# cchao0116/EasyDGL

Hardware: AMD Instinct MI355X
Metric: sequences/sec (fwd+bwd+Adam) B=512 L=100 d=128 |I|=20K (higher is better)
Workload: dtype bf16

## Files before the change

### easydgl_amd/_lib.py

```python
from __future__ import annotations

import ctypes
import os
from ctypes import c_char_p, c_float, c_int, c_int64, c_long, c_uint32, c_void_p

import torch

_HERE = os.path.dirname(os.path.abspath(__file__))
LIB_PATH = os.environ.get("EDGL_LIB_PATH") or os.path.join(_HERE, "libeasydgl_hip.so")

F32, BF16 = 0, 1
EPI_BIAS, EPI_GELU, EPI_SAVE_PRE, EPI_MUL_DGELU, EPI_ACCUM, EPI_OUT_F32, EPI_RELU = 1, 2, 4, 8, 16, 32, 64
MAU_CAUSAL, MAU_NO_DIAG, MAU_DIAG_ZERO = 1, 2, 4
MAU_NO_SKIP = 8
TATTN_CAUSAL = 1

P, I, F, L, U32, I64 = c_void_p, c_int, c_float, c_long, c_uint32, c_int64

SIGNATURES = {
    "edgl_last_error": (c_char_p, []),
    "edgl_version": (I, []),
    "edgl_profile_next": (I, [I, P, P]),
    "edgl_rng_advance": (I, [P, P]),
    "edgl_mask_random": (I, [P, I, I, I, I64, P, U32, P, P, P, P]),
    "edgl_mask_last": (I, [P, I, I, I64, P, P]),
    "edgl_encode_fwd": (I, [P, P, P, P, P, P, P, I, I, I, I, I, I64, F, F, P, U32, P, P, P, I, P]),
    "edgl_encode_bwd_workspace": (L, [I, I, I]),
    "edgl_encode_bwd": (I, [P, P, P, I, I, I, I, I, F, P, U32, P, P, P, P, I, P]),
    "edgl_encode_bwd_add": (I, [P, P, P, P, P, I, I, I, I, I, F, P, U32, P, P, P, P, I, P]),
    "edgl_encode_fwd_ct": (I, [P, P, P, P, P, P, P, I, I, I, I, I, I64, F, F, P, U32, P, P, P, I, I, I, P]),
    "edgl_encode_fwd_prep": (I, [P, P, P, P, P, P, P, I, I, I, I, I, I64, F, F, P, U32, P, P, P, I, I, P, I, P, P, P, P, P, P, I, P]),
    "edgl_encode_bwd_add_ct": (I, [P, P, P, P, P, I, I, I, I, I, F, P, U32, P, P, P, P, I, I, P]),
    "edgl_encode_bwd_label_fused": (I, [I, I]),
    "edgl_encode_bwd_add_label": (I, [P, P, P, P, P, I, I, I, I, I, F, P, U32, P, P, P, P, I, P, P, P, P, I, P, I, P]),
    "edgl_embed_pos_fwd": (I, [P, P, P, P, P, I, I, I, I, F, F, P, U32, P, P, P, I, P]),
    "edgl_embed_pos_bwd": (I, [P, P, I, I, I, I, F, P, U32, P, P, I, P]),
    "edgl_embed_pos_fwd_ct": (I, [P, P, P, P, P, I, I, I, I, F, F, P, U32, P, P, P, I, I, P]),
    "edgl_embed_pos_bwd_ct": (I, [P, P, I, I, I, I, F, P, U32, P, P, I, I, P]),
    "edgl_gemm": (I, [P, P, P, I, I, I, I, I, I, I, I, P, P, I, I, P, I, P]),
    "edgl_colsum": (I, [P, I, I, I, P, I, P, I, I, P]),
    "edgl_gemm_dw_workspace": (L, [I, I, I, I]),
    "edgl_gemm_dw": (I, [P, P, P, P, I, I, I, I, I, I, P, I, P]),
    "edgl_gemm_dw_defer": (I, [I, P]),
    "edgl_bimau_pack_bytes": (L, [I, I, I, I]),
    "edgl_bimau_pack": (I, [P, P, P, P, I, I, I, P, I, P]),
    "edgl_bimau_saved_bytes": (L, [I, I, I, I, I]),
    "edgl_bimau_mark_group": (I, [I, I, I]),
    "edgl_bimau_fwd": (I, [P, P, I, P, P, P, P, I, I, I, I, I, F, P, U32, P, P, P, I, I, P]),
    "edgl_bimau_fwd_zr": (I, [P, P, I, P, P, P, P, I, I, I, I, I, F, P, U32, P, P, P, P, I, I, P]),
    "edgl_bimau_dropbits_bytes": (L, [I, I, I]),
    "edgl_bimau_dropbits": (I, [I, I, I, F, P, U32, P, P]),
    "edgl_bimau_fwd_db": (I, [P, P, I, P, P, P, P, I, I, I, I, I, F, P, U32, P, F, P, P, P, P, I, I, P]),
    "edgl_bimau_bwd_db": (I, [P, P, P, P, P, P, P, P, P, I, I, I, I, I, F, P, U32, P, F, P, P, P, P, P, P, I, I, P]),
    "edgl_bimau_job_order": (I, [P, I, I, P, P]),
    "edgl_bimau_fwd_ord": (I, [P, P, I, P, P, P, P, I, I, I, I, I, F, P, U32, P, F, P, P, P, P, P, I, I, P]),
    "edgl_bimau_bwd_ord": (I, [P, P, P, P, P, P, P, P, I, P, F, P, P, P, I, I, I, I, I, F, P, U32, P, F, P, P, P, P, P, P, P, I, I, P]),
    "edgl_bimau_bwd_workspace": (L, [I, I, I, I, I, I]),
    "edgl_bimau_bwd": (I, [P, P, P, P, P, P, P, P, P, I, I, I, I, I, F, P, U32, P, P, P, P, P, P, I, I, P]),
    "edgl_add_layernorm_fwd": (I, [P, P, I, P, P, I, I, I, F, P, U32, P, I, P, P, I, P]),
    "edgl_add_layernorm_bwd": (I, [P, P, I, P, P, P, I, I, I, F, P, U32, P, I, P, P, P, P, P, P, I, P]),
    "edgl_add_layernorm_bwd_act": (I, [P, P, I, P, P, P, I, I, I, F, P, U32, P, I, P, P, P, P, P, P, P, I, P]),
    "edgl_add_layernorm_fwd_ct": (I, [P, P, I, P, P, I, I, I, F, P, U32, P, I, P, P, I, I, I, P]),
    "edgl_add_layernorm_bwd_act_ct": (I, [P, P, I, P, P, P, I, I, I, F, P, U32, P, I, P, P, P, P, P, P, P, I, I, I, P]),
    "edgl_score_chunks": (I, [I, I]),
    "edgl_compact_rows": (I, [P, P, I, I, P, P, P, P, P, I, P]),
    "edgl_compact_scan": (I, [P, I, P, P, P, P]),
    "edgl_compact_scan_labels": (I, [P, I, P, P, P, P, P]),
    "edgl_compact_gather": (I, [P, P, P, I, I, P, P, I, P]),
    "edgl_scatter_rows": (I, [P, P, I, I, P, I, P]),
    "edgl_score_lse_fwd": (I, [P, P, P, P, I, I, I, I, I, P, P, P, P, P, I, P]),
    "edgl_ce_loss_fwd": (I, [P, P, P, I, P, P, P]),
    "edgl_ce_loss_fwd_add": (I, [P, P, P, I, P, P, P, P, P]),
    "edgl_ce_loss_fwd_add_w": (I, [P, P, P, I, P, P, P, P, P, P]),
    "edgl_score_bwd_workspace": (L, [I, I, I, I, I]),
    "edgl_score_ce_bwd": (I, [P, P, P, P, P, P, P, I, I, I, I, I, P, P, P, P, P, I, P]),
    "edgl_score_flash_workspace": (L, [I, I, I, I, I]),
    "edgl_score_flash_fwd": (I, [P, P, P, P, I, I, I, I, I, P, P, P, P, I, P]),
    "edgl_score_prepare_table": (I, [P, I, I, I, I, I, P, I, P]),
    "edgl_score_flash_fwd_pre": (I, [P, P, P, P, I, I, I, I, I, P, P, P, P, I, I, P]),
    "edgl_score_flash_fwd_coef": (I, [P, P, P, P, I, I, I, P, P, P, P, P, I, P]),
    "edgl_score_flash_fwd_coef_w": (I, [P, P, P, P, I, I, I, P, P, P, P, P, P, I, P]),
    "edgl_score_flash_fwd_rows_w": (I, [P, P, P, P, I, I, I, P, P, P, P, P, P, P, P, I, P]),
    "edgl_score_ce_nparts": (I, [I, I]),
    "edgl_score_flash_fwd_rows_wp": (I, [P, P, P, P, I, I, I, P, P, P, P, P, P, P, P, P, I, P]),
    "edgl_ce_loss_parts": (I, [P, I, P, P, P, P, P]),
    "edgl_score_flash_bwd": (I, [P, P, P, P, P, P, P, I, I, I, I, I, P, P, P, P, P, I, P]),
    "edgl_score_flash_bwd_ex": (I, [P, P, P, P, P, P, P, I, I, I, I, I, P, P, P, P, P, I, I, P]),
    "edgl_score_flash_label_term": (I, [P, P, P, P, I, I, I, I, I, P, P, P, I, P]),
    "edgl_reduce_defer": (I, [I, P]),
    "edgl_reduce_flush": (I, [P]),
    "edgl_mask_topk": (I, [P, I, I, I, P, I, I, P, P, P]),
    "edgl_score_topk_fused_supported": (I, [I, I, I, I, I, I]),
    "edgl_score_topk_fused_workspace": (L, [I, I, I, I, I]),
    "edgl_score_topk_fused": (I, [P, P, P, P, I, I, I, I, I, I, I, P, P, P, I, P]),
    "edgl_topk_merge": (I, [P, P, I, I, I, P, P, P]),
    "edgl_rank_metrics": (I, [P, I, I, P, P, P]),
    "edgl_tpp_workspace": (I, []),
    "edgl_tpp_fwd": (I, [P, P, P, P, P, I, I, I, I, I, F, P, P, I, P]),
    "edgl_tpp_bwd": (I, [P, P, P, P, P, I, I, I, I, I, F, P, P, P, P]),
    "edgl_tpp_fwd_bwd": (I, [P, P, P, P, P, I, I, I, I, I, F, P, P, I, P, P]),
    "edgl_tpp_norm": (I, [P, P, I, I, I, P, P]),
    "edgl_tpp_fwd_bwd_ex": (I, [P, P, P, P, P, I, I, I, I, I, F, P, P, I, P, I, P]),
    "edgl_tpp_rows_workspace": (L, [I, I, I]),
    "edgl_tpp_fwd_bwd_rows": (I, [P, P, P, P, P, I, I, I, I, I, F, P, P, I, P, P]),
    "edgl_tpp_prep_bytes": (L, [I, I, I]),
    "edgl_tpp_prep": (I, [P, P, P, P, I, I, I, I, P, P]),
    "edgl_bimau_bwd_tpp": (I, [P, P, P, P, P, P, P, I, P, F, P, P, P, I, I, I, I, I, F, P, U32, P, F, P, P, P, P, P, P, I, I, P]),
# ... 130 lines not shown
```

### easydgl_amd/csrc/bimau_bwd_impl.h

```cpp
#pragma once
#include <algorithm>

#include "bimau_common.h"

#ifdef EDGL_PHASE_TIMING
extern __device__ unsigned long long g_phase_cycles[16];
#endif

namespace bimau {


constexpr int KY_ECH = 8;
constexpr int KY_NY = EP / KY_ECH;
constexpr int KY_BLOCKS = 384;

constexpr int WG_NJ64 = 4;
constexpr int big_nj(int dh) { return dh == 64 ? WG_NJ64 : 32 / (dh / 16); }
inline int big_row_splits(int dh, int E) {
    const int nc = big_nj(dh) * 16;
    const int groups = std::max(1, (dh * E + nc - 1) / nc);
    return std::max(16, 512 / groups);
}

struct WsLayout { size_t dz, dh, rowdot, dsc, wpart, total; };
inline WsLayout ws_layout(int B, int T_, int C, int H, int E) {
    const int dh = C / H;
    const bool big = dh >= 64;
    const size_t R = (size_t)B * H * T_;
    WsLayout w;
    size_t o = 0;
    auto take = [&](size_t bytes) { const size_t at = o; o += (bytes + 255) & ~(size_t)255; return at; };
    w.dz = take(R * EP * sizeof(float));
    w.dh = take((size_t)(big ? 1 : KY_NY) * R * dh * sizeof(float));
    w.rowdot = take(R * sizeof(float));
    w.dsc = take((size_t)B * H * EP * sizeof(float));
    w.wpart = take((size_t)(big ? big_row_splits(dh, E) : KY_BLOCKS) * ((size_t)(dh + 3) * dh * E + EP) * sizeof(float));
    w.total = o;
    return w;
}

struct BwdP {
    const void* qkvt; const int64_t* ids; const float* spans; const uint8_t* marks; const char* pack;
    const void* d_out; const float* d_lam_ext; const float* lam; const float* z; const void* hin;
    int B, T, C, H, E;
    float rate; const uint64_t* rng; uint32_t stream_id;
    void* d_qkvt;
    float* dz_ws; float* dh_ws; float* rowdot_ws; float* dsc_part; float* wpart;
    int waves;
    int flags;
    int noskip;
    const uint32_t* dbits;
    float qk_scale;
    const void* tpp_desc; int tpp_M; const float* tpp_sums; float tpp_coef;
    const int32_t* order;
    float* tpp_part;
};

template <typename T>
__device__ __forceinline__ void st_frag(T* dst, const f32x4& a) {
    Frag4<T> f = frag_from_acc<T>(a);
    if constexpr (sizeof(T) == 4) *reinterpret_cast<uint4*>(dst) = *reinterpret_cast<uint4*>(&f);
    else *reinterpret_cast<uint2*>(dst) = *reinterpret_cast<uint2*>(&f);
}

template <typename T, int DT, int NT, int EC, bool PREF = true, int FL = -1, bool DB = false, bool TP = false, bool SK = false>
__global__ __launch_bounds__(256) void bimau_bwd_sweep1_kernel(BwdP p) {
    constexpr int dh = 16 * DT, Tp = 16 * NT, LDT = Tp + 4;
    extern __shared__ __attribute__((aligned(16))) char smem[];
    const int E = EC ? EC : p.E;
    const int lane = threadIdx.x & 63, wave = __builtin_amdgcn_readfirstlane(threadIdx.x >> 6);
    const long slot = (long)blockIdx.x * p.waves + wave;
    if (slot >= (long)p.B * p.H) return;
    const int sb = (int)(slot / p.H), head = (int)(slot % p.H);
    const int b = p.order ? __builtin_amdgcn_readfirstlane(p.order[sb]) : sb;
    const long job = (long)b * p.H + head;
    const long bp = (long)head * p.B + b;
    const int g4 = (lane >> 4) * 4, l15 = lane & 15;
    constexpr bool SWZ = img_swz<T>();
    const int g4s = SWZ ? swz_col<16>(l15, g4) : g4;
    int cw[DT];
#pragma unroll
    for (int ub = 0; ub < DT; ++ub) cw[ub] = SWZ ? swz_col<16 * DT>(l15, ub * 16 + g4) : ub * 16 + g4;

    constexpr bool TR = sizeof(T) == 2;
    constexpr size_t EXTRA = TR ? 0 : (size_t)EP * LDT;
    constexpr size_t MASK_ELEMS = (size_t)Tp * sizeof(float) / sizeof(T);
    constexpr size_t WAVE_ELEMS = 2 * (size_t)Tp * dh + (size_t)Tp * EP + EXTRA + MASK_ELEMS;
    T* Ks = reinterpret_cast<T*>(smem) + (size_t)wave * WAVE_ELEMS;
    T* Vs = Ks + Tp * dh;
    T* Ms = Vs + Tp * dh;
    T* MTs = Ms + Tp * EP;
    const T* qkvt = reinterpret_cast<const T*>(p.qkvt) + (long)b * p.T * 4 * p.C;
    const T* dout = reinterpret_cast<const T*>(p.d_out) + (long)b * p.T * p.C;
    T* dqkvt = reinterpret_cast<T*>(p.d_qkvt) + (long)b * p.T * 4 * p.C;
    const int ldq = 4 * p.C;
    const KeyMask<NT> km = stage_wave<T, DT, NT, EC>(
        qkvt + p.C + head * dh, Ks, nullptr, static_cast<const T*>(nullptr), static_cast<T*>(nullptr), static_cast<T*>(nullptr),
        qkvt + 2 * p.C + head * dh, Vs, nullptr, ldq, p.marks + (long)b * p.T * E, E, Ms, TR ? nullptr : MTs,
        p.ids + (long)b * p.T, reinterpret_cast<float*>(Ks + WAVE_ELEMS - MASK_ELEMS), p.T, LDT, lane);
    __builtin_amdgcn_fence(__ATOMIC_RELEASE, "wavefront");
    __builtin_amdgcn_wave_barrier();

    const PackDims pd = pack_dims<T>(dh, E);
    const float* iscs_g = reinterpret_cast<const float*>(p.pack + pd.off_f32) + 3 * pd.JE + EP;
    float isc[4];
#pragma unroll
    for (int i = 0; i < 4; ++i) isc[i] = iscs_g[g4 + i];

    const float cscale = p.qk_scale > 0.f ? p.qk_scale : rsqrtf((float)dh);
    const DropKey dk = make_dropkey(p.rng, p.stream_id, p.rate);
    const Frag4<T> ident = identity_frag<T>(lane);
    const f32x4 zero4 = {0.f, 0.f, 0.f, 0.f};

    struct QOps { Frag4<T> qf[DT], dof[DT]; float4 z; float lam[4], dlx[4]; uint32_t kb; uint32_t nmw; float spr; };
    const float* dlx_src = p.d_lam_ext ? p.d_lam_ext : p.lam;
    const float dlx_on = p.d_lam_ext ? 1.0f : 0.0f;
    TppDesc td{};
    int tp_novf = 0;
    float tp_k = 0.f;
    if constexpr (TP) {
        td = tpp_desc(p.tpp_desc, p.B, p.T, p.tpp_M);
        tp_novf = __builtin_amdgcn_readfirstlane(td.novf[b]);
        int cnt;
        if (p.tpp_sums) {
            cnt = reinterpret_cast<const int*>(p.tpp_sums)[4];
        } else {
            cnt = 0;
            for (int i = lane; i < p.B; i += 64) cnt += td.cntp[i];
            for (int o = 32; o > 0; o >>= 1) cnt += __shfl_xor(cnt, o, 64);
        }
        tp_k = -p.tpp_coef / ((float)cnt * (float)p.H);
        if (job == 0 && lane == 0) reinterpret_cast<int*>(p.tpp_part)[2 * p.B * p.H] = cnt;
    }
    auto load_q = [&](int qt) {
        QOps o;
        const int q = min(qt * 16 + l15, p.T - 1);
        const long row = bp * p.T + q;
#pragma unroll
        for (int ub = 0; ub < DT; ++ub) {
            o.qf[ub] = frag_ld<T>(qkvt + (long)q * ldq + head * dh + ub * 16 + g4);
            o.dof[ub] = frag_ld<T>(dout + (long)q * p.C + head * dh + ub * 16 + g4);
        }
        o.z = *reinterpret_cast<const float4*>(p.z + row * EP + g4);
        if constexpr (DB) o.kb = p.dbits[(bp * NT + qt) * 64 + lane];
        if constexpr (TP) {
            const float4 l4 = *reinterpret_cast<const float4*>(p.lam + row * EC + g4);
            o.lam[0] = l4.x; o.lam[1] = l4.y; o.lam[2] = l4.z; o.lam[3] = l4.w;
            o.dlx[0] = 0.f; o.dlx[1] = 0.f; o.dlx[2] = 0.f; o.dlx[3] = 0.f;
            o.nmw = td.nmw[((long)b * p.T + q) * 4 + (lane >> 4)];
            o.spr = td.spr[(long)b * p.T + q];
        } else if constexpr (EC == 16) {
            const float4 l4 = *reinterpret_cast<const float4*>(p.lam + row * EC + g4), d4 = *reinterpret_cast<const float4*>(dlx_src + row * EC + g4);
            o.lam[0] = l4.x; o.lam[1] = l4.y; o.lam[2] = l4.z; o.lam[3] = l4.w;
            o.dlx[0] = d4.x; o.dlx[1] = d4.y; o.dlx[2] = d4.z; o.dlx[3] = d4.w;
        } else {
#pragma unroll
            for (int i = 0; i < 4; ++i) {
                const int e = min(g4 + i, E - 1);
                o.lam[i] = p.lam[row * E + e];
                o.dlx[i] = dlx_src[row * E + e];
            }
        }
        return o;
    };
    auto mask_q = [&](QOps& o, bool ok) {
#pragma unroll
        for (int ub = 0; ub < DT; ++ub)
            if (!ok) o.dof[ub] = frag_zero<T>();
#pragma unroll
        for (int i = 0; i < 4; ++i) {
            const bool oke = ok && (EC == 16 || (g4 + i) < E);
            o.lam[i] = oke ? o.lam[i] : 0.f;
            o.dlx[i] = oke ? o.dlx[i] * dlx_on : 0.f;
        }
    };
    PH_DECL
    auto run = [&](auto nk_c) {
    constexpr int NK = decltype(nk_c)::value, K0 = NT - NK;
    const KeyMask<NK> kmk = keymask_tail<NK, NT>(km);
    float dsc_acc[4] = {0.f, 0.f, 0.f, 0.f}, tp_a = 0.f, tp_b = 0.f;
    f32x4 dVa[DT][NK];
#pragma unroll
    for (int u = 0; u < DT; ++u)
#pragma unroll
        for (int kt = 0; kt < NK; ++kt) dVa[u][kt] = zero4;
    QOps qcur = load_q(0);
    touch_regs(qcur);
    float pend_dz[4] = {0.f, 0.f, 0.f, 0.f}, pend_rowdot = 0.f;
    int pend_q = p.T;
    auto flush_pending = [&]() {
        if (pend_q < p.T) {
            *reinterpret_cast<float4*>(p.dz_ws + (bp * p.T + pend_q) * EP + g4) = make_float4(pend_dz[0], pend_dz[1], pend_dz[2], pend_dz[3]);
            if (lane < 16) p.rowdot_ws[bp * p.T + pend_q] = pend_rowdot;
        }
    };
    for (int qt = 0; qt < NT; ++qt) {
        asm volatile("" ::: "memory");
        const int q = qt * 16 + l15;
        const bool qok = q < p.T;
        QOps qnext;
        if constexpr (PREF) qnext = load_q(qt + 1 < NT ? qt + 1 : qt);
        asm volatile("" ::: "memory");
        mask_q(qcur, qok);
        if constexpr (TP) {
            float gr[4] = {0.f, 0.f, 0.f, 0.f};
            tpp_slot(qcur.lam, qcur.nmw, qcur.spr, qok && qcur.spr >= 0.f, tp_k, gr, tp_a, tp_b);
            for (int j = 0; j < tp_novf; ++j) {
                const int tj = td.ovf_pos[(long)b * td.M + j];
                if ((tj >> 4) != qt) continue;
                tpp_slot(qcur.lam, td.ovf_nm[((long)b * td.M + j) * 4 + (lane >> 4)], qcur.spr, qok && q == tj, tp_k, gr, tp_a, tp_b);
            }
#pragma unroll
            for (int i = 0; i < 4; ++i) qcur.dlx[i] = gr[i];
        }
        const float zq4[4] = {qcur.z.x, qcur.z.y, qcur.z.z, qcur.z.w};
        f32x4 s[NK];
#pragma unroll
        for (int kt = 0; kt < NK; ++kt) {
            f32x4 a = zero4;
#pragma unroll
            for (int ub = 0; ub < DT; ++ub)
                a = mma16(frag_ld<T>(Ks + ((K0 + kt) * 16 + l15) * dh + cw[ub]), qcur.qf[ub], a);
            s[kt] = a;
        }
        if constexpr (FL == 0) masked_softmax_impl<NK, false, false>(s, kmk, cscale, lane, q, dk.scale);
        else {
            masked_softmax<NK, 0>(s, kmk, cscale, lane, q, (p.flags & MAU_CAUSAL) != 0);
#pragma unroll
            for (int kt = 0; kt < NK; ++kt)
#pragma unroll
                for (int r = 0; r < 4; ++r) s[kt][r] *= dk.scale;
        }
        asm volatile("" ::: "memory");
        flush_pending();
        asm volatile("" ::: "memory");
        PH_MARK(0);
        Frag4<T> lf;
#pragma unroll
        for (int i = 0; i < 4; ++i) lf.v[i] = from_f32<T>(qcur.lam[i]);
        Frag4<T> dOT[DT];
#pragma unroll
        for (int vt = 0; vt < DT; ++vt) dOT[vt] = frag_from_acc<T>(mma16(qcur.dof[vt], ident, zero4));
        float rowdot = 0.f;
        f32x4 dlamT = zero4;
        const uint32_t dbase = (uint32_t)((bp * p.T + q) * p.T);
#pragma unroll
        for (int kt = 0; kt < NK; ++kt) {
            const f32x4 gacc = mma16(frag_ld<T>(Ms + ((K0 + kt) * 16 + l15) * EP + g4s), lf, zero4);
            f32x4 da = zero4;
#pragma unroll
            for (int vb = 0; vb < DT; ++vb)
                da = mma16(frag_ld<T>(Vs + ((K0 + kt) * 16 + l15) * dh + cw[vb]), qcur.dof[vb], da);
            f32x4 ap, dg, gv = gacc;
            const bool dtile = K0 + kt == qt && (FL == 0 || !(p.flags & MAU_NO_DIAG));
            if constexpr (FL == 0) {
#pragma unroll
                for (int r = 0; r < 4; ++r) gv[r] = (dtile && g4 + r == l15) ? 1.0f : gacc[r];
            } else if (dtile) {
#pragma unroll
                for (int r = 0; r < 4; ++r) gv[r] = (g4 + r == l15) ? ((p.flags & MAU_DIAG_ZERO) ? 0.0f : 1.0f) : gacc[r];
            }
            uint64_t hw = 0ull;
            if constexpr (!DB) hw = drop_hash_quad(dk, dbase + (K0 + kt) * 16 + g4);
            const bool keep[4] = {drop_quad_keep<0>(dk, hw), drop_quad_keep<1>(dk, hw), drop_quad_keep<2>(dk, hw), drop_quad_keep<3>(dk, hw)};
#pragma unroll
            for (int r = 0; r < 4; ++r) {
                float fp;
                if constexpr (DB) fp = keep_bit(qcur.kb, (K0 + kt) * 4 + r, s[kt][r]);
                else fp = keep[r] ? s[kt][r] : 0.f;
                ap[r] = gv[r] * fp;
                dg[r] = da[r] * fp;
                rowdot = fmaf(dg[r], gv[r], rowdot);
            }
            if constexpr (FL == 0) {
#pragma unroll
                for (int r = 0; r < 4; ++r) dg[r] = (dtile && g4 + r == l15) ? 0.f : dg[r];
            } else if (dtile) {
#pragma unroll
                for (int r = 0; r < 4; ++r) dg[r] = (g4 + r == l15) ? 0.f : dg[r];
            }
            dlamT = mma16(kfrag<T, SWZ ? 16 : 0>(Ms, EP, MTs, LDT, (K0 + kt) * 16, 0, lane), frag_from_acc<T>(dg), dlamT);
            const Frag4<T> apT = frag_from_acc<T>(transpose_tile<T>(ap, ident));
#pragma unroll
            for (int vt = 0; vt < DT; ++vt) dVa[vt][kt] = mma16(dOT[vt], apT, dVa[vt][kt]);
            if (kt & 1) __builtin_amdgcn_sched_barrier(0);
        }
        PH_MARK(1);
        float dz4[4];
#pragma unroll
        for (int i = 0; i < 4; ++i) {
            const float dl = dlamT[i] + qcur.dlx[i];
            const float sg = sigmoid_f(zq4[i] * isc[i]);
            dz4[i] = dl * sg;
            if (qok && (EC == 16 || (g4 + i) < E)) dsc_acc[i] += dl * (qcur.lam[i] - zq4[i] * sg);
        }
        pend_rowdot = group_sum4(rowdot);
#pragma unroll
        for (int i = 0; i < 4; ++i) pend_dz[i] = dz4[i];
        pend_q = q;
        if constexpr (PREF) qcur = qnext;
        else if (qt + 1 < NT) qcur = load_q(qt + 1);
        PH_MARK(2);
    }
#pragma unroll
    for (int i = 0; i < 4; ++i) {
        float v = dsc_acc[i];
        v += __shfl_xor(v, 1, 64); v += __shfl_xor(v, 2, 64); v += __shfl_xor(v, 4, 64); v += __shfl_xor(v, 8, 64);
        dsc_acc[i] = v;
    }
    if constexpr (TP) {
#pragma unroll
        for (int o = 1; o < 16; o <<= 1) { tp_a += __shfl_xor(tp_a, o, 64); tp_b += __shfl_xor(tp_b, o, 64); }
    }
    flush_pending();
    if constexpr (TP) {
        if (lane == 0) *reinterpret_cast<float2*>(p.tpp_part + job * 2) = make_float2(tp_a, tp_b);
    }
    if (l15 == 0) *reinterpret_cast<float4*>(p.dsc_part + job * EP + g4) = make_float4(dsc_acc[0], dsc_acc[1], dsc_acc[2], dsc_acc[3]);
#pragma unroll
    for (int kt = 0; kt < NT; ++kt) {
        const int k = kt * 16 + l15;
        if (k < p.T) {
#pragma unroll
            for (int ut = 0; ut < DT; ++ut) {
                T* dst = dqkvt + (long)k * ldq + 2 * p.C + head * dh + ut * 16 + g4;
                if constexpr (K0 > 0) {
                    if (kt < K0) st_frag<T>(dst, zero4);
                    else st_frag<T>(dst, dVa[ut][kt < K0 ? 0 : kt - K0]);
                } else {
                    st_frag<T>(dst, dVa[ut][kt]);
                }
            }
        }
    }
    };
    if constexpr (SK) {
        static_assert(FL == 0 && sizeof(T) == 2, "the key-tile skip exists for the bidirectional bf16 form");
        dispatch_nk<NT>(NT - km.kt0, run);
    } else {
        run(std::integral_constant<int, NT>{});
    }
    PH_MARK(3);
    PH_FLUSH(0);
}

template <typename T, int DT, int NT, int EC, int NYP = KY_NY, bool PREF = true, int FL = -1, bool DB = false, int US = 1, int SL = 0, bool SK = false>
__global__ __launch_bounds__(256) void bimau_bwd_sweep2_kernel(BwdP p) {
    constexpr int dh = 16 * DT, Tp = 16 * NT, LDT = Tp + 4;
    static_assert(DT % US == 0 && SL < US, "channel slices");
    constexpr int DTS = DT / US, U0 = SL * DTS;
    extern __shared__ __attribute__((aligned(16))) char smem[];
    const int E = EC ? EC : p.E;
    const int lane = threadIdx.x & 63, wave = __builtin_amdgcn_readfirstlane(threadIdx.x >> 6);
    const long slot = (long)blockIdx.x * p.waves + wave;
    if (slot >= (long)p.B * p.H) return;
    const int sb = (int)(slot / p.H), head = (int)(slot % p.H);
    const int b = p.order ? __builtin_amdgcn_readfirstlane(p.order[sb]) : sb;
    const long job = (long)b * p.H + head;
    const long bp = (long)head * p.B + b;
    const int g4 = (lane >> 4) * 4, l15 = lane & 15;
    constexpr bool SWZ = img_swz<T>();
    const int g4s = SWZ ? swz_col<16>(l15, g4) : g4;
    int cw[DT];
#pragma unroll
    for (int ub = 0; ub < DT; ++ub) cw[ub] = SWZ ? swz_col<16 * DT>(l15, ub * 16 + g4) : ub * 16 + g4;

    constexpr bool TR = sizeof(T) == 2;
    constexpr size_t EXTRA = TR ? 0 : (size_t)dh * LDT;
    constexpr size_t MASK_ELEMS = (size_t)Tp * sizeof(float) / sizeof(T);
    constexpr size_t WAVE_ELEMS = 3 * (size_t)Tp * dh + (size_t)Tp * EP + EXTRA + MASK_ELEMS;
    T* Ks = reinterpret_cast<T*>(smem) + (size_t)wave * WAVE_ELEMS;
    T* Ts = Ks + Tp * dh;
    T* Vs = Ts + Tp * dh;
    T* Ms = Vs + Tp * dh;
    T* KTs = Ms + Tp * EP;
    const T* qkvt = reinterpret_cast<const T*>(p.qkvt) + (long)b * p.T * 4 * p.C;
    const T* dout = reinterpret_cast<const T*>(p.d_out) + (long)b * p.T * p.C;
    const T* hin = reinterpret_cast<const T*>(p.hin);
    T* dqkvt = reinterpret_cast<T*>(p.d_qkvt) + (long)b * p.T * 4 * p.C;
    const int ldq = 4 * p.C;
    const KeyMask<NT> km = stage_wave<T, DT, NT, EC>(
        qkvt + p.C + head * dh, Ks, TR ? nullptr : KTs, qkvt + 3 * p.C + head * dh, Ts, static_cast<T*>(nullptr),
        qkvt + 2 * p.C + head * dh, Vs, static_cast<T*>(nullptr), ldq, p.marks + (long)b * p.T * E, E, Ms, static_cast<T*>(nullptr),
        p.ids + (long)b * p.T, reinterpret_cast<float*>(Ks + WAVE_ELEMS - MASK_ELEMS), p.T, LDT, lane);
    __builtin_amdgcn_fence(__ATOMIC_RELEASE, "wavefront");
    __builtin_amdgcn_wave_barrier();

    const float cscale = p.qk_scale > 0.f ? p.qk_scale : rsqrtf((float)dh);
    const DropKey dk = make_dropkey(p.rng, p.stream_id, p.rate);
    float cz = cscale;
    if constexpr (FL == 0) {
        bool real = false;
        for (int k = lane; k < Tp; k += 64) real |= km.madd[k] == 0.f;
        cz = __any(real) ? cscale : 0.f;
    }
    (void)cz;
    const Frag4<T> ident = identity_frag<T>(lane);
    const f32x4 zero4 = {0.f, 0.f, 0.f, 0.f};
    const long R = (long)p.B * p.H * p.T;

    struct QOps { Frag4<T> qf[DT], dof[DT], hf[DT]; float4 dHp[DT][NYP]; float lam[4], rowdot; uint32_t kb; };
    auto load_q = [&](int qt) {
        QOps o;
        const int q = min(qt * 16 + l15, p.T - 1);
        const long row = bp * p.T + q;
#pragma unroll
        for (int ub = 0; ub < DT; ++ub) {
            o.qf[ub] = frag_ld<T>(qkvt + (long)q * ldq + head * dh + ub * 16 + g4);
            o.dof[ub] = frag_ld<T>(dout + (long)q * p.C + head * dh + ub * 16 + g4);
            o.hf[ub] = frag_ld<T>(hin + row * dh + ub * 16 + g4);
#pragma unroll
            for (int y = 0; y < NYP; ++y)
                o.dHp[ub][y] = *reinterpret_cast<const float4*>(p.dh_ws + ((long)y * R + row) * dh + ub * 16 + g4);
        }
        if constexpr (EC == 16) {
            const float4 l4 = *reinterpret_cast<const float4*>(p.lam + row * EC + g4);
            o.lam[0] = l4.x; o.lam[1] = l4.y; o.lam[2] = l4.z; o.lam[3] = l4.w;
        } else {
#pragma unroll
            for (int i = 0; i < 4; ++i) o.lam[i] = p.lam[row * E + min(g4 + i, E - 1)];
        }
        o.rowdot = p.rowdot_ws[row];
        if constexpr (DB) o.kb = p.dbits[(bp * NT + qt) * 64 + lane];
        return o;
    };
    PH_DECL
#ifdef EDGL_PHASE_TIMING
    const unsigned long long clk_m0 = __builtin_readcyclecounter(), clk_r0 = wall_clock64();
#endif
    auto run = [&](auto nk_c) {
    constexpr int NK = decltype(nk_c)::value, K0 = NT - NK;
    const KeyMask<NK> kmk = keymask_tail<NK, NT>(km);
    f32x4 dKa[DTS][NK], dTa[DTS][NK];
#pragma unroll
    for (int u = 0; u < DTS; ++u)
#pragma unroll
        for (int kt = 0; kt < NK; ++kt) { dKa[u][kt] = zero4; dTa[u][kt] = zero4; }
    QOps qcur = load_q(0);
    touch_regs(qcur);
    Frag4<T> pend_dq[DTS];
    int pend_q = p.T;
    auto flush_pending = [&]() {
        if (pend_q < p.T) {
#pragma unroll
            for (int ut = 0; ut < DTS; ++ut) {
                T* dst = dqkvt + (long)pend_q * ldq + head * dh + (U0 + ut) * 16 + g4;
                if constexpr (sizeof(T) == 4) *reinterpret_cast<uint4*>(dst) = *reinterpret_cast<uint4*>(&pend_dq[ut]);
                else *reinterpret_cast<uint2*>(dst) = *reinterpret_cast<uint2*>(&pend_dq[ut]);
            }
        }
    };
#pragma unroll
    for (int ut = 0; ut < DTS; ++ut) pend_dq[ut] = frag_zero<T>();
    for (int qt = 0; qt < NT; ++qt) {
        asm volatile("" ::: "memory");
        const int q = qt * 16 + l15;
        const bool qok = q < p.T;
        (void)qok;
        QOps qnext;
        if constexpr (PREF) qnext = load_q(qt + 1 < NT ? qt + 1 : qt);
        asm volatile("" ::: "memory");
        PH_MARK(3);
        f32x4 dHq[DT];
#pragma unroll
        for (int ub = 0; ub < DT; ++ub) {
            f32x4 a = zero4;
#pragma unroll
            for (int y = 0; y < NYP; ++y) {
                a[0] += qcur.dHp[ub][y].x; a[1] += qcur.dHp[ub][y].y; a[2] += qcur.dHp[ub][y].z; a[3] += qcur.dHp[ub][y].w;
            }
#pragma unroll
            for (int r = 0; r < 4; ++r) dHq[ub][r] = qok ? a[r] : 0.f;
            if (!qok) qcur.dof[ub] = frag_zero<T>();
        }
        const float rowdot1 = qok ? qcur.rowdot : 0.f;
        PH_MARK(4);
        f32x4 s[NK];
#pragma unroll
        for (int kt = 0; kt < NK; ++kt) {
            f32x4 a = zero4;
#pragma unroll
            for (int ub = 0; ub < DT; ++ub)
                a = mma16(frag_ld<T>(Ks + ((K0 + kt) * 16 + l15) * dh + cw[ub]), qcur.qf[ub], a);
            s[kt] = a;
        }
        PH_MARK(5);
        if constexpr (FL == 0) masked_softmax_impl<NK, false, false>(s, kmk, cscale, lane, q);
        else masked_softmax<NK, 0>(s, kmk, cscale, lane, q, (p.flags & MAU_CAUSAL) != 0);
        asm volatile("" ::: "memory");
        flush_pending();
        asm volatile("" ::: "memory");
        PH_MARK(0);
        Frag4<T> lf;
#pragma unroll
        for (int i = 0; i < 4; ++i) lf.v[i] = from_f32<T>((EC == 16 || (g4 + i) < E) ? qcur.lam[i] * dk.scale : 0.f);
        float rowdot = 0.f;
        Frag4<T> dhf[DT], QT[DTS], dHT[DTS];
#pragma unroll
        for (int ut = 0; ut < DT; ++ut) {
#pragma unroll
            for (int r = 0; r < 4; ++r) rowdot = fmaf(dHq[ut][r], to_f32(qcur.hf[ut].v[r]), rowdot);
            dhf[ut] = frag_from_acc<T>(dHq[ut]);
        }
#pragma unroll
        for (int ut = 0; ut < DTS; ++ut) {
            QT[ut] = frag_from_acc<T>(mma16(qcur.qf[U0 + ut], ident, zero4));
            dHT[ut] = frag_from_acc<T>(transpose_tile<T>(dHq[U0 + ut], ident));
        }
        rowdot = group_sum4(rowdot) + rowdot1;
        f32x4 dQ[DTS];
#pragma unroll
        for (int ut = 0; ut < DTS; ++ut) dQ[ut] = zero4;
        const uint32_t dbase = (uint32_t)((bp * p.T + q) * p.T);
#pragma unroll
        for (int kt = 0; kt < NK; ++kt) {
            const f32x4 gacc = mma16(frag_ld<T>(Ms + ((K0 + kt) * 16 + l15) * EP + g4s), lf, zero4);
            f32x4 da = zero4;
#pragma unroll
            for (int vb = 0; vb < DT; ++vb)
                da = mma16(frag_ld<T>(Vs + ((K0 + kt) * 16 + l15) * dh + cw[vb]), qcur.dof[vb], da);
            f32x4 gv = gacc;
            if constexpr (FL == 0) {
                const bool dtile = K0 + kt == qt;
#pragma unroll
                for (int r = 0; r < 4; ++r) gv[r] = (dtile && g4 + r == l15) ? dk.scale : gacc[r];
            } else if (kt == qt && !(p.flags & MAU_NO_DIAG)) {
#pragma unroll
                for (int r = 0; r < 4; ++r) gv[r] = (g4 + r == l15) ? ((p.flags & MAU_DIAG_ZERO) ? 0.0f : dk.scale) : gacc[r];
            }
            uint64_t hw = 0ull;
            if constexpr (!DB) hw = drop_hash_quad(dk, dbase + (K0 + kt) * 16 + g4);
            const bool keep[4] = {drop_quad_keep<0>(dk, hw), drop_quad_keep<1>(dk, hw), drop_quad_keep<2>(dk, hw), drop_quad_keep<3>(dk, hw)};
            f32x4 a;
#pragma unroll
            for (int r = 0; r < 4; ++r) {
                if constexpr (DB) a[r] = keep_bit(qcur.kb, (K0 + kt) * 4 + r, da[r] * gv[r]);
                else a[r] = keep[r] ? da[r] * gv[r] : 0.f;
            }
#pragma unroll
            for (int ub = 0; ub < DT; ++ub)
                a = mma16(frag_ld<T>(Ts + ((K0 + kt) * 16 + l15) * dh + cw[ub]), dhf[ub], a);
            f32x4 ds;
#pragma unroll
            for (int r = 0; r < 4; ++r) {
                if constexpr (FL == 0) {
                    ds[r] = s[kt][r] * (a[r] - rowdot);
                } else {
                    const bool padded = ((km.pad >> (kt * 4 + r)) & 1ull) || ((p.flags & MAU_CAUSAL) && kt * 16 + g4 + r > q);
                    ds[r] = padded ? 0.f : s[kt][r] * (a[r] - rowdot) * cscale;
                }
            }
            const Frag4<T> dsf = frag_from_acc<T>(ds);
#pragma unroll
            for (int ut = 0; ut < DTS; ++ut)
                dQ[ut] = mma16(kfrag<T, SWZ ? 16 * DT : 0>(Ks, dh, KTs, LDT, (K0 + kt) * 16, (U0 + ut) * 16, lane), dsf, dQ[ut]);
            const Frag4<T> dsT = frag_from_acc<T>(transpose_tile<T>(ds, ident));
            const Frag4<T> pT = frag_from_acc<T>(transpose_tile<T>(s[kt], ident));
#pragma unroll
            for (int ut = 0; ut < DTS; ++ut) {
                dKa[ut][kt] = mma16(QT[ut], dsT, dKa[ut][kt]);
                dTa[ut][kt] = mma16(dHT[ut], pT, dTa[ut][kt]);
            }
        }
#pragma unroll
        for (int ut = 0; ut < DTS; ++ut) {
            if constexpr (FL == 0) {
#pragma unroll
                for (int r = 0; r < 4; ++r) dQ[ut][r] *= cz;
            }
            pend_dq[ut] = frag_from_acc<T>(dQ[ut]);
        }
        pend_q = q;
        if constexpr (PREF) qcur = qnext;
        else if (qt + 1 < NT) qcur = load_q(qt + 1);
        PH_MARK(1);
    }
    flush_pending();
#pragma unroll
    for (int kt = 0; kt < NT; ++kt) {
        const int k = kt * 16 + l15;
        if (k < p.T) {
#pragma unroll
            for (int ut = 0; ut < DTS; ++ut) {
                T* row = dqkvt + (long)k * ldq + head * dh + (U0 + ut) * 16 + g4;
                if (kt < K0) {
                    st_frag<T>(row + p.C, zero4);
                    st_frag<T>(row + 3 * p.C, zero4);
                } else {
                    const int kk = kt < K0 ? 0 : kt - K0;
                    if constexpr (FL == 0) {
#pragma unroll
                        for (int r = 0; r < 4; ++r) dKa[ut][kk][r] *= cz;
                    }
                    st_frag<T>(row + p.C, dKa[ut][kk]);
                    st_frag<T>(row + 3 * p.C, dTa[ut][kk]);
                }
            }
        }
    }
    };
    if constexpr (SK) {
        static_assert(FL == 0 && sizeof(T) == 2, "the key-tile skip exists for the bidirectional bf16 form");
        dispatch_nk<NT>(NT - km.kt0, run);
    } else {
        run(std::integral_constant<int, NT>{});
    }
    PH_MARK(2);
    PH_FLUSH(8);
#ifdef EDGL_PHASE_TIMING
    if (lane == 0) { atomicAdd(&g_phase_cycles[14], __builtin_readcyclecounter() - clk_m0); atomicAdd(&g_phase_cycles[15], wall_clock64() - clk_r0); }
#endif
}


int big_bwd(const BwdP& p, char* ws, float* dW1, float* db1, float* dw, float* dsc, int dtype, hipStream_t st);

}
```

### easydgl_amd/csrc/bimau_common.h

```cpp
#pragma once
#include <cstdlib>
#include <type_traits>

#include "edgl_common.h"

namespace bimau {

constexpr int EP = 16;
constexpr float NLOG2E = -1.4426950408889634f;

__device__ __forceinline__ float sigmoid_pre(float xs) { return fast_rcp(1.0f + __builtin_amdgcn_exp2f(xs)); }

constexpr int XW = 8;
struct PackDims {
    int dh, E, JE, LDW, LDR;
    size_t off_w1x, off_f32, off_w1r, fwd_bytes, bytes;
};
template <typename T>
__host__ __device__ inline PackDims pack_dims(int dh, int E) {
    PackDims d;
    d.dh = dh; d.E = E; d.JE = dh * E; d.LDW = dh + 4; d.LDR = d.JE + 4;
    size_t w1t = (size_t)d.JE * d.LDW * sizeof(T);
    w1t = (w1t + 15) & ~(size_t)15;
    const size_t w1x = sizeof(T) == 2 ? (size_t)d.JE * XW * sizeof(T) : 0;
// ... 58 lines not shown
}

template <typename T>
__global__ void pack_kernel(const float* W1, const float* b1, const float* w, const float* scaling, int dh, int E,
                            char* pack) {
    const PackDims d = pack_dims<T>(dh, E);
    T* w1t = reinterpret_cast<T*>(pack);
    T* w1r = reinterpret_cast<T*>(pack + d.off_w1r);
    float* f = reinterpret_cast<float*>(pack + d.off_f32);
    const int tid = blockIdx.x * blockDim.x + threadIdx.x, nth = gridDim.x * blockDim.x;
    if constexpr (sizeof(T) == 2) {
        T* w1x = reinterpret_cast<T*>(pack + d.off_w1x);
        for (int j = tid; j < d.JE; j += nth) {
            const Split3 w = split3(NLOG2E * W1[(long)dh * d.JE + j]), b = split3(NLOG2E * b1[j]);
            T* r = w1x + (long)j * XW;
            r[0] = w.t0; r[1] = w.t1; r[2] = w.t0; r[3] = w.t2; r[4] = w.t1; r[5] = w.t0; r[6] = b.t0; r[7] = b.t1;
        }
    }
    for (int i = tid; i < d.JE * d.LDW; i += nth) {
        const int j = i / d.LDW, u = i % d.LDW;
        w1t[i] = from_f32<T>(u < dh ? NLOG2E * W1[(long)u * d.JE + j] : 0.f);
    }
    for (int i = tid; i < dh * d.LDR; i += nth) {
        const int u = i / d.LDR, j = i % d.LDR;
        w1r[i] = from_f32<T>(j < d.JE ? W1[(long)u * d.JE + j] : 0.f);
    }
    for (int j = tid; j < d.JE; j += nth) {
        f[j] = NLOG2E * W1[(long)dh * d.JE + j];
        f[d.JE + j] = NLOG2E * b1[j];
        f[2 * d.JE + j] = w[j];
    }
    for (int e = tid; e < EP; e += nth) {
        const float s = e < E ? __expf(scaling[e]) : 1.f;
        f[3 * d.JE + e] = s;
        f[3 * d.JE + EP + e] = 1.f / s;
    }
}

template <int NT>
struct KeyMask { const float* madd; uint64_t pad; int kt0; };
template <int NR>
__device__ __forceinline__ int first_real_tile(const uint64_t (&real)[NR]) {
    int first = -1;
#pragma unroll
    for (int i = NR - 1; i >= 0; --i)
        if (real[i] != 0ull) first = 64 * i + (int)__builtin_ctzll(real[i]);
    return first < 0 ? 0 : first >> 4;
}
template <int NK, int NT>
__device__ __forceinline__ KeyMask<NK> keymask_tail(const KeyMask<NT>& km) {
    constexpr int K0 = NT - NK;
    return KeyMask<NK>{km.madd + K0 * 16, km.pad >> (K0 * 4), 0};
}
inline bool bimau_skip_enabled() {
    return edgl_env_on("EDGL_BIMAU_SKIP");
}
template <int N, typename F>
__device__ __forceinline__ void dispatch_nk(int nk, F&& f) {
    if constexpr (N <= 1) {
        f(std::integral_constant<int, 1>{});
    } else {
        if (nk >= N) f(std::integral_constant<int, N>{});
        else dispatch_nk<N - 1>(nk, f);
    }
}
template <int NT>
__device__ __forceinline__ KeyMask<NT> load_keymask(const int64_t* ids_row, int T, int lane, float* lds_madd) {
    KeyMask<NT> km;
    km.pad = 0ull;
    km.madd = lds_madd;
    constexpr int NR = (16 * NT + 63) / 64;
    uint64_t padded[NR], real[NR];
#pragma unroll
    for (int i = 0; i < NR; ++i) {
        const int k = lane + 64 * i;
        const int64_t id = ids_row[min(k, T - 1)];
        const bool pd = k < T && id == 0;
        padded[i] = __ballot(pd);
        real[i] = __ballot(k < T && id != 0);
        if (k < 16 * NT) lds_madd[k] = k >= T ? -INFINITY : (pd ? -4294967296.0f : 0.f);
    }
    km.kt0 = first_real_tile<NR>(real);
    const int g4 = (lane >> 4) * 4;
#pragma unroll
    for (int kt = 0; kt < NT; ++kt) {
        const uint64_t nib = (padded[kt / 4] >> ((kt % 4) * 16 + g4)) & 0xfull;
        km.pad |= nib << (kt * 4);
    }
    return km;
}

constexpr int MAU_CAUSAL = 1;
constexpr int MAU_NO_DIAG = 2;
constexpr int MAU_DIAG_ZERO = 4;
typedef __attribute__((ext_vector_type(2))) float f32x2;
template <int NT, bool CAUSAL, bool VEC, bool NORM = true>
__device__ __forceinline__ float masked_softmax_impl(f32x4 (&s)[NT], const KeyMask<NT>& km, float cscale, int lane, int q, float post = 1.0f) {
    const float c2 = cscale * 1.4426950408889634f;
    float mx = -INFINITY;
    const float* mrow = km.madd + (lane >> 4) * 4;
#pragma unroll
    for (int kt = 0; kt < NT; ++kt) {
        const f32x4 m4 = *reinterpret_cast<const f32x4*>(mrow + kt * 16);
        f32x4 v;
        if constexpr (VEC) {
            v = s[kt] * f32x4{c2, c2, c2, c2} + m4;
// ... 40 lines not shown
    if constexpr (!NORM) return inv;
    const float f = inv * post;
#pragma unroll
    for (int kt = 0; kt < NT; ++kt) {
        if constexpr (VEC) {
            s[kt] *= f32x4{f, f, f, f};
        } else {
#pragma unroll
            for (int r = 0; r < 4; ++r) s[kt][r] *= f;
        }
    }
    return inv;
}
template <int NT, int MODE = 0>
__device__ __forceinline__ void masked_softmax(f32x4 (&s)[NT], const KeyMask<NT>& km, float cscale, int lane, int q = 0,
                                               bool causal = false) {
    if constexpr (MODE != 0) {
        if (causal) masked_softmax_impl<NT, true, false>(s, km, cscale, lane, q);
        else masked_softmax_impl<NT, false, false>(s, km, cscale, lane, q);
    } else {
        const float c2 = cscale * 1.4426950408889634f;
        float mx = -INFINITY;
        const float* mrow = km.madd + (lane >> 4) * 4;
#pragma unroll
        for (int kt = 0; kt < NT; ++kt) {
            const float4 m4 = *reinterpret_cast<const float4*>(mrow + kt * 16);
            const float mm[4] = {m4.x, m4.y, m4.z, m4.w};
#pragma unroll
            for (int r = 0; r < 4; ++r) {
                float v = fmaf(s[kt][r], c2, mm[r]);
                if (causal && kt * 16 + (lane >> 4) * 4 + r > q && mm[r] != -INFINITY) v = -4294967296.0f;
                s[kt][r] = v;
                mx = fmaxf(mx, v);
            }
        }
        mx = group_max4(mx);
        float sum = 0.f;
#pragma unroll
        for (int kt = 0; kt < NT; ++kt)
#pragma unroll
            for (int r = 0; r < 4; ++r) {
                const float e = __builtin_amdgcn_exp2f(s[kt][r] - mx);
                s[kt][r] = e;
                sum += e;
            }
        sum = group_sum4(sum);
        const float inv = fast_rcp(sum);
#pragma unroll
        for (int kt = 0; kt < NT; ++kt)
#pragma unroll
            for (int r = 0; r < 4; ++r) s[kt][r] *= inv;
    }
}

template <int I>
__device__ __forceinline__ float keep_bit_c(uint32_t kb, float x) {
    int m;
    asm("v_bfe_i32 %0, %1, %2, 1" : "=v"(m) : "v"(kb), "n"(I));
    return __int_as_float(__float_as_int(x) & m);
}
__device__ __forceinline__ float keep_bit(uint32_t kb, int i, float x) {
    switch (i) {
#define EDGL_KB_CASE(n) case n: return keep_bit_c<n>(kb, x);
        EDGL_KB_CASE(0) EDGL_KB_CASE(1) EDGL_KB_CASE(2) EDGL_KB_CASE(3) EDGL_KB_CASE(4) EDGL_KB_CASE(5) EDGL_KB_CASE(6) EDGL_KB_CASE(7)
        EDGL_KB_CASE(8) EDGL_KB_CASE(9) EDGL_KB_CASE(10) EDGL_KB_CASE(11) EDGL_KB_CASE(12) EDGL_KB_CASE(13) EDGL_KB_CASE(14) EDGL_KB_CASE(15)
        EDGL_KB_CASE(16) EDGL_KB_CASE(17) EDGL_KB_CASE(18) EDGL_KB_CASE(19) EDGL_KB_CASE(20) EDGL_KB_CASE(21) EDGL_KB_CASE(22) EDGL_KB_CASE(23)
        EDGL_KB_CASE(24) EDGL_KB_CASE(25) EDGL_KB_CASE(26) EDGL_KB_CASE(27) EDGL_KB_CASE(28) EDGL_KB_CASE(29) EDGL_KB_CASE(30) EDGL_KB_CASE(31)
#undef EDGL_KB_CASE
    }
    return x;
}
template <int NT>
__global__ __launch_bounds__(256) void dropbits_kernel(const uint64_t* rng, uint32_t stream_id, float rate, int T, long njobs, uint32_t* bits) {
    static_assert(NT <= 8, "one 32-bit word per lane and query tile");
    const int lane = threadIdx.x & 63;
    const long job = (long)blockIdx.x * 4 + (threadIdx.x >> 6);
    if (job >= njobs) return;
    const long bp = job / NT;
    const int qt = (int)(job % NT), q = qt * 16 + (lane & 15), g4 = (lane >> 4) * 4;
    const DropKey dk = make_dropkey(rng, stream_id, rate);
    const uint32_t dbase = (uint32_t)((bp * T + q) * T);
    uint32_t w = 0u;
#pragma unroll
    for (int kt = 0; kt < NT; ++kt) {
        const uint64_t hw = drop_hash_quad(dk, dbase + kt * 16 + g4);
        w |= (drop_quad_keep<0>(dk, hw) ? 1u : 0u) << (kt * 4);
        w |= (drop_quad_keep<1>(dk, hw) ? 1u : 0u) << (kt * 4 + 1);
        w |= (drop_quad_keep<2>(dk, hw) ? 1u : 0u) << (kt * 4 + 2);
        w |= (drop_quad_keep<3>(dk, hw) ? 1u : 0u) << (kt * 4 + 3);
    }
    bits[job * 64 + lane] = w;
}

struct TppDesc {
    const uint32_t* nmw;
    const float* spr;
    const int32_t* novf;
    const int32_t* ovf_pos;
    const uint32_t* ovf_nm;
    const int32_t* cntp;
    int M;
};
struct TppLayout { size_t off_spr, off_novf, off_ovf_pos, off_ovf_nm, off_cntp, bytes; };
__host__ __device__ inline TppLayout tpp_layout(int B, int T, int M) {
    TppLayout l;
    l.off_spr = (size_t)B * T * 16;
    l.off_novf = l.off_spr + (size_t)B * T * 4;
    l.off_ovf_pos = (l.off_novf + (size_t)B * 4 + 15) & ~(size_t)15;
    l.off_ovf_nm = (l.off_ovf_pos + (size_t)B * M * 4 + 15) & ~(size_t)15;
    l.off_cntp = l.off_ovf_nm + (size_t)B * M * 16;
    l.bytes = l.off_cntp + (((size_t)B * 4 + 15) & ~(size_t)15);
    return l;
}
__host__ __device__ inline TppDesc tpp_desc(const void* base, int B, int T, int M) {
    const TppLayout l = tpp_layout(B, T, M);
    const char* c = reinterpret_cast<const char*>(base);
    return TppDesc{reinterpret_cast<const uint32_t*>(c), reinterpret_cast<const float*>(c + l.off_spr),
                   reinterpret_cast<const int32_t*>(c + l.off_novf), reinterpret_cast<const int32_t*>(c + l.off_ovf_pos),
                   reinterpret_cast<const uint32_t*>(c + l.off_ovf_nm), reinterpret_cast<const int32_t*>(c + l.off_cntp), M};
}
__device__ __forceinline__ void tpp_bytes(uint32_t w, float (&f)[4]) {
    f[0] = (float)(w & 0xffu); f[1] = (float)((w >> 8) & 0xffu);
    f[2] = (float)((w >> 16) & 0xffu); f[3] = (float)(w >> 24);
}
__device__ __forceinline__ void group_sum4_pair(float& x, float& y) {
    const FPair p = swap16(x, y);
    const float t = p.first + p.second;
    const FPair q = swap32(t, t);
    const float u = q.first + q.second;
    const FPair r = swap16(u, u);
    x = r.first; y = r.second;
}
__device__ __forceinline__ void tpp_slot(const float (&lam4)[4], uint32_t w, float sp, bool on, float k, float (&gr)[4], float& a, float& bs) {
    float f[4];
    tpp_bytes(w, f);
    float ev = lam4[0] * f[0], ent = lam4[0] + lam4[1];
    ev = fmaf(lam4[1], f[1], ev); ev = fmaf(lam4[2], f[2], ev); ev = fmaf(lam4[3], f[3], ev);
    ent += lam4[2] + lam4[3];
    group_sum4_pair(ev, ent);
    ev = on ? ev : 0.f;
    const float hs = sp * 0.5f, kg = on ? k : 0.f;
    a += __logf(ev == 0.f ? 1.f : ev);
    bs = fmaf(on ? ent : 0.f, hs, bs);
// ... 94 lines not shown
#pragma unroll
    for (int i = 0; i < NR; ++i) {
        const int k = lane + 64 * i;
        const uint8_t* row = marks_row + (long)min(k, Tlen - 1) * E;
        uint32_t w[4];
        if constexpr (EC == 16) {
            const uint4 v = *reinterpret_cast<const uint4*>(row);
            w[0] = v.x; w[1] = v.y; w[2] = v.z; w[3] = v.w;
        } else {
            uint8_t by[16];
#pragma unroll
            for (int e = 0; e < 16; ++e) by[e] = row[min(e, E - 1)];
#pragma unroll
            for (int j = 0; j < 4; ++j) {
                w[j] = 0u;
#pragma unroll
                for (int e = 0; e < 4; ++e) w[j] |= (4 * j + e < E ? (uint32_t)by[4 * j + e] : 0u) << (8 * e);
            }
        }
        if (k < Tp) {
            const bool ok = k < Tlen;
            T vals[16];
#pragma unroll
            for (int e = 0; e < 16; ++e) vals[e] = from_f32<T>(ok ? (float)((w[e / 4] >> (8 * (e % 4))) & 0xffu) : 0.f);
            if (rowmajor) {
#pragma unroll
                for (int j = 0; j < (int)(16 * sizeof(T) / 16); ++j)
                    reinterpret_cast<uint4*>(rowmajor + k * EP)[SW ? (j ^ ((k >> 3) & 1)) : j] = reinterpret_cast<const uint4*>(vals)[j];
            }
            if (transposed) {
#pragma unroll
                for (int e = 0; e < 16; ++e) transposed[e * LDT + k] = vals[e];
            }
        }
    }
}

template <typename T, int DT, int NT>
struct RowStage {
    static constexpr int cpr = 4 * DT, dh = 16 * DT, NI = NT * DT;
    Frag4<T> f[NI];
    __device__ __forceinline__ void load(const T* src, int ld, int Tlen, int lane) {
#pragma unroll
        for (int j = 0; j < NI; ++j) {
            const int c = lane + 64 * j, k = c / cpr, u4 = (c % cpr) * 4;
            f[j] = frag_ld<T>(src + (long)min(k, Tlen - 1) * ld + u4);
        }
    }
    __device__ __forceinline__ void pin() {
        static_assert(sizeof(Frag4<T>) == 8, "bf16 fragments");
#pragma unroll
        for (int j = 0; j < NI; ++j) { uint2& u = *reinterpret_cast<uint2*>(&f[j]); asm volatile("" : "+v"(u.x), "+v"(u.y)); }
    }
    __device__ __forceinline__ void store(T* rowmajor, T* transposed, int LDT, int Tlen, int lane) {
#pragma unroll
        for (int j = 0; j < NI; ++j) {
            const int c = lane + 64 * j, k = c / cpr, u4 = (c % cpr) * 4;
            if (k >= Tlen) f[j] = frag_zero<T>();
            if (rowmajor) *reinterpret_cast<uint2*>(rowmajor + k * dh + (img_swz<T>() ? swz_col<dh>(k, u4) : u4)) = *reinterpret_cast<uint2*>(&f[j]);
            if (transposed) {
#pragma unroll
                for (int r = 0; r < 4; ++r) transposed[(u4 + r) * LDT + k] = f[j].v[r];
            }
        }
    }
};
template <typename T, int DT, int NT, int EC>
constexpr bool stage_merged() { return sizeof(T) == 2 && NT * DT <= 8 && EC == 16; }

template <typename T, int DT, int NT, int EC>
__device__ __forceinline__ KeyMask<NT> stage_wave(const T* k_src, T* k_rm, T* k_tr, const T* t_src, T* t_rm, T* t_tr,
                                                  const T* v_src, T* v_rm, T* v_tr, int ld, const uint8_t* marks_row, int E,
                                                  T* m_rm, T* m_tr, const int64_t* ids_row, float* lds_madd, int Tlen, int LDT,
                                                  int lane) {
    if constexpr (stage_merged<T, DT, NT, EC>()) {
        constexpr int Tp = 16 * NT, NR = (Tp + 63) / 64;
        RowStage<T, DT, NT> sk, st, sv;
        uint4 mk[NR];
        int64_t id[NR];
        sk.load(k_src, ld, Tlen, lane);
        if (t_src) st.load(t_src, ld, Tlen, lane);
        if (v_src) sv.load(v_src, ld, Tlen, lane);
#pragma unroll
        for (int i = 0; i < NR; ++i) {
            const int k = min(lane + 64 * i, Tlen - 1);
            if (marks_row) mk[i] = *reinterpret_cast<const uint4*>(marks_row + (long)k * 16);
            id[i] = ids_row[k];
        }
        sk.pin();
        if (t_src) st.pin();
        if (v_src) sv.pin();
#pragma unroll
        for (int i = 0; i < NR; ++i) {
            if (marks_row) asm volatile("" : "+v"(mk[i].x), "+v"(mk[i].y), "+v"(mk[i].z), "+v"(mk[i].w));
            asm volatile("" : "+v"(id[i]));
        }
        sk.store(k_rm, k_tr, LDT, Tlen, lane);
        if (t_src) st.store(t_rm, t_tr, LDT, Tlen, lane);
        if (v_src) sv.store(v_rm, v_tr, LDT, Tlen, lane);
        if (marks_row) {
#pragma unroll
            for (int i = 0; i < NR; ++i) {
                const int k = lane + 64 * i;
                if (k < Tp) {
                    const bool ok = k < Tlen;
                    const uint32_t w[4] = {mk[i].x, mk[i].y, mk[i].z, mk[i].w};
                    T vals[16];
#pragma unroll
                    for (int e = 0; e < 16; ++e) vals[e] = from_f32<T>(ok ? (float)((w[e / 4] >> (8 * (e % 4))) & 0xffu) : 0.f);
                    if (m_rm) {
#pragma unroll
                        for (int j = 0; j < (int)(16 * sizeof(T) / 16); ++j)
                            reinterpret_cast<uint4*>(m_rm + k * EP)[img_swz<T>() ? (j ^ ((k >> 3) & 1)) : j] = reinterpret_cast<const uint4*>(vals)[j];
                    }
                    if (m_tr) {
#pragma unroll
                        for (int e = 0; e < 16; ++e) m_tr[e * LDT + k] = vals[e];
                    }
                }
            }
        }
        KeyMask<NT> km;
        km.pad = 0ull;
        km.madd = lds_madd;
        uint64_t padded[NR], real[NR];
#pragma unroll
        for (int i = 0; i < NR; ++i) {
            const int k = lane + 64 * i;
// ... 24 lines not shown
```

### easydgl_amd/csrc/bimau_fwd_impl.h

```cpp
#pragma once
#include <type_traits>

#include "bimau_common.h"

namespace bimau {

constexpr int FWD_WAVES = 2;

struct FwdP {
    const void* qkvt; const void* resid; int ld_res;
    const int64_t* ids; const float* spans; const uint8_t* marks;
    const char* pack;
    int B, T, C, H, E;
    float rate; const uint64_t* rng; uint32_t stream_id;
    void* out; float* lam;
    void* hin_out; float* z_out;
    float* zero_rows;
    int waves;
    int flags;
    const uint32_t* dbits;
    float qk_scale;
    const int32_t* order;
    int noskip;
};

template <typename T, int DT, int NT, int PHASE>
__host__ __device__ constexpr size_t fwd_wave_bytes() {
    constexpr size_t dh = 16 * DT, Tp = 16 * NT, LDT = Tp + 4;
    constexpr size_t kv = sizeof(T) == 2 ? Tp * dh : dh * LDT;
    return (Tp * dh + (PHASE != 2 ? kv : 0) + (PHASE != 1 ? kv : 0) + (PHASE != 1 ? Tp * EP : 0)) * sizeof(T) + Tp * sizeof(float);
}

template <typename T, int DT, int NT, int EC, int PHASE = 0, bool DB = false, bool SK = false>
__global__ __launch_bounds__(256, (sizeof(T) == 2 && DT == 1 && EC == 16 && PHASE == 0) ? FWD_WAVES : 1) void bimau_fwd_kernel(FwdP p) {
    constexpr int dh = 16 * DT, Tp = 16 * NT, LDT = Tp + 4;
    extern __shared__ __attribute__((aligned(16))) char smem[];
    const int E = EC ? EC : p.E;
    constexpr bool FUSED = PHASE == 0, HAS_T = PHASE != 2, HAS_V = PHASE != 1, HAS_M = PHASE != 1;
    const PackDims pd = pack_dims<T>(dh, E);
    const size_t pack_bytes = FUSED ? pd.fwd_bytes : 0;
    if constexpr (FUSED) copy_pack_to_lds(smem, p.pack, pd.fwd_bytes);
    const T* W1T = reinterpret_cast<const T*>(smem);
    const T* W1X = reinterpret_cast<const T*>(smem + pd.off_w1x);
    const float* fW = reinterpret_cast<const float*>(smem + pd.off_f32);
    const float* w1s = fW; const float* b1s = fW + pd.JE; const float* wvs = fW + 2 * pd.JE;
    const float* scs = fW + 3 * pd.JE; const float* iscs = scs + EP;
    (void)W1T; (void)W1X; (void)w1s; (void)b1s; (void)wvs; (void)scs; (void)iscs;
    if constexpr (FUSED) __syncthreads();

    const int lane = threadIdx.x & 63, wave = __builtin_amdgcn_readfirstlane(threadIdx.x >> 6);
    const long slot = (long)blockIdx.x * p.waves + wave;
    if (slot >= (long)p.B * p.H) return;
    const int sb = (int)(slot / p.H), head = (int)(slot % p.H);
    const int b = p.order ? __builtin_amdgcn_readfirstlane(p.order[sb]) : sb;
    const long job = (long)b * p.H + head;
    const long bp = (long)head * p.B + b;

    constexpr bool TR = sizeof(T) == 2;
    constexpr size_t KV_ELEMS = TR ? (size_t)Tp * dh : (size_t)dh * LDT;
    constexpr size_t MASK_ELEMS = (size_t)Tp * sizeof(float) / sizeof(T);
    constexpr size_t WAVE_ELEMS = (size_t)Tp * dh + (HAS_T ? KV_ELEMS : 0) + (HAS_V ? KV_ELEMS : 0) + (HAS_M ? (size_t)Tp * EP : 0) + MASK_ELEMS;
    static_assert(WAVE_ELEMS * sizeof(T) == fwd_wave_bytes<T, DT, NT, PHASE>(), "host / device LDS layouts differ");
    T* Ks = reinterpret_cast<T*>(smem + pack_bytes) + (size_t)wave * WAVE_ELEMS;
    T* Ts = Ks + Tp * dh;
    T* Vs = Ts + (HAS_T ? KV_ELEMS : 0);
    T* Ms = Vs + (HAS_V ? KV_ELEMS : 0);
    const T* qkvt = reinterpret_cast<const T*>(p.qkvt) + (long)b * p.T * 4 * p.C;
    const int ldq = 4 * p.C;
    const KeyMask<NT> km = stage_wave<T, DT, NT, EC>(
        qkvt + p.C + head * dh, Ks, nullptr,
        HAS_T ? qkvt + 3 * p.C + head * dh : nullptr, TR ? Ts : nullptr, TR ? nullptr : Ts,
        HAS_V ? qkvt + 2 * p.C + head * dh : nullptr, TR ? Vs : nullptr, TR ? nullptr : Vs, ldq,
        HAS_M ? p.marks + (long)b * p.T * E : nullptr, E, Ms, nullptr, p.ids + (long)b * p.T,
        reinterpret_cast<float*>(Ms + (HAS_M ? Tp * EP : 0)), p.T, LDT, lane);
    __builtin_amdgcn_fence(__ATOMIC_RELEASE, "wavefront");
    __builtin_amdgcn_wave_barrier();

    const float cscale = p.qk_scale > 0.f ? p.qk_scale : rsqrtf((float)dh);
    const DropKey dk = make_dropkey(p.rng, p.stream_id, p.rate);
    const int g4 = (lane >> 4) * 4, l15 = lane & 15;
    constexpr bool SWZ = img_swz<T>();
    const int g4s = SWZ ? swz_col<16>(l15, g4) : g4;
    int cw[DT];
#pragma unroll
    for (int ub = 0; ub < DT; ++ub) cw[ub] = SWZ ? swz_col<16 * DT>(l15, ub * 16 + g4) : ub * 16 + g4;

    struct QOps { Frag4<T> qf[DT], rf[DT]; float span; float lam[4]; uint32_t kb; };
    auto load_q = [&](int qt) {
        QOps o;
        const int q = min(qt * 16 + l15, p.T - 1);
#pragma unroll
        for (int ub = 0; ub < DT; ++ub) {
            o.qf[ub] = frag_ld<T>(qkvt + (long)q * ldq + head * dh + ub * 16 + g4);
            o.rf[ub] = frag_ld<T>(reinterpret_cast<const T*>(p.resid) + ((long)b * p.T + q) * p.ld_res + head * dh + ub * 16 + g4);
        }
        o.span = p.spans[(long)b * p.T + q];
        if constexpr (DB) o.kb = p.dbits[(bp * NT + qt) * 64 + lane];
        if constexpr (PHASE == 2) {
#pragma unroll
            for (int i = 0; i < 4; ++i) o.lam[i] = p.lam[(bp * p.T + q) * E + min(g4 + i, E - 1)];
        }
        return o;
    };
    auto run = [&](auto nk_c) {
    constexpr int NK = decltype(nk_c)::value, K0 = NT - NK;
    const KeyMask<NK> kmk = keymask_tail<NK, NT>(km);
    QOps qcur = load_q(0);
    touch_regs(qcur);
    Frag4<T> pend_o[DT];
#pragma unroll
    for (int ut = 0; ut < DT; ++ut) pend_o[ut] = frag_zero<T>();
    int pend_q = p.T;
    auto flush_pending = [&]() {
        if (pend_q < p.T) {
#pragma unroll
            for (int ut = 0; ut < DT; ++ut) {
                T* dst = reinterpret_cast<T*>(p.out) + ((long)b * p.T + pend_q) * p.C + head * dh + ut * 16 + g4;
                if constexpr (sizeof(T) == 4) *reinterpret_cast<uint4*>(dst) = *reinterpret_cast<uint4*>(&pend_o[ut]);
                else *reinterpret_cast<uint2*>(dst) = *reinterpret_cast<uint2*>(&pend_o[ut]);
            }
        }
    };
    for (int qt = 0; qt < NT; ++qt) {
        const int q = qt * 16 + l15;
        const bool qok = q < p.T;
        const QOps qnext = load_q(qt + 1 < NT ? qt + 1 : qt);
        asm volatile("" ::: "memory");
        Frag4<T> qf[DT];
#pragma unroll
        for (int ub = 0; ub < DT; ++ub) qf[ub] = qcur.qf[ub];
        f32x4 s[NK];
#pragma unroll
        for (int kt = 0; kt < NK; ++kt) {
            f32x4 a = {0.f, 0.f, 0.f, 0.f};
#pragma unroll
            for (int ub = 0; ub < DT; ++ub)
                a = mma16(frag_ld<T>(Ks + ((K0 + kt) * 16 + l15) * dh + cw[ub]), qf[ub], a);
            s[kt] = a;
        }
        float pinv = 1.0f;
        if constexpr (TR) {
            if constexpr (K0 == 0) {
                if (p.flags & MAU_CAUSAL) pinv = masked_softmax_impl<NT, true, false, false>(s, kmk, cscale, lane, q);
                else pinv = masked_softmax_impl<NT, false, false, false>(s, kmk, cscale, lane, q);
            } else {
                pinv = masked_softmax_impl<NK, false, false, false>(s, kmk, cscale, lane, q);
            }
        } else {
            masked_softmax<NT, 0>(s, kmk, cscale, lane, q, (p.flags & MAU_CAUSAL) != 0);
        }
        const float gfac = pinv * dk.scale;
        asm volatile("" ::: "memory");
        flush_pending();
        asm volatile("" ::: "memory");
        Frag4<T> pf[NK];
#pragma unroll
        for (int kt = 0; kt < NK; ++kt) pf[kt] = frag_from_acc<T>(s[kt]);
        Frag4<T> hf[DT];
        if constexpr (HAS_T) {
#pragma unroll
            for (int ut = 0; ut < DT; ++ut) {
                f32x4 a = {0.f, 0.f, 0.f, 0.f};
#pragma unroll
                for (int kt = 0; kt < NK; ++kt)
                    a = mma16(kfrag<T, SWZ ? 16 * DT : 0>(Ts, dh, Ts, LDT, (K0 + kt) * 16, ut * 16, lane), pf[kt], a);
                if constexpr (TR) {
#pragma unroll
                    for (int r = 0; r < 4; ++r) a[r] *= pinv;
                }
                hf[ut] = frag_from_acc<T>(a);
                if (p.hin_out && qok) {
                    T* dst = reinterpret_cast<T*>(p.hin_out) + (bp * p.T + q) * dh + ut * 16 + g4;
                    if constexpr (sizeof(T) == 4) *reinterpret_cast<uint4*>(dst) = *reinterpret_cast<uint4*>(&hf[ut]);
                    else *reinterpret_cast<uint2*>(dst) = *reinterpret_cast<uint2*>(&hf[ut]);
                }
            }
        }
        if constexpr (PHASE == 1) {
            qcur = qnext;
            continue;
        }
        Frag4<T> lf;
        if constexpr (FUSED) {
        const float span = qcur.span;
        float zp[16];
        struct MlpOps { Frag4<T> w[DT]; Frag4<T> wx; f32x4 ws, bs, wv; };
        Frag4<T> sf;
        if constexpr (TR) sf = span_frag(span, lane);
        auto load_ops = [&](int jt) {
            MlpOps o;
#pragma unroll
            for (int ub = 0; ub < DT; ++ub) o.w[ub] = frag_ld<T>(W1T + (jt * 16 + l15) * pd.LDW + ub * 16 + g4);
            if constexpr (TR) {
                o.wx = frag_ld<T>(W1X + (jt * 16 + l15) * XW + (g4 & 4));
            } else {
// ... 41 lines not shown
                if ((jt + 2) % DT == 0) zp[e1] = zacc;
                c0 = n0; c1 = n1; n0 = m0; n1 = m1; a0 = b0; a1 = b1;
                EDGL_PIN();
            }
        } else {
            MlpOps cur = load_ops(0);
#pragma unroll
            for (int e = 0; e < 16; ++e) {
                zp[e] = 0.f;
                if (e < E) {
                    float zacc;
#pragma unroll
                    for (int d = 0; d < DT; ++d) {
                        const int jt = e * DT + d;
                        const MlpOps nxt = load_ops(jt + 1 < E * DT ? jt + 1 : jt);
                        EDGL_PIN();
                        const f32x4 a = tile_pre(cur);
                        tile_post(a, cur, zacc, d == 0);
                        cur = nxt;
                        EDGL_PIN();
                    }
                    zp[e] = zacc;
                }
            }
        }
        float z4[4];
        reduce_scatter16(zp, z4, lane);
        if (p.z_out && qok) *reinterpret_cast<float4*>(p.z_out + (bp * p.T + q) * EP + g4) = make_float4(z4[0], z4[1], z4[2], z4[3]);
        float lam4[4];
#pragma unroll
        for (int i = 0; i < 4; ++i) {
            const float sc = scs[g4 + i], isc = iscs[g4 + i];
            lam4[i] = sc * __logf(1.0f + __expf(z4[i] * isc));
            lf.v[i] = from_f32<T>(lam4[i] * gfac);
        }
        if (qok) {
            float* dst = p.lam + (bp * p.T + q) * E + g4;
            if constexpr (EC == 16) {
                *reinterpret_cast<float4*>(dst) = make_float4(lam4[0], lam4[1], lam4[2], lam4[3]);
                if (p.zero_rows) *reinterpret_cast<float4*>(p.zero_rows + (bp * p.T + q) * E + g4) = make_float4(0.f, 0.f, 0.f, 0.f);
            } else {
#pragma unroll
                for (int i = 0; i < 4; ++i)
                    if (g4 + i < E) { dst[i] = lam4[i]; if (p.zero_rows) p.zero_rows[(bp * p.T + q) * E + g4 + i] = 0.f; }
            }
        }
        } else {
#pragma unroll
            for (int i = 0; i < 4; ++i) lf.v[i] = from_f32<T>(qcur.lam[i] * gfac);
        }
        const uint32_t dbase = (uint32_t)((bp * p.T + q) * p.T);
        const bool set_diag = !(p.flags & MAU_NO_DIAG);
        const float dval = (p.flags & MAU_DIAG_ZERO) ? 0.0f : gfac;
        auto modulate = [&](auto drop_on) {
#pragma unroll
            for (int kt = 0; kt < NK; ++kt) {
                f32x4 gacc = mma16(frag_ld<T>(Ms + ((K0 + kt) * 16 + l15) * EP + g4s), lf, f32x4{0.f, 0.f, 0.f, 0.f});
                const bool dtile = set_diag && K0 + kt == qt;
#pragma unroll
                for (int r = 0; r < 4; ++r) {
                    gacc[r] = (dtile && g4 + r == l15) ? dval : gacc[r];
                    s[kt][r] = gacc[r] * s[kt][r];
                }
                if constexpr (decltype(drop_on)::value) {
                    if constexpr (DB) {
#pragma unroll
                        for (int r = 0; r < 4; ++r) s[kt][r] = keep_bit(qcur.kb, (K0 + kt) * 4 + r, s[kt][r]);
                    } else {
                        const uint64_t hw = drop_hash_quad(dk, dbase + (K0 + kt) * 16 + g4);
                        s[kt][0] = drop_quad_keep<0>(dk, hw) ? s[kt][0] : 0.f;
                        s[kt][1] = drop_quad_keep<1>(dk, hw) ? s[kt][1] : 0.f;
                        s[kt][2] = drop_quad_keep<2>(dk, hw) ? s[kt][2] : 0.f;
                        s[kt][3] = drop_quad_keep<3>(dk, hw) ? s[kt][3] : 0.f;
                    }
                }
                pf[kt] = frag_from_acc<T>(s[kt]);
            }
        };
        if (dk.thresh != 0u) modulate(std::true_type{});
        else modulate(std::false_type{});
#pragma unroll
        for (int vt = 0; vt < DT; ++vt) {
            f32x4 a = {0.f, 0.f, 0.f, 0.f};
#pragma unroll
            for (int kt = 0; kt < NK; ++kt)
                a = mma16(kfrag<T, SWZ ? 16 * DT : 0>(Vs, dh, Vs, LDT, (K0 + kt) * 16, vt * 16, lane), pf[kt], a);
            const Frag4<T> rf = qcur.rf[vt];
            f32x4 o4;
#pragma unroll
            for (int r = 0; r < 4; ++r) o4[r] = a[r] + to_f32(rf.v[r]);
            pend_o[vt] = frag_from_acc<T>(o4);
        }
        pend_q = q;
        qcur = qnext;
    }
    flush_pending();
    };
    if constexpr (SK) {
        static_assert(TR && PHASE == 0, "the key-tile skip exists for the fused bf16 form");
        dispatch_nk<NT>((p.flags & MAU_CAUSAL) ? NT : NT - km.kt0, run);
    } else {
        run(std::integral_constant<int, NT>{});
    }
}

template <typename T, int DT, int NT, int EC, int PHASE = 0>
int launch_fwd_e(FwdP p, hipStream_t st) {
    constexpr int dh = 16 * DT;
    const size_t pack_bytes = PHASE == 0 ? pack_dims<T>(dh, p.E).fwd_bytes : 0;
    constexpr size_t wave_bytes = fwd_wave_bytes<T, DT, NT, PHASE>();
    int waves = 4;
    while (waves > 1 && pack_bytes + waves * wave_bytes > 80 * 1024) waves >>= 1;
    if (waves == 1 && pack_bytes + wave_bytes > 80 * 1024)
        while (waves < 4 && pack_bytes + (waves + 1) * wave_bytes <= 160 * 1024) ++waves;
    const size_t smem = pack_bytes + waves * wave_bytes;
    EDGL_REQUIRE(smem <= 160 * 1024, EDGL_ERR_SHAPE, "edgl_bimau_fwd: needs %zu B of LDS (dh=%d E=%d T=%d)", smem, dh,
                 p.E, p.T);
    p.waves = waves;
    auto kern = bimau_fwd_kernel<T, DT, NT, EC, PHASE>;
    if constexpr (sizeof(T) == 2 && DT == 1 && EC == 16 && PHASE == 0 && NT <= 8) {
        const bool sk = NT >= 2 && bimau_skip_enabled() && !p.noskip;
        if (p.dbits && p.rate > 0.f) kern = sk ? bimau_fwd_kernel<T, DT, NT, EC, PHASE, true, (NT >= 2)> : bimau_fwd_kernel<T, DT, NT, EC, PHASE, true>;
        else if (sk) kern = bimau_fwd_kernel<T, DT, NT, EC, PHASE, false, (NT >= 2)>;
    }
    if (smem > 48 * 1024) hipFuncSetAttribute((const void*)kern, hipFuncAttributeMaxDynamicSharedMemorySize, (int)smem);
    const long jobs = (long)p.B * p.H;
    hipLaunchKernelGGL(kern, dim3((unsigned)((jobs + waves - 1) / waves)), dim3(64 * waves), smem, st, p);
    EDGL_LAUNCH_CHECK();
    return EDGL_OK;
}

template <typename T, int DT, int NT>
int launch_fwd(FwdP p, hipStream_t st) {
    return p.E == 16 ? launch_fwd_e<T, DT, NT, 16>(p, st) : launch_fwd_e<T, DT, NT, 0>(p, st);
}

template <typename T, int DT>
int dispatch_nt(FwdP p, hipStream_t st) {
    const int nt = (p.T + 15) / 16;
    switch (nt) {
        case 1: return launch_fwd<T, DT, 1>(p, st);
        case 2: return launch_fwd<T, DT, 2>(p, st);
        case 3: return launch_fwd<T, DT, 3>(p, st);
        case 4: return launch_fwd<T, DT, 4>(p, st);
        case 5: return launch_fwd<T, DT, 5>(p, st);
        case 6: return launch_fwd<T, DT, 6>(p, st);
        case 7: return launch_fwd<T, DT, 7>(p, st);
        case 8: return launch_fwd<T, DT, 8>(p, st);
        case 9: return launch_fwd<T, DT, 9>(p, st);
        case 10: return launch_fwd<T, DT, 10>(p, st);
        case 11: return launch_fwd<T, DT, 11>(p, st);
        case 12: return launch_fwd<T, DT, 12>(p, st);
        case 13: return launch_fwd<T, DT, 13>(p, st);
    }
    edgl_set_error("edgl_bimau_fwd: T=%d not supported (T <= 208)", p.T);
    return EDGL_ERR_SHAPE;
}


int big_fwd(const FwdP& p, int dtype, hipStream_t st);

}
```

### easydgl_amd/csrc/k_bimau_bwd.hip

```cpp
#include <algorithm>
#include <cstdlib>

#include "bimau_bwd_impl.h"

#ifdef EDGL_PHASE_TIMING
__device__ unsigned long long g_phase_cycles[16];
#endif

namespace {
using namespace bimau;

template <typename T>
constexpr int intensity_bwd_nreg(int DT) {
    return KY_ECH * DT * DT * 4 + (sizeof(T) == 2 ? (KY_ECH / 4) * DT * 4 : 2 * KY_ECH * DT) + KY_ECH * DT;
}

struct MlpP {
    const void* hin; const float* dz_ws; const float* spans; const char* pack;
    long R; int B, T, E; float* dh_ws; float* wpart; const float* dsc_part; long njobs;
    int slab_epi;
};

template <typename T, int DT, int EC>
__global__ __launch_bounds__(256, (sizeof(T) == 2 && DT == 1) ? 3 : 1) void intensity_bwd_kernel(MlpP p) {
// ... 254 lines not shown
#pragma unroll
                            for (int r = 0; r < 4; ++r) {
                                const int j = jt * 16 + g4 + r, u = ub * 16 + l15;
                                accs[j * (dh + 1) + u] += dW[ee][d][ub][r];
                            }
                    }
                }
            }
        }
        __syncthreads();
    }
    for (int i = threadIdx.x; i < NPAR; i += blockDim.x) {
        const int e = (i % JE) / dh;
        const int row = i / JE, j = i - row * JE;
        if (e >= e0 && e < e0 + ECH) p.wpart[(long)blockIdx.x * NPARX + i] = row < dh ? accs[j * (dh + 1) + row] : accs[WROW + (row - dh) * JE + j];
    }
    }
    if (blockIdx.y == 0) {
        const long per = (p.njobs + gridDim.x - 1) / gridDim.x;
        const long j0 = blockIdx.x * per, j1 = min(p.njobs, j0 + per);
        const int e = threadIdx.x & 15, sl = threadIdx.x >> 4;
        float a = 0.f;
        for (long j = j0 + sl; j < j1; j += 16) a += p.dsc_part[j * EP + e];
        __syncthreads();
        accs[sl * EP + e] = a;
        __syncthreads();
        if (threadIdx.x < EP) {
            float v = 0.f;
#pragma unroll
            for (int k = 0; k < 16; ++k) v += accs[k * EP + threadIdx.x];
            p.wpart[(long)blockIdx.x * NPARX + NPAR + threadIdx.x] = v;
        }
    }
    PH_MARK(7);
    PH_FLUSH(0);
}

template <typename T>
size_t intensity_bwd_lds(int dh, int E) {
    const int NACC = dh * E * (dh + 4);
    return pack_dims<T>(dh, E).bytes + ((size_t)((NACC + 3) & ~3) + 4 * (16 * KY_ECH + 16)) * sizeof(float);
}

template <typename T, int DT, int NT>
int launch_bwd(BwdP p, char* ws, float* dW1, float* db1, float* dw, float* dscaling, hipStream_t st) {
    constexpr int dh = 16 * DT, Tp = 16 * NT, LDT = Tp + 4;
    const PackDims pd = pack_dims<T>(dh, p.E);
    const WsLayout wl = ws_layout(p.B, p.T, p.C, p.H, p.E);
    p.dz_ws = reinterpret_cast<float*>(ws + wl.dz); p.dh_ws = reinterpret_cast<float*>(ws + wl.dh);
    p.rowdot_ws = reinterpret_cast<float*>(ws + wl.rowdot);
    p.dsc_part = reinterpret_cast<float*>(ws + wl.dsc); p.wpart = reinterpret_cast<float*>(ws + wl.wpart);
    const long jobs = (long)p.B * p.H;
    constexpr bool TR = sizeof(T) == 2;
    edgl_prof_begin(EDGL_KERNEL_BIMAU_BWD_ALL, st);
    {
        const size_t wave_bytes = (2 * (size_t)Tp * dh + (size_t)Tp * EP + (TR ? 0 : (size_t)EP * LDT)) * sizeof(T) + (size_t)Tp * sizeof(float);
        int waves = 4;
        while (waves > 1 && waves * wave_bytes > 64 * 1024) waves >>= 1;
        const size_t smem = waves * wave_bytes;
        p.waves = waves;
        constexpr bool SPEC = sizeof(T) == 2 && DT == 1;
        auto kern = p.E == 16 ? bimau_bwd_sweep1_kernel<T, DT, NT, 16> : bimau_bwd_sweep1_kernel<T, DT, NT, 0>;
        if constexpr (SPEC) {
            if (p.flags == 0) kern = p.E == 16 ? bimau_bwd_sweep1_kernel<T, DT, NT, 16, true, 0> : bimau_bwd_sweep1_kernel<T, DT, NT, 0, true, 0>;
            if constexpr (NT <= 8) {
                constexpr bool SKC = NT >= 2;
                const bool sk = SKC && p.flags == 0 && p.E == 16 && bimau_skip_enabled() && !p.noskip;
                const bool db = p.dbits && p.rate > 0.f;
                if (p.flags == 0 && p.E == 16 && db) kern = sk ? bimau_bwd_sweep1_kernel<T, DT, NT, 16, true, 0, true, false, SKC> : bimau_bwd_sweep1_kernel<T, DT, NT, 16, true, 0, true>;
                else if (sk) kern = bimau_bwd_sweep1_kernel<T, DT, NT, 16, true, 0, false, false, SKC>;
                if (p.tpp_desc) {
                    if (sk) kern = db ? bimau_bwd_sweep1_kernel<T, DT, NT, 16, true, 0, true, true, SKC> : bimau_bwd_sweep1_kernel<T, DT, NT, 16, true, 0, false, true, SKC>;
                    else kern = db ? bimau_bwd_sweep1_kernel<T, DT, NT, 16, true, 0, true, true> : bimau_bwd_sweep1_kernel<T, DT, NT, 16, true, 0, false, true>;
                }
            }
        }
        hipFuncSetAttribute((const void*)kern, hipFuncAttributeMaxDynamicSharedMemorySize, (int)smem);
        hipLaunchKernelGGL(kern, dim3((unsigned)((jobs + waves - 1) / waves)), dim3(64 * waves), smem, st, p);
        EDGL_LAUNCH_CHECK();
    }
    {
        MlpP mp{p.hin, p.dz_ws, p.spans, p.pack, (long)p.B * p.H * p.T, p.B, p.T, p.E, p.dh_ws, p.wpart, p.dsc_part, jobs, 0};
        size_t smem_b = intensity_bwd_lds<T>(dh, p.E);
        const size_t slab_b = (size_t)4 * intensity_bwd_nreg<T>(DT) * 64 * sizeof(float);
        mp.slab_epi = slab_b <= std::max(smem_b, (size_t)52 * 1024);
        if (mp.slab_epi) smem_b = std::max(smem_b, slab_b);
        EDGL_REQUIRE(smem_b <= 160 * 1024, EDGL_ERR_SHAPE, "edgl_bimau_bwd: intensity kernel needs %zu B of LDS", smem_b);
        EDGL_REQUIRE((long)p.B * p.H * p.T < (1l << 31) - 16, EDGL_ERR_SHAPE, "edgl_bimau_bwd: B*H*T = %ld rows exceed the 32-bit row index", (long)p.B * p.H * p.T);
        auto kb = intensity_bwd_kernel<T, DT, 0>;
        hipFuncSetAttribute((const void*)kb, hipFuncAttributeMaxDynamicSharedMemorySize, (int)smem_b);
        hipLaunchKernelGGL(kb, dim3(KY_BLOCKS, KY_NY), dim3(256), smem_b, st, mp);
        EDGL_LAUNCH_CHECK();
    }
    {
        const size_t wave_bytes = (3 * (size_t)Tp * dh + (size_t)Tp * EP + (TR ? 0 : (size_t)dh * LDT)) * sizeof(T) + (size_t)Tp * sizeof(float);
        int waves = 4;
        while (waves > 1 && waves * wave_bytes > 80 * 1024) waves >>= 1;
        const size_t smem = waves * wave_bytes;
        EDGL_REQUIRE(smem <= 160 * 1024, EDGL_ERR_SHAPE, "edgl_bimau_bwd: needs %zu B of LDS", smem);
        p.waves = waves;
        constexpr bool SPEC = sizeof(T) == 2 && DT == 1;
        auto kern = p.E == 16 ? bimau_bwd_sweep2_kernel<T, DT, NT, 16> : bimau_bwd_sweep2_kernel<T, DT, NT, 0>;
        if constexpr (SPEC) {
            if (p.flags == 0) kern = p.E == 16 ? bimau_bwd_sweep2_kernel<T, DT, NT, 16, KY_NY, true, 0> : bimau_bwd_sweep2_kernel<T, DT, NT, 0, KY_NY, true, 0>;
            if constexpr (NT <= 8) {
                constexpr bool SKC = NT >= 2;
                const bool sk = SKC && p.flags == 0 && p.E == 16 && bimau_skip_enabled() && !p.noskip;
                if (p.flags == 0 && p.E == 16 && p.dbits && p.rate > 0.f) kern = sk ? bimau_bwd_sweep2_kernel<T, DT, NT, 16, KY_NY, true, 0, true, 1, 0, SKC> : bimau_bwd_sweep2_kernel<T, DT, NT, 16, KY_NY, true, 0, true>;
                else if (sk) kern = bimau_bwd_sweep2_kernel<T, DT, NT, 16, KY_NY, true, 0, false, 1, 0, SKC>;
            }
        }
        hipFuncSetAttribute((const void*)kern, hipFuncAttributeMaxDynamicSharedMemorySize, (int)smem);
        edgl_prof_begin(EDGL_KERNEL_BIMAU_BWD, st);
        hipLaunchKernelGGL(kern, dim3((unsigned)((jobs + waves - 1) / waves)), dim3(64 * waves), smem, st, p);
        edgl_prof_end(EDGL_KERNEL_BIMAU_BWD, st);
        edgl_prof_end(EDGL_KERNEL_BIMAU_BWD_ALL, st);
        EDGL_LAUNCH_CHECK();
    }
    const int JE = dh * p.E, NPAR = (dh + 3) * JE, NPARX = NPAR + EP;
    if (db1 == dW1 + (dh + 1) * JE && dw == db1 + JE && dscaling == dw + JE) {
        return edgl_reduce_rows(p.wpart, KY_BLOCKS, NPAR + p.E, NPARX, dW1, 0, st);
    }
    int rc = edgl_reduce_rows(p.wpart, KY_BLOCKS, (dh + 1) * JE, NPARX, dW1, 0, st);
    if (rc) return rc;
    rc = edgl_reduce_rows(p.wpart + (dh + 1) * JE, KY_BLOCKS, JE, NPARX, db1, 0, st);
    if (rc) return rc;
    rc = edgl_reduce_rows(p.wpart + (dh + 2) * JE, KY_BLOCKS, JE, NPARX, dw, 0, st);
    if (rc) return rc;
    rc = edgl_reduce_rows(p.wpart + NPAR, KY_BLOCKS, p.E, NPARX, dscaling, 0, st);
    if (rc) return rc;
    return EDGL_OK;
}

template <typename T, int DT>
int dispatch_nt(BwdP p, char* ws, float* dW1, float* db1, float* dw, float* dsc, hipStream_t st) {
    switch ((p.T + 15) / 16) {
        case 1: return launch_bwd<T, DT, 1>(p, ws, dW1, db1, dw, dsc, st);
        case 2: return launch_bwd<T, DT, 2>(p, ws, dW1, db1, dw, dsc, st);
        case 3: return launch_bwd<T, DT, 3>(p, ws, dW1, db1, dw, dsc, st);
        case 4: return launch_bwd<T, DT, 4>(p, ws, dW1, db1, dw, dsc, st);
        case 5: return launch_bwd<T, DT, 5>(p, ws, dW1, db1, dw, dsc, st);
        case 6: return launch_bwd<T, DT, 6>(p, ws, dW1, db1, dw, dsc, st);
        case 7: return launch_bwd<T, DT, 7>(p, ws, dW1, db1, dw, dsc, st);
        case 8: return launch_bwd<T, DT, 8>(p, ws, dW1, db1, dw, dsc, st);
        case 9: return launch_bwd<T, DT, 9>(p, ws, dW1, db1, dw, dsc, st);
        case 10: return launch_bwd<T, DT, 10>(p, ws, dW1, db1, dw, dsc, st);
        case 11: return launch_bwd<T, DT, 11>(p, ws, dW1, db1, dw, dsc, st);
        case 12: return launch_bwd<T, DT, 12>(p, ws, dW1, db1, dw, dsc, st);
        case 13: return launch_bwd<T, DT, 13>(p, ws, dW1, db1, dw, dsc, st);
    }
    edgl_set_error("edgl_bimau_bwd: T=%d not supported (T <= 208)", p.T);
    return EDGL_ERR_SHAPE;
}

}

extern "C" long edgl_bimau_bwd_workspace(int B, int T, int C, int H, int E, int dtype) {
    (void)dtype;
    if (H <= 0 || C % H) return -1;
    return (long)ws_layout(B, T, C, H, E).total;
}

extern "C" int edgl_bimau_mark_group(int C, int H, int dtype) {
    if (H <= 0 || C % H || (dtype != EDGL_F32 && dtype != EDGL_BF16)) return -1;
    const int dh = C / H;
    if (dh >= 64) return bimau::EP;
    for (int E = bimau::EP; E >= 1; --E) {
        const size_t b = dtype == EDGL_BF16 ? intensity_bwd_lds<bf16>(dh, E) : intensity_bwd_lds<float>(dh, E);
        if (b <= 160 * 1024) return E;
    }
    return -1;
}

extern "C" int edgl_bimau_bwd_db(const void* qkvt, const int64_t* ids, const float* spans, const uint8_t* marks,
                                 const void* pack, const void* d_out, const float* d_lam_ext, const float* lam,
                                 const void* saved, int B, int T, int C, int H, int E, float drop_rate,
                                 const uint64_t* rng_state, uint32_t stream_id, const uint32_t* dropbits, float qk_scale, void* d_qkvt,
                                 float* dW1, float* db1, float* dw, float* dscaling, void* workspace, int flags, int dtype, void* stream);
extern "C" int edgl_bimau_bwd(const void* qkvt, const int64_t* ids, const float* spans, const uint8_t* marks,
                              const void* pack, const void* d_out, const float* d_lam_ext, const float* lam,
                              const void* saved, int B, int T, int C, int H, int E, float drop_rate,
                              const uint64_t* rng_state, uint32_t stream_id, void* d_qkvt, float* dW1, float* db1,
                              float* dw, float* dscaling, void* workspace, int flags, int dtype, void* stream) {
    return edgl_bimau_bwd_db(qkvt, ids, spans, marks, pack, d_out, d_lam_ext, lam, saved, B, T, C, H, E, drop_rate, rng_state, stream_id,
                             nullptr, 0.f, d_qkvt, dW1, db1, dw, dscaling, workspace, flags, dtype, stream);
}
static int bimau_bwd_impl(const void* qkvt, const int64_t* ids, const float* spans, const uint8_t* marks,
                          const void* pack, const void* d_out, const float* d_lam_ext, const float* lam,
                          const void* saved, int B, int T, int C, int H, int E, float drop_rate,
                          const uint64_t* rng_state, uint32_t stream_id, const uint32_t* dropbits, float qk_scale, void* d_qkvt,
                          float* dW1, float* db1, float* dw, float* dscaling, void* workspace, const void* tpp_desc, int tpp_M,
                          const float* tpp_sums, float tpp_coef, float* tpp_part, const int32_t* order, int flags, int dtype, void* stream) {
    EDGL_REQUIRE(qkvt && ids && spans && marks && pack && d_out && lam && saved && d_qkvt && dW1 && db1 && dw && dscaling && workspace,
                 EDGL_ERR_NULL, "edgl_bimau_bwd: null pointer");
    EDGL_REQUIRE(B > 0 && T > 0 && H > 0 && C % H == 0 && E >= 1 && E <= bimau::EP, EDGL_ERR_SHAPE,
                 "edgl_bimau_bwd: bad shape B=%d T=%d C=%d H=%d E=%d", B, T, C, H, E);
    EDGL_REQUIRE(dtype == EDGL_F32 || dtype == EDGL_BF16, EDGL_ERR_DTYPE, "edgl_bimau_bwd: bad dtype %d", dtype);
    EDGL_REQUIRE(drop_rate == 0.f || rng_state, EDGL_ERR_NULL, "edgl_bimau_bwd: dropout without rng_state");
    EDGL_REQUIRE((double)B * H * T * T < 4294967296.0, EDGL_ERR_SHAPE, "edgl_bimau_bwd: H*B*T*T must be < 2^32");
    BwdP p{};
    p.qkvt = qkvt; p.ids = ids; p.spans = spans; p.marks = marks; p.pack = (const char*)pack; p.d_out = d_out;
    p.d_lam_ext = d_lam_ext; p.lam = lam;
    const bimau::SavedLayout sl = bimau::saved_layout(B, T, C, H, dtype == EDGL_BF16 ? 2 : 4);
    p.hin = (const char*)saved + sl.off_hin;
    p.z = reinterpret_cast<const float*>((const char*)saved + sl.off_z);
    p.B = B; p.T = T; p.C = C; p.H = H; p.E = E; p.rate = drop_rate; p.rng = rng_state;
    p.noskip = (flags & EDGL_MAU_NO_SKIP) ? 1 : 0; flags &= ~EDGL_MAU_NO_SKIP;
    p.stream_id = stream_id; p.d_qkvt = d_qkvt; p.flags = flags; p.dbits = dropbits; p.qk_scale = qk_scale;
    p.tpp_desc = tpp_desc; p.tpp_M = tpp_M; p.tpp_sums = tpp_sums; p.tpp_coef = tpp_coef; p.tpp_part = tpp_part; p.order = order;
    EDGL_REQUIRE(!tpp_desc || (dtype == EDGL_BF16 && C / H == 16 && E == 16 && T <= 128 && flags == 0 && tpp_part && tpp_M > 0 && !d_lam_ext),
                 EDGL_ERR_SHAPE, "edgl_bimau_bwd_tpp: the fused TPP form exists for bf16, head dim 16, 16 marks, T <= 128, BiMAU flags "
                 "(C/H=%d E=%d T=%d flags=%d)", C / H, E, T, flags);
    hipStream_t st = (hipStream_t)stream;
    const int dh = C / H;
    char* ws = (char*)workspace;
    if (dtype == EDGL_F32) {
        if (dh == 16) return dispatch_nt<float, 1>(p, ws, dW1, db1, dw, dscaling, st);
        if (dh == 32) return dispatch_nt<float, 2>(p, ws, dW1, db1, dw, dscaling, st);
    } else {
        if (dh == 16) return dispatch_nt<bf16, 1>(p, ws, dW1, db1, dw, dscaling, st);
        if (dh == 32) return dispatch_nt<bf16, 2>(p, ws, dW1, db1, dw, dscaling, st);
    }
    if (dh == 64 || dh == 128) return bimau::big_bwd(p, ws, dW1, db1, dw, dscaling, dtype, st);
    edgl_set_error("edgl_bimau_bwd: head dim %d not supported (16, 32, 64 or 128)", dh);
    return EDGL_ERR_SHAPE;
}
extern "C" int edgl_bimau_bwd_db(const void* qkvt, const int64_t* ids, const float* spans, const uint8_t* marks,
                                 const void* pack, const void* d_out, const float* d_lam_ext, const float* lam,
                                 const void* saved, int B, int T, int C, int H, int E, float drop_rate,
                                 const uint64_t* rng_state, uint32_t stream_id, const uint32_t* dropbits, float qk_scale, void* d_qkvt,
                                 float* dW1, float* db1, float* dw, float* dscaling, void* workspace, int flags, int dtype, void* stream) {
    return bimau_bwd_impl(qkvt, ids, spans, marks, pack, d_out, d_lam_ext, lam, saved, B, T, C, H, E, drop_rate, rng_state, stream_id,
                          dropbits, qk_scale, d_qkvt, dW1, db1, dw, dscaling, workspace, nullptr, 0, nullptr, 0.f, nullptr, nullptr, flags, dtype, stream);
}
extern "C" int edgl_bimau_bwd_tpp(const void* qkvt, const int64_t* ids, const float* spans, const uint8_t* marks,
                                  const void* pack, const void* d_out, const void* tpp_desc, int M, const float* tpp_sums, float coef,
                                  float* tpp_part, const float* lam, const void* saved, int B, int T, int C, int H, int E, float drop_rate,
                                  const uint64_t* rng_state, uint32_t stream_id, const uint32_t* dropbits, float qk_scale, void* d_qkvt,
                                  float* dW1, float* db1, float* dw, float* dscaling, void* workspace, int flags, int dtype, void* stream) {
    EDGL_REQUIRE(tpp_desc && tpp_part, EDGL_ERR_NULL, "edgl_bimau_bwd_tpp: null pointer");
    return bimau_bwd_impl(qkvt, ids, spans, marks, pack, d_out, nullptr, lam, saved, B, T, C, H, E, drop_rate, rng_state, stream_id,
                          dropbits, qk_scale, d_qkvt, dW1, db1, dw, dscaling, workspace, tpp_desc, M, tpp_sums, coef, tpp_part, nullptr, flags, dtype,
                          stream);
}
extern "C" int edgl_bimau_bwd_ord(const void* qkvt, const int64_t* ids, const float* spans, const uint8_t* marks, const void* pack,
                                  const void* d_out, const float* d_lam_ext, const void* tpp_desc, int M, const float* tpp_sums, float coef,
                                  float* tpp_part, const float* lam, const void* saved, int B, int T, int C, int H, int E, float drop_rate,
                                  const uint64_t* rng_state, uint32_t stream_id, const uint32_t* dropbits, float qk_scale, void* d_qkvt,
                                  float* dW1, float* db1, float* dw, float* dscaling, void* workspace, const int32_t* order, int flags,
                                  int dtype, void* stream) {
    EDGL_REQUIRE(!tpp_desc || tpp_part, EDGL_ERR_NULL, "edgl_bimau_bwd_ord: tpp_desc without tpp_part");
    return bimau_bwd_impl(qkvt, ids, spans, marks, pack, d_out, d_lam_ext, lam, saved, B, T, C, H, E, drop_rate, rng_state, stream_id,
                          dropbits, qk_scale, d_qkvt, dW1, db1, dw, dscaling, workspace, tpp_desc, M, tpp_sums, coef, tpp_part, order, flags,
                          dtype, stream);
}

#ifdef EDGL_PHASE_TIMING
extern "C" int edgl_debug_phase_cycles(unsigned long long* out16, int reset) {
    if (hipMemcpyFromSymbol(out16, HIP_SYMBOL(g_phase_cycles), 16 * sizeof(unsigned long long)) != hipSuccess) return -1;
    if (reset) {
// ... 7 lines not shown
```

### easydgl_amd/csrc/k_bimau_fwd.hip

```cpp
#include "bimau_fwd_impl.h"

namespace {
using namespace bimau;

template <typename T>
int dispatch_dt(FwdP p, hipStream_t st) {
    const int dh = p.C / p.H;
    if (dh == 16) return dispatch_nt<T, 1>(p, st);
    if (dh == 32) return dispatch_nt<T, 2>(p, st);
    edgl_set_error("edgl_bimau_fwd: head dim %d not supported (16, 32, 64 or 128)", dh);
    return EDGL_ERR_SHAPE;
}

}

extern "C" long edgl_bimau_pack_bytes(int C, int H, int E, int dtype) {
    const int dh = C / (H > 0 ? H : 1);
    return (long)(dtype == EDGL_BF16 ? bimau::pack_dims<bf16>(dh, E).bytes : bimau::pack_dims<float>(dh, E).bytes);
}

extern "C" long edgl_bimau_saved_bytes(int B, int T, int C, int H, int dtype) {
    if (H <= 0 || C % H) return -1;
    return (long)bimau::saved_layout(B, T, C, H, dtype == EDGL_BF16 ? 2 : 4).bytes;
}

extern "C" int edgl_bimau_pack(const float* W1, const float* b1, const float* w, const float* scaling, int C, int H,
                               int E, void* pack, int dtype, void* stream) {
    EDGL_REQUIRE(W1 && b1 && w && scaling && pack, EDGL_ERR_NULL, "edgl_bimau_pack: null pointer");
    EDGL_REQUIRE(H > 0 && C % H == 0 && E >= 1 && E <= bimau::EP, EDGL_ERR_SHAPE, "edgl_bimau_pack: bad C=%d H=%d E=%d", C, H, E);
    const int dh = C / H;
    hipStream_t st = (hipStream_t)stream;
    if (dtype == EDGL_F32) hipLaunchKernelGGL((bimau::pack_kernel<float>), dim3(16), dim3(256), 0, st, W1, b1, w, scaling, dh, E, (char*)pack);
    else if (dtype == EDGL_BF16) hipLaunchKernelGGL((bimau::pack_kernel<bf16>), dim3(16), dim3(256), 0, st, W1, b1, w, scaling, dh, E, (char*)pack);
    else { edgl_set_error("edgl_bimau_pack: bad dtype %d", dtype); return EDGL_ERR_DTYPE; }
    EDGL_LAUNCH_CHECK();
    return EDGL_OK;
}

extern "C" int edgl_bimau_fwd_zr(const void* qkvt, const void* resid, int ld_res, const int64_t* ids, const float* spans,
                                 const uint8_t* marks, const void* pack, int B, int T, int C, int H, int E,
                                 float drop_rate, const uint64_t* rng_state, uint32_t stream_id, void* out,
                                 float* lam_out, void* saved, float* zero_rows, int flags, int dtype, void* stream);
extern "C" int edgl_bimau_fwd_db(const void* qkvt, const void* resid, int ld_res, const int64_t* ids, const float* spans,
                                 const uint8_t* marks, const void* pack, int B, int T, int C, int H, int E,
                                 float drop_rate, const uint64_t* rng_state, uint32_t stream_id, const uint32_t* dropbits, float qk_scale,
                                 void* out, float* lam_out, void* saved, float* zero_rows, int flags, int dtype, void* stream);

extern "C" int edgl_bimau_fwd_ord(const void* qkvt, const void* resid, int ld_res, const int64_t* ids, const float* spans,
                                  const uint8_t* marks, const void* pack, int B, int T, int C, int H, int E,
                                  float drop_rate, const uint64_t* rng_state, uint32_t stream_id, const uint32_t* dropbits, float qk_scale,
                                  void* out, float* lam_out, void* saved, float* zero_rows, const int32_t* order, int flags, int dtype,
                                  void* stream);

extern "C" long edgl_bimau_dropbits_bytes(int B, int T, int H) {
    if (B <= 0 || T <= 0 || H <= 0) return -1;
    const int nt = (T + 15) / 16;
    return nt <= 8 ? (long)B * H * nt * 64 * (long)sizeof(uint32_t) : 0;
}
extern "C" int edgl_bimau_dropbits(int B, int T, int H, float drop_rate, const uint64_t* rng_state, uint32_t stream_id,
                                   uint32_t* bits, void* stream) {
    EDGL_REQUIRE(rng_state && bits, EDGL_ERR_NULL, "edgl_bimau_dropbits: null pointer");
    EDGL_REQUIRE(B > 0 && T > 0 && H > 0 && T <= 128, EDGL_ERR_SHAPE, "edgl_bimau_dropbits: bad shape B=%d T=%d H=%d (T <= 128)", B, T, H);
    EDGL_REQUIRE((double)B * H * T * T < 4294967296.0, EDGL_ERR_SHAPE, "edgl_bimau_dropbits: H*B*T*T must be < 2^32");
    const int nt = (T + 15) / 16;
    const long njobs = (long)B * H * nt;
    const dim3 grid((unsigned)((njobs + 3) / 4));
    hipStream_t st = (hipStream_t)stream;
    switch (nt) {
#define EDGL_DB_CASE(N) case N: hipLaunchKernelGGL((bimau::dropbits_kernel<N>), grid, dim3(256), 0, st, rng_state, stream_id, drop_rate, T, njobs, bits); break;
        EDGL_DB_CASE(1) EDGL_DB_CASE(2) EDGL_DB_CASE(3) EDGL_DB_CASE(4) EDGL_DB_CASE(5) EDGL_DB_CASE(6) EDGL_DB_CASE(7) EDGL_DB_CASE(8)
#undef EDGL_DB_CASE
    }
    EDGL_LAUNCH_CHECK();
    return EDGL_OK;
}
extern "C" int edgl_bimau_fwd(const void* qkvt, const void* resid, int ld_res, const int64_t* ids, const float* spans,
                              const uint8_t* marks, const void* pack, int B, int T, int C, int H, int E,
                              float drop_rate, const uint64_t* rng_state, uint32_t stream_id, void* out,
                              float* lam_out, void* saved, int flags, int dtype, void* stream) {
    return edgl_bimau_fwd_zr(qkvt, resid, ld_res, ids, spans, marks, pack, B, T, C, H, E, drop_rate, rng_state, stream_id, out, lam_out,
                             saved, nullptr, flags, dtype, stream);
}
extern "C" int edgl_bimau_fwd_zr(const void* qkvt, const void* resid, int ld_res, const int64_t* ids, const float* spans,
                                 const uint8_t* marks, const void* pack, int B, int T, int C, int H, int E,
                                 float drop_rate, const uint64_t* rng_state, uint32_t stream_id, void* out,
                                 float* lam_out, void* saved, float* zero_rows, int flags, int dtype, void* stream) {
    return edgl_bimau_fwd_db(qkvt, resid, ld_res, ids, spans, marks, pack, B, T, C, H, E, drop_rate, rng_state, stream_id, nullptr, 0.f, out,
                             lam_out, saved, zero_rows, flags, dtype, stream);
}
extern "C" int edgl_bimau_fwd_db(const void* qkvt, const void* resid, int ld_res, const int64_t* ids, const float* spans,
                                 const uint8_t* marks, const void* pack, int B, int T, int C, int H, int E,
                                 float drop_rate, const uint64_t* rng_state, uint32_t stream_id, const uint32_t* dropbits, float qk_scale,
                                 void* out, float* lam_out, void* saved, float* zero_rows, int flags, int dtype, void* stream) {
    return edgl_bimau_fwd_ord(qkvt, resid, ld_res, ids, spans, marks, pack, B, T, C, H, E, drop_rate, rng_state, stream_id, dropbits, qk_scale,
                              out, lam_out, saved, zero_rows, nullptr, flags, dtype, stream);
}

namespace {
__global__ __launch_bounds__(256) void job_tiles_kernel(const int64_t* ids, int B, int T, int32_t* nk) {
    const int lane = threadIdx.x & 63, b = blockIdx.x * 4 + (threadIdx.x >> 6);
    if (b >= B) return;
    const int NT = (T + 15) / 16, NR = (T + 63) / 64;
    int first = -1;
    for (int r0 = 0; r0 < NR; r0 += 4) {
        int64_t v[4];
#pragma unroll
        for (int j = 0; j < 4; ++j) v[j] = ids[(long)b * T + min(lane + 64 * (r0 + j), T - 1)];
#pragma unroll
        for (int j = 3; j >= 0; --j) {
            const int k = lane + 64 * (r0 + j);
            const uint64_t real = __ballot(k < T && v[j] != 0);
            if (real != 0ull && (first < 0 || 64 * (r0 + j) < first)) first = 64 * (r0 + j) + (int)__builtin_ctzll(real);
        }
        if (first >= 0) break;
    }
    if (lane == 0) nk[b] = first < 0 ? NT : NT - (first >> 4);
}
constexpr int ORD_THREADS = 256;
__global__ __launch_bounds__(ORD_THREADS) void job_rank_kernel(const int32_t* nk, int B, int32_t* order) {
    extern __shared__ __attribute__((aligned(16))) int nk_s[];
    for (int b = threadIdx.x; b < B; b += ORD_THREADS) nk_s[b] = nk[b];
    __syncthreads();
    for (int b = threadIdx.x; b < B; b += ORD_THREADS) {
        const int mine = nk_s[b];
        int rank = 0;
        int o = 0;
        for (; o + 32 <= B; o += 32) {
            int4 v[8];
#pragma unroll
            for (int j = 0; j < 8; ++j) v[j] = *reinterpret_cast<const int4*>(nk_s + o + 4 * j);
#pragma unroll
            for (int j = 0; j < 8; ++j) {
                const int oo = o + 4 * j;
                rank += (v[j].x > mine || (v[j].x == mine && oo < b)) ? 1 : 0;
                rank += (v[j].y > mine || (v[j].y == mine && oo + 1 < b)) ? 1 : 0;
                rank += (v[j].z > mine || (v[j].z == mine && oo + 2 < b)) ? 1 : 0;
                rank += (v[j].w > mine || (v[j].w == mine && oo + 3 < b)) ? 1 : 0;
            }
        }
        for (; o < B; ++o) {
            const int v = nk_s[o];
            rank += (v > mine || (v == mine && o < b)) ? 1 : 0;
        }
        order[rank] = b;
    }
}
}
extern "C" int edgl_bimau_job_order(const int64_t* ids, int B, int T, int32_t* order, void* stream) {
    EDGL_REQUIRE(ids && order, EDGL_ERR_NULL, "edgl_bimau_job_order: null pointer");
    EDGL_REQUIRE(B > 0 && T > 0 && B <= 16384, EDGL_ERR_SHAPE, "edgl_bimau_job_order: bad shape B=%d T=%d (B <= 16384)", B, T);
    hipLaunchKernelGGL(job_tiles_kernel, dim3((B + 3) / 4), dim3(256), 0, (hipStream_t)stream, ids, B, T, order + B);
    hipLaunchKernelGGL(job_rank_kernel, dim3(1), dim3(ORD_THREADS), (size_t)((B + 3) & ~3) * sizeof(int), (hipStream_t)stream, order + B, B, order);
    EDGL_LAUNCH_CHECK();
    return EDGL_OK;
}

extern "C" int edgl_bimau_fwd_ord(const void* qkvt, const void* resid, int ld_res, const int64_t* ids, const float* spans,
                                  const uint8_t* marks, const void* pack, int B, int T, int C, int H, int E,
                                  float drop_rate, const uint64_t* rng_state, uint32_t stream_id, const uint32_t* dropbits, float qk_scale,
                                  void* out, float* lam_out, void* saved, float* zero_rows, const int32_t* order, int flags, int dtype,
                                  void* stream) {
    EDGL_REQUIRE(qkvt && resid && ids && spans && marks && pack && out && lam_out, EDGL_ERR_NULL,
                 "edgl_bimau_fwd: null pointer");
    EDGL_REQUIRE(B > 0 && T > 0 && H > 0 && C % H == 0 && E >= 1 && E <= bimau::EP, EDGL_ERR_SHAPE,
                 "edgl_bimau_fwd: bad shape B=%d T=%d C=%d H=%d E=%d", B, T, C, H, E);
    EDGL_REQUIRE(drop_rate == 0.f || rng_state, EDGL_ERR_NULL, "edgl_bimau_fwd: dropout without rng_state");
    EDGL_REQUIRE(ld_res % 4 == 0, EDGL_ERR_SHAPE, "edgl_bimau_fwd: ld_res must be a multiple of 4");
    EDGL_REQUIRE((double)B * H * T * T < 4294967296.0, EDGL_ERR_SHAPE, "edgl_bimau_fwd: H*B*T*T must be < 2^32");
    FwdP p{qkvt, resid, ld_res, ids, spans, marks, (const char*)pack, B, T, C, H, E, drop_rate, rng_state, stream_id,
           out, lam_out, nullptr, nullptr, nullptr, 4, flags & ~EDGL_MAU_NO_SKIP, dropbits, qk_scale, order, (flags & EDGL_MAU_NO_SKIP) ? 1 : 0};
    flags &= ~EDGL_MAU_NO_SKIP;
    hipStream_t st = (hipStream_t)stream;
    if (C / H == 64 || C / H == 128) {
        if (zero_rows && hipMemsetAsync(zero_rows, 0, (size_t)H * B * T * E * sizeof(float), st) != hipSuccess) {
            edgl_set_error("edgl_bimau_fwd: memset failed");
            return EDGL_ERR_LAUNCH;
        }
    } else {
        p.zero_rows = zero_rows;
    }
    if (saved) {
        const bimau::SavedLayout sl = bimau::saved_layout(B, T, C, H, dtype == EDGL_BF16 ? 2 : 4);
        p.hin_out = (char*)saved + sl.off_hin;
        p.z_out = reinterpret_cast<float*>((char*)saved + sl.off_z);
    }
    EDGL_REQUIRE(dtype == EDGL_F32 || dtype == EDGL_BF16, EDGL_ERR_DTYPE, "edgl_bimau_fwd: bad dtype %d", dtype);
    edgl_prof_begin(EDGL_KERNEL_BIMAU_FWD, st);
    int rc;
    if (C / H == 64 || C / H == 128) rc = bimau::big_fwd(p, dtype, st);
    else if (dtype == EDGL_F32) rc = dispatch_dt<float>(p, st);
    else rc = dispatch_dt<bf16>(p, st);
    edgl_prof_end(EDGL_KERNEL_BIMAU_FWD, st);
    return rc;
}
```

### easydgl_amd/engine.py

```python
from __future__ import annotations

import ctypes
import os
from typing import Dict, Optional

import torch

from . import _lib, ops
from ._lib import check, lib
from .ops import _ptr, _stream

EPI_BIAS, EPI_GELU, EPI_SAVE_PRE, EPI_MUL_DGELU, EPI_ACCUM, EPI_OUT_F32 = 1, 2, 4, 8, 16, 32


class TrainEngine:
    _SIDE_STREAMS = {}

    def __init__(self, model, batch: int, use_graph: bool = True, process_group=None, fused_tail=None, flash_ce=None):
        env = os.environ.get
        self.sw_flash_ce = env("EDGL_FLASH_CE", "1") != "0"
        self.sw_tpp_fused = env("EDGL_TPP_FUSED", "1") != "0"
        self.sw_prep_in_encoder = env("EDGL_PREP_IN_ENCODER", "1") != "0"
        self.sw_bimau_order = env("EDGL_BIMAU_ORDER", "0") == "1"
        self.sw_ce_parts = env("EDGL_CE_PARTS", "1") != "0"
        self.sw_defer_loss = env("EDGL_DEFER_LOSS", "1") != "0"
        self.sw_adam_ex = env("EDGL_ADAM_EX", "1") != "0"
        self.sw_score_strip = env("EDGL_SCORE_STRIP", "1") != "0"
        self.m = model
        self.B = batch
        self.use_graph = use_graph
        self.group = process_group
        self.graph: Optional[torch.cuda.CUDAGraph] = None
        m = model
        dev = m._arena.device
        self.dev = dev
        self.dt = m.act_dtype
        self.code = ops._DT[self.dt]
        B, T, C, H, E, M, I = batch, m.seqslen, m.num_units, m.num_heads, m.num_events, m.masklen, m.num_items
        self.T, self.C, self.H, self.E, self.M, self.I = T, C, H, E, M, I
        self.pad = tuple(m.pad)
        self.c_true = int(m.width_true) if self.pad[0] else 0
        self.qk_scale = float(m.qk_scale)
        gmax = int(lib.edgl_bimau_mark_group(C, H, self.code))
        if gmax <= 0:
            raise _lib.EdglError(f"TrainEngine: head dim {C // H} / {self.dt} unsupported by the attention kernels")
        self.mgroups = [(e0, min(E, e0 + gmax)) for e0 in range(0, E, gmax)] if E > gmax else []
        self.R = B * M
        self.rows = B * T
        nb = len(m.layers)
        self.flash_ce = self.sw_flash_ce if flash_ce is None else bool(flash_ce)
        self.fused_tpp = (self.code == _lib.BF16 and C // H == 16 and E == 16 and not self.mgroups and M <= 256 and T <= 128
                          and m.ct_reg != 0.0 and self.flash_ce and nb > 0 and self.sw_tpp_fused)
        e = lambda *s, dtype=None: torch.empty(s, device=dev, dtype=dtype or self.dt)
        f32 = torch.float32
        self.ids = torch.zeros((B, T), device=dev, dtype=torch.int64)
        self.ts = torch.zeros((B, T), device=dev, dtype=f32)
        self.mpos = torch.zeros((B, M), device=dev, dtype=torch.int64)
        self.labels = torch.zeros((B, M), device=dev, dtype=torch.int64)
        self.x0 = e(B, T, 3 * C)
        self.spans = e(B, T, dtype=f32)
        self.marks = e(B, T, E, dtype=torch.uint8)
        self.blk = []
        for i in range(nb):
            d = dict(qkvt=e(B, T, 4 * C), att=e(B, T, C), lam=e(H * B, T, E, dtype=f32), ao=e(B, T, C), a1=e(B, T, C),
                     st1=e(B, 2, dtype=f32), pre_f=e(B, T, 2 * C), f=e(B, T, 2 * C), o=e(B, T, C), y=e(B, T, C),
                     st2=e(B, 2, dtype=f32),
                     pack=e(0 if self.mgroups else lib.edgl_bimau_pack_bytes(C, H, E, self.code), dtype=torch.uint8),
                     saved=e(0 if self.mgroups else lib.edgl_bimau_saved_bytes(B, T, C, H, self.code), dtype=torch.uint8),
                     dlam=None if self.fused_tpp else e(H * B, T, E, dtype=f32),
                     tpp_part=torch.zeros((B * H + 1, 2), device=dev, dtype=f32) if self.fused_tpp else None,
                     tpp=torch.zeros(max(lib.edgl_tpp_workspace(), lib.edgl_tpp_rows_workspace(B, H, M)), device=dev, dtype=f32))
            nb_bits = int(lib.edgl_bimau_dropbits_bytes(B, T, H)) if m.attention_probs_dropout_rate > 0 else 0
            d["dbits"] = e(nb_bits // 4, dtype=torch.int32) if nb_bits > 0 else None
            if self.mgroups:
                dh = C // H
                d["grp"] = []
                for (e0, e1) in self.mgroups:
                    eg = e1 - e0
                    d["grp"].append(dict(
                        marks=e(B, T, eg, dtype=torch.uint8), W1=e(dh + 1, dh * eg, dtype=f32), dW1=e(dh + 1, dh * eg, dtype=f32),
                        pack=e(lib.edgl_bimau_pack_bytes(C, H, eg, self.code), dtype=torch.uint8),
                        saved=e(lib.edgl_bimau_saved_bytes(B, T, C, H, self.code), dtype=torch.uint8),
                        lam=e(H * B, T, eg, dtype=f32), dlam=e(H * B, T, eg, dtype=f32),
                        out=e(B, T, C) if e0 else None, dqkvt=e(B, T, 4 * C) if e0 else None))
            self.blk.append(d)
        self.job_order = (torch.arange(2 * B, device=dev, dtype=torch.int32)
                          if (not self.mgroups and B <= 16384 and nb > 0 and self.sw_bimau_order) else None)
        self.tpp_desc = torch.zeros(int(lib.edgl_tpp_prep_bytes(B, T, M)), device=dev, dtype=torch.uint8) if self.fused_tpp else None
        self.zero_resid = torch.zeros((B, T, C), device=dev, dtype=self.dt) if self.mgroups else None
        self.pre_t, self.so, self.st3 = e(B, T, C), e(B, T, C), e(B, 2, dtype=f32)
        if m.ct_reg != 0.0 and (M > 256 or T > 1024):
            raise _lib.EdglError(f"TrainEngine: masklen {M} > 256 or T {T} > 1024 exceeds the fused TPP kernel (edgl_tpp_fwd_bwd_ex)")
        ok = bool(lib.edgl_tail_supported(T, C, self.code)) and M <= 256
        self.fused_tail = ok if fused_tail is None else (bool(fused_tail) and ok)
        self.tail_pack = [e(int(lib.edgl_tail_pack_elems(C))) for _ in range(nb)] if self.fused_tail else []
        if self.fused_tail:
            self.d_pre_t, self.d_o, self.d_pre_f, self.d_ao = e(B, T, C), e(B, T, C), e(B, T, 2 * C), e(B, T, C)
        self.ws_flash = e(int(lib.edgl_score_flash_workspace(self.R, C, I, I, self.code)), dtype=f32) if self.flash_ce else None
        self.hrows, self.hrows_c = e(self.R, C), e(self.R, C)
        self.hrows_c.zero_()
        self.labels_c = torch.zeros(self.R, device=dev, dtype=torch.int64)
        self.perm, self.inv = e(self.R, dtype=torch.int32), e(self.R, dtype=torch.int32)
        self.nvalid = torch.zeros(1, device=dev, dtype=torch.int32)
        self.lse, self.lab_logit, self.coef = e(self.R, dtype=f32), e(self.R, dtype=f32), e(self.R, dtype=f32)
        self.loss = e(1, dtype=f32)
        self.ce_nparts = int(lib.edgl_score_ce_nparts(self.R, C)) if (self.flash_ce and self.sw_ce_parts) else 0
        self.ce_part = torch.zeros(self.ce_nparts + 1, device=dev, dtype=f32) if self.ce_nparts > 0 else None
        self.loss_aux, self.loss_tpp = torch.zeros(1, device=dev, dtype=f32), torch.zeros(1, device=dev, dtype=f32)
        self.ws_l2 = e(1024, dtype=f32)
        self.l2_nparts = int(lib.edgl_adam_l2_parts(m._arena.numel()))
        self.l2_parts = [torch.zeros(self.l2_nparts, device=dev, dtype=f32) for _ in range(2)] \
            if (m.l2_reg != 0.0 and not use_graph) else None
        self._l2p_cur, self._l2p_ready = 0, False
        key = (dev.type, dev.index if dev.index is not None else torch.cuda.current_device())
        if key not in TrainEngine._SIDE_STREAMS:
            TrainEngine._SIDE_STREAMS[key] = (torch.cuda.Stream(device=dev), torch.cuda.Stream(device=dev))
        self.side, self.side2 = TrainEngine._SIDE_STREAMS[key]
        self._pending_loss = None
        self.accumulate_loss = False
        self.loss_sum = torch.zeros(1, device=dev, dtype=torch.float64)
        self._pending_label = None
        self._lazy_loss, self._side_has_grads, self._loss_unjoined = False, False, False
        self._label_fused = False
        self.mau_flags = _lib.MAU_NO_SKIP
        self.adam_ex = (not use_graph) and self.sw_adam_ex
        self._rng_alt, self._adam_alt = torch.zeros_like(m._rng_state), torch.zeros_like(m._adam_state)
        self._slabs = None
        self._slab_info = None
        if self.adam_ex and self.flash_ce:
            info = (ctypes.c_long * 4)()
            check(lib.edgl_score_flash_slab_info(self.R, C, I, I, self.code, info), "edgl_score_flash_slab_info")
            self._slab_info = (int(info[0]), int(info[1]), int(info[2]))
        self._ar_events = None
        self.sync_loss = True
        self._deferred_loss = None
        self._alt = None
        if self.ce_part is not None:
            self._alt = dict(ce_part=torch.zeros_like(self.ce_part), loss_aux=torch.zeros_like(self.loss_aux),
                             tpp_desc=torch.zeros_like(self.tpp_desc) if self.tpp_desc is not None else None,
                             tpp_part=[torch.zeros_like(b["tpp_part"]) if b["tpp_part"] is not None else None for b in self.blk])
        self.counts = torch.zeros(2, device=dev, dtype=torch.int32)
        self._dp = False
        self.d_rows = e(self.R, C)
        self.G1, self.G2, self.G3, self.G4 = e(B, T, C), e(B, T, C), e(B, T, C), e(B, T, C)
        self.G2c, self.G4c, self.G3c = e(B, T, 2 * C), e(B, T, 4 * C), e(B, T, 3 * C)
        wsz = [2 * self.R * lib.edgl_score_chunks(self.R, I),
               lib.edgl_score_bwd_workspace(self.R, C, I, I, self.code),
               lib.edgl_encode_bwd_workspace(B, T, C), B * 2 * C, 1024]
        for (kf, n) in ((3 * C, 4 * C), (C, 4 * C), (C, C), (C, 2 * C), (2 * C, C)):
            wsz.append(lib.edgl_gemm_dw_workspace(self.rows, kf, n, self.code))
        self.ws = e(max(wsz), dtype=f32)
        self._ws_list, self._ws_i = [], 0
        segs = []
        params = dict(m.named_parameters())
        for n in m.l2_param_names():
            segs += [m._offsets[n], m._offsets[n] + params[n].numel()]
        self.l2_seg = torch.tensor(segs, device=dev, dtype=torch.int64)
        self.nseg = len(segs) // 2

    def _gemm(self, A, Bm, Cm, M, N, K, lda, ldb, ldc, b_kc, bias=None, aux=None, flags=0):
        check(lib.edgl_gemm(_ptr(A), _ptr(Bm), _ptr(Cm), M, N, K, lda, ldb, ldc, 1, int(b_kc), _ptr(bias), _ptr(aux), flags,
                            1, None, self.code, _stream()), "edgl_gemm")

    def _dense_fwd(self, x, dense_kernel, dense_bias, out, K, N, gelu=False, pre=None):
        flags = EPI_BIAS | ((EPI_GELU | EPI_SAVE_PRE) if gelu else 0)
        self._gemm(x, self.m.compute(dense_kernel), out, self.rows, N, K, K, N, N, False, bias=dense_bias, aux=pre, flags=flags)

    def _dense_dx(self, dz, kernel, out, K_in, N, flags=0, aux=None):
        self._gemm(dz, self.m.compute(kernel), out, self.rows, K_in, N, N, N, K_in, True, aux=aux, flags=flags)

    def _ws(self, n, dtype=torch.float32):
        i = self._ws_i
        self._ws_i += 1
        if i == len(self._ws_list):
            self._ws_list.append(torch.empty(max(int(n), 1), device=self.m._arena.device, dtype=dtype))
        w = self._ws_list[i]
        if w.numel() < n or w.dtype != dtype:
# ... 54 lines not shown
        if self._pending_loss is not None:
            self._pending_loss(st)
            self._pending_loss = None
            if self.accumulate_loss:
                self.loss_sum.add_(self.loss)
        if self._lazy_loss and not self._side_has_grads:
            self._loss_unjoined = True
        else:
            torch.cuda.current_stream().wait_stream(self.side)
            self._loss_unjoined = False

    def _l2_term(self, from_parts, sst):
        m = self.m
        if m.l2_reg != 0.0 and from_parts:
            check(lib.edgl_l2_from_parts(_ptr(self.l2_parts[self._l2p_cur]), self.l2_nparts, float(m.l2_reg), _ptr(self.loss_aux), 0,
                                         sst), "edgl_l2_from_parts")
        elif m.l2_reg != 0.0:
            check(lib.edgl_l2_loss(_ptr(m._arena), _ptr(self.l2_seg), self.nseg, float(m.l2_reg), _ptr(self.loss_aux), 0,
                                   _ptr(self.ws_l2), sst), "edgl_l2_loss")

    def _issue_side_chain(self, main, l2_from_parts):
        m = self.m
        B, T, C, H, E, M, R = self.B, self.T, self.C, self.H, self.E, self.M, self.R
        code, ad = self.code, m.attention_probs_dropout_rate
        side, side2 = self.side, self.side2
        sst = side.cuda_stream
        if self._loss_unjoined and self.ce_part is None:
            main.wait_stream(side)
            self._loss_unjoined = False
        side.wait_stream(main)
        if self._deferred_loss is not None:
            a = self._alt
            self.ce_part, a["ce_part"] = a["ce_part"], self.ce_part
            self.loss_aux, a["loss_aux"] = a["loss_aux"], self.loss_aux
            self.tpp_desc, a["tpp_desc"] = a["tpp_desc"], self.tpp_desc
            for j, bj in enumerate(self.blk):
                bj["tpp_part"], a["tpp_part"][j] = a["tpp_part"][j], bj["tpp_part"]
        if not self.sw_prep_in_encoder:
            side2.wait_stream(main)
            if self._loss_unjoined:
                side2.wait_stream(side)
            with torch.cuda.stream(side2):
                check(lib.edgl_compact_scan_labels(_ptr(self.labels), R, _ptr(self.perm), _ptr(self.inv), _ptr(self.nvalid),
                                                   _ptr(self.labels_c), side2.cuda_stream), "edgl_compact_scan_labels")
                if self.fused_tpp:
                    check(lib.edgl_tpp_prep(_ptr(self.mpos), _ptr(self.labels), _ptr(self.ts), _ptr(m.mark_lookup_table), B, T, E, M,
                                            _ptr(self.tpp_desc), side2.cuda_stream), "edgl_tpp_prep")
        with torch.cuda.stream(side):
            if self._fold and m._table_grad_zero != id(self):
                tab = m.item_embs.lookup_table
                tab.grad.zero_()
                m.output_bias.grad.zero_()
            if self.job_order is not None:
                check(lib.edgl_bimau_job_order(_ptr(self.ids), B, T, _ptr(self.job_order), sst), "edgl_bimau_job_order")
            for i, (blk, b) in enumerate(zip(m.layers, self.blk)):
                att = blk.attention
                if m.ct_reg != 0.0 and not self._dp and not self.fused_tpp:
                    check(lib.edgl_tpp_norm(_ptr(self.labels), _ptr(m.mark_lookup_table), B, M, E, _ptr(b["tpp"]), sst),
                          "edgl_tpp_norm")
                if self.fused_tail:
                    check(lib.edgl_tail_pack(_ptr(m.compute(blk.att_out.kernel)), _ptr(m.compute(blk.inter.kernel)),
                                             _ptr(m.compute(blk.out.kernel)), _ptr(m.compute(m.transform.kernel)), C,
                                             _ptr(self.tail_pack[i]), sst), "edgl_tail_pack")
                if self.mgroups:
                    dh = C // H
                    for (e0, e1), gb in zip(self.mgroups, b["grp"]):
                        gb["W1"].copy_(att.st_kernel[:, e0 * dh:e1 * dh])
                        check(lib.edgl_bimau_pack(_ptr(gb["W1"]), _ptr(att.st_bias[e0 * dh:e1 * dh]), _ptr(att.weight[e0:e1]),
                                                  _ptr(att.scaling[e0:e1]), C, H, e1 - e0, _ptr(gb["pack"]), code, sst), "edgl_bimau_pack")
                else:
                    check(lib.edgl_bimau_pack(_ptr(att.st_kernel), _ptr(att.st_bias), _ptr(att.weight), _ptr(att.scaling), C, H, E,
                                              _ptr(b["pack"]), code, sst), "edgl_bimau_pack")
                if b["dbits"] is not None:
                    check(lib.edgl_bimau_dropbits(B, T, H, float(ad), _ptr(m._rng_state), 10 + 4 * i, _ptr(b["dbits"]), sst),
                          "edgl_bimau_dropbits")
            l2_behind = l2_from_parts and bool(self.blk)
            if not l2_behind:
                self._l2_term(l2_from_parts, sst)
            if not self.sw_prep_in_encoder:
                side.wait_stream(side2)
            ev_pack = side.record_event()
            if self._deferred_loss is not None:
                self._deferred_loss(sst)
                self._deferred_loss = None
            if l2_behind:
                self._l2_term(l2_from_parts, sst)
        return ev_pack

    def _issue_forward(self, main, ev_pack, drop, tab_c, st):
        m = self.m
        B, T, C, H, E, M, I, R = self.B, self.T, self.C, self.H, self.E, self.M, self.I, self.R
        code = self.code
        hd, ad = m.hidden_dropout_rate, m.attention_probs_dropout_rate
        d0 = drop(hd, 1)
        if self.sw_prep_in_encoder:
            check(lib.edgl_encode_fwd_prep(_ptr(self.ids), _ptr(self.ts), _ptr(tab_c), _ptr(m.pcoding.pembs.lookup_table),
                                           _ptr(m.mark_embs.lookup_table), _ptr(m.mark_lookup_table), _ptr(m.tcoding.scale), B, T, C,
                                           E, I, int(m.mask), float(m.time_scale), float(d0.rate), d0.ptr(), d0.stream_id,
                                           _ptr(self.x0), _ptr(self.spans), _ptr(self.marks), self.pad[0], self.pad[1],
                                           _ptr(self.labels), M, _ptr(self.perm), _ptr(self.inv), _ptr(self.nvalid), _ptr(self.labels_c),
                                           _ptr(self.mpos), _ptr(self.tpp_desc) if self.fused_tpp else None, code, st),
                  "edgl_encode_fwd_prep")
        else:
            check(lib.edgl_encode_fwd_ct(_ptr(self.ids), _ptr(self.ts), _ptr(tab_c), _ptr(m.pcoding.pembs.lookup_table),
                                         _ptr(m.mark_embs.lookup_table), _ptr(m.mark_lookup_table), _ptr(m.tcoding.scale), B, T, C,
                                         E, I, int(m.mask), float(m.time_scale), float(d0.rate), d0.ptr(), d0.stream_id,
                                         _ptr(self.x0), _ptr(self.spans), _ptr(self.marks), self.pad[0], self.pad[1], code, st),
                  "edgl_encode_fwd")
        x, cin = self.x0, 3 * C
        for i, (blk, b) in enumerate(zip(m.layers, self.blk)):
            att = blk.attention
            self._dense_fwd(x, att.dense_kernel, att.dense_bias, b["qkvt"], cin, 4 * C)
            if i == 0:
                main.wait_event(ev_pack)
            da = drop(ad, 10 + 4 * i)
            if self.mgroups:
                self._attention_fwd_groups(b, x, cin, da, st)
            else:
                check(lib.edgl_bimau_fwd_ord(_ptr(b["qkvt"]), x.data_ptr(), cin, _ptr(self.ids), _ptr(self.spans), _ptr(self.marks),
                                             _ptr(b["pack"]), B, T, C, H, E, float(da.rate), da.ptr(), da.stream_id, _ptr(b["dbits"]),
                                             self.qk_scale, _ptr(b["att"]), _ptr(b["lam"]), _ptr(b["saved"]),
                                             _ptr(b["dlam"]) if (m.ct_reg != 0.0 and not self.fused_tpp) else None, _ptr(self.job_order),
                                             self.mau_flags, code, st), "edgl_bimau_fwd_ord")
            if m.ct_reg != 0.0 and not self.fused_tpp:
                check(lib.edgl_tpp_fwd_bwd_rows(_ptr(b["lam"]), _ptr(self.mpos), _ptr(self.labels), _ptr(self.ts),
                                                _ptr(m.mark_lookup_table), B, T, H, E, M, float(m.ct_reg / H), _ptr(b["tpp"]),
# ... 406 lines not shown
```

### include/easydgl_hip.h

```cpp
#ifndef EASYDGL_HIP_H
#define EASYDGL_HIP_H

#include <stdint.h>

#ifdef __cplusplus
extern "C" {
#endif

typedef enum { EDGL_F32 = 0, EDGL_BF16 = 1 } edgl_dtype;

enum {
    EDGL_OK = 0,
    EDGL_ERR_SHAPE = -1,
    EDGL_ERR_DTYPE = -2,
    EDGL_ERR_LAUNCH = -3,
    EDGL_ERR_NULL = -4,
    EDGL_ERR_WORKSPACE = -5
};

enum {
    EDGL_EPI_BIAS = 1,
    EDGL_EPI_GELU = 2,
    EDGL_EPI_SAVE_PRE = 4,
    EDGL_EPI_MUL_DGELU = 8,
// ... 28 lines not shown
int edgl_encode_bwd_add(const int64_t* ids, const uint8_t* marks, const void* dx0, const void* add1, const void* add2, int B,
                        int T, int C, int E, int I, float drop_rate, const uint64_t* rng_state, uint32_t stream_id,
                        float* d_item, float* d_pos, float* d_mark_emb, float* workspace, int dtype, void* stream);
int edgl_encode_fwd_ct(const int64_t* ids, const float* ts, const void* item_tab, const float* pos_tab, const float* mark_emb,
                       const uint8_t* mark_table, const float* tscale, int B, int T, int C, int E, int I, int64_t mask_id,
                       float time_scale, float drop_rate, const uint64_t* rng_state, uint32_t stream_id, void* x0, float* spans,
                       uint8_t* marks, int dh_pad, int dh_true, int dtype, void* stream);
int edgl_encode_fwd_prep(const int64_t* ids, const float* ts, const void* item_tab, const float* pos_tab, const float* mark_emb,
                         const uint8_t* mark_table, const float* tscale, int B, int T, int C, int E, int I, int64_t mask_id,
                         float time_scale, float drop_rate, const uint64_t* rng_state, uint32_t stream_id, void* x0, float* spans,
                         uint8_t* marks, int dh_pad, int dh_true, const int64_t* labels, int M, int32_t* perm, int32_t* inv,
                         int32_t* nvalid, int64_t* labels_c, const int64_t* masked_pos, void* tpp_desc, int dtype, void* stream);
int edgl_encode_bwd_add_ct(const int64_t* ids, const uint8_t* marks, const void* dx0, const void* add1, const void* add2, int B,
                           int T, int C, int E, int I, float drop_rate, const uint64_t* rng_state, uint32_t stream_id,
                           float* d_item, float* d_pos, float* d_mark_emb, float* workspace, int c_true, int dtype, void* stream);
int edgl_encode_bwd_label_fused(int C, int dtype);
int edgl_encode_bwd_add_label(const int64_t* ids, const uint8_t* marks, const void* dx0, const void* add1, const void* add2, int B,
                              int T, int C, int E, int I, float drop_rate, const uint64_t* rng_state, uint32_t stream_id,
                              float* d_item, float* d_pos, float* d_mark_emb, float* workspace, int c_true, const void* lab_rows,
                              const int64_t* lab_ids, const float* lab_coef, const int32_t* lab_nvalid, int lab_R, float* d_bias,
                              int dtype, void* stream);

int edgl_embed_pos_fwd(const int64_t* ids, const float* ts, const void* item_tab, const float* pos_tab,
                       const uint8_t* mark_table, int B, int T, int C, int E, float time_scale, float drop_rate,
                       const uint64_t* rng_state, uint32_t stream_id, void* x0, float* spans, uint8_t* marks,
                       int dtype, void* stream);
int edgl_embed_pos_bwd(const int64_t* ids, const void* dx0, int B, int T, int C, int I, float drop_rate,
                       const uint64_t* rng_state, uint32_t stream_id, float* d_item, float* d_pos, int dtype,
                       void* stream);
int edgl_embed_pos_fwd_ct(const int64_t* ids, const float* ts, const void* item_tab, const float* pos_tab,
                          const uint8_t* mark_table, int B, int T, int C, int E, float time_scale, float drop_rate,
                          const uint64_t* rng_state, uint32_t stream_id, void* x0, float* spans, uint8_t* marks,
                          int c_true, int dtype, void* stream);
int edgl_embed_pos_bwd_ct(const int64_t* ids, const void* dx0, int B, int T, int C, int I, float drop_rate,
                          const uint64_t* rng_state, uint32_t stream_id, float* d_item, float* d_pos, int c_true,
                          int dtype, void* stream);

int edgl_gemm(const void* A, const void* Bm, void* Cm, int M, int N, int K, int lda, int ldb, int ldc,
              int a_kc, int b_kc, const float* bias, void* aux, int epi_flags, int splitk, float* workspace,
              int dtype, void* stream);

long edgl_gemm_dw_workspace(int R, int Kf, int N, int dtype);
int edgl_gemm_dw(const void* X, const void* dY, float* dW, float* dbias, int R, int Kf, int N, int ldx, int ldy,
                 int accumulate, float* workspace, int dtype, void* stream);
int edgl_gemm_dw_defer(int on, void* stream);

int edgl_colsum(const void* X, int M, int N, int ld, float* out, int accumulate, float* workspace,
                int x_f32, int dtype, void* stream);

#define EDGL_MAU_CAUSAL 1
#define EDGL_MAU_NO_DIAG 2
#define EDGL_MAU_DIAG_ZERO 4
#define EDGL_MAU_NO_SKIP 8
long edgl_bimau_pack_bytes(int C, int H, int E, int dtype);
long edgl_bimau_saved_bytes(int B, int T, int C, int H, int dtype);
int edgl_bimau_mark_group(int C, int H, int dtype);
int edgl_bimau_pack(const float* W1, const float* b1, const float* w, const float* scaling, int C, int H, int E,
                    void* pack, int dtype, void* stream);
int edgl_bimau_fwd(const void* qkvt, const void* resid, int ld_res, const int64_t* ids, const float* spans,
                   const uint8_t* marks, const void* pack, int B, int T, int C, int H, int E, float drop_rate,
                   const uint64_t* rng_state, uint32_t stream_id, void* out, float* lam_out, void* saved,
                   int flags, int dtype, void* stream);
int edgl_bimau_fwd_zr(const void* qkvt, const void* resid, int ld_res, const int64_t* ids, const float* spans,
                      const uint8_t* marks, const void* pack, int B, int T, int C, int H, int E, float drop_rate,
                      const uint64_t* rng_state, uint32_t stream_id, void* out, float* lam_out, void* saved,
                      float* zero_rows, int flags, int dtype, void* stream);

long edgl_bimau_dropbits_bytes(int B, int T, int H);
int edgl_bimau_dropbits(int B, int T, int H, float drop_rate, const uint64_t* rng_state, uint32_t stream_id, uint32_t* bits,
                        void* stream);
int edgl_bimau_fwd_db(const void* qkvt, const void* resid, int ld_res, const int64_t* ids, const float* spans,
                      const uint8_t* marks, const void* pack, int B, int T, int C, int H, int E, float drop_rate,
                      const uint64_t* rng_state, uint32_t stream_id, const uint32_t* dropbits, float qk_scale, void* out,
                      float* lam_out, void* saved, float* zero_rows, int flags, int dtype, void* stream);

int edgl_bimau_job_order(const int64_t* ids, int B, int T, int32_t* order, void* stream);
int edgl_bimau_fwd_ord(const void* qkvt, const void* resid, int ld_res, const int64_t* ids, const float* spans,
                       const uint8_t* marks, const void* pack, int B, int T, int C, int H, int E, float drop_rate,
                       const uint64_t* rng_state, uint32_t stream_id, const uint32_t* dropbits, float qk_scale, void* out,
                       float* lam_out, void* saved, float* zero_rows, const int32_t* order, int flags, int dtype, void* stream);
int edgl_bimau_bwd_ord(const void* qkvt, const int64_t* ids, const float* spans, const uint8_t* marks, const void* pack,
                       const void* d_out, const float* d_lam_ext, const void* tpp_desc, int M, const float* tpp_sums, float coef,
                       float* tpp_part, const float* lam, const void* saved, int B, int T, int C, int H, int E, float drop_rate,
                       const uint64_t* rng_state, uint32_t stream_id, const uint32_t* dropbits, float qk_scale, void* d_qkvt,
                       float* dW1, float* db1, float* dw, float* dscaling, void* workspace, const int32_t* order, int flags,
                       int dtype, void* stream);

long edgl_bimau_bwd_workspace(int B, int T, int C, int H, int E, int dtype);
int edgl_bimau_bwd(const void* qkvt, const int64_t* ids, const float* spans, const uint8_t* marks,
                   const void* pack, const void* d_out, const float* d_lam_ext, const float* lam,
                   const void* saved, int B, int T, int C, int H, int E, float drop_rate,
                   const uint64_t* rng_state, uint32_t stream_id, void* d_qkvt, float* dW1, float* db1,
                   float* dw, float* dscaling, void* workspace, int flags, int dtype, void* stream);
int edgl_bimau_bwd_db(const void* qkvt, const int64_t* ids, const float* spans, const uint8_t* marks,
                      const void* pack, const void* d_out, const float* d_lam_ext, const float* lam,
                      const void* saved, int B, int T, int C, int H, int E, float drop_rate,
                      const uint64_t* rng_state, uint32_t stream_id, const uint32_t* dropbits, float qk_scale, void* d_qkvt,
                      float* dW1, float* db1, float* dw, float* dscaling, void* workspace, int flags, int dtype, void* stream);

int edgl_add_layernorm_fwd(const void* x, const void* resid, int ld_res, const float* gamma,
                           const float* beta, int B, int T, int C, float drop_rate,
                           const uint64_t* rng_state, uint32_t stream_id, const int64_t* gather_pos,
                           int Mg, void* y, float* stats, int dtype, void* stream);

int edgl_add_layernorm_bwd(const void* x, const void* resid, int ld_res, const float* gamma,
                           const float* stats, const void* dy, int B, int T, int C, float drop_rate,
                           const uint64_t* rng_state, uint32_t stream_id, const int64_t* gather_pos,
                           int Mg, const int32_t* dy_rowmap, void* dsum, void* dx_drop, float* dgamma,
                           float* dbeta, float* workspace, int dtype, void* stream);
int edgl_add_layernorm_bwd_act(const void* x, const void* resid, int ld_res, const float* gamma,
                               const float* stats, const void* dy, int B, int T, int C, float drop_rate,
                               const uint64_t* rng_state, uint32_t stream_id, const int64_t* gather_pos,
                               int Mg, const int32_t* dy_rowmap, const void* act_pre, void* dsum, void* dx_drop,
                               float* dgamma, float* dbeta, float* workspace, int dtype, void* stream);
int edgl_add_layernorm_fwd_ct(const void* x, const void* resid, int ld_res, const float* gamma, const float* beta, int B, int T,
                              int C, float drop_rate, const uint64_t* rng_state, uint32_t stream_id, const int64_t* gather_pos,
                              int Mg, void* y, float* stats, int dh_pad, int dh_true, int dtype, void* stream);
int edgl_add_layernorm_bwd_act_ct(const void* x, const void* resid, int ld_res, const float* gamma, const float* stats,
                                  const void* dy, int B, int T, int C, float drop_rate, const uint64_t* rng_state,
                                  uint32_t stream_id, const int64_t* gather_pos, int Mg, const int32_t* dy_rowmap,
                                  const void* act_pre, void* dsum, void* dx_drop, float* dgamma, float* dbeta, float* workspace,
                                  int dh_pad, int dh_true, int dtype, void* stream);

int edgl_score_chunks(int R, int n_items);
int edgl_compact_rows(const void* rows, const int64_t* labels, int R, int C, int32_t* perm, int32_t* inv,
                      int32_t* nvalid, void* rows_c, int64_t* labels_c, int dtype, void* stream);
int edgl_compact_scan(const int64_t* labels, int R, int32_t* perm, int32_t* inv, int32_t* nvalid, void* stream);
int edgl_compact_scan_labels(const int64_t* labels, int R, int32_t* perm, int32_t* inv, int32_t* nvalid, int64_t* labels_c,
                             void* stream);
// ... 215 lines not shown
```

Baseline: 663,500.

## Compact non-padded keys into leading tiles for bidirectional MAU attention

Adds a compact-keys mode for the bidirectional bf16 MAU attention. Valid (non-padding) keys are permuted into the leading tiles during staging, so forward and backward iterate only over the occupied key tiles. Results are scattered back through a stored original-index map, and the diagonal is located through a per-query slot. A matching dropout-bits kernel is added, and job ordering by compact tile count is now enabled by default. This removes wasted work on padding scattered anywhere in the sequence, at the cost of extra permutation bookkeeping, more LDS per wave, and index-dependent dropout masks.

```diff
diff --git a/easydgl_amd/_lib.py b/easydgl_amd/_lib.py
--- a/easydgl_amd/_lib.py
+++ b/easydgl_amd/_lib.py
@@ -13,6 +13,7 @@
 EPI_BIAS, EPI_GELU, EPI_SAVE_PRE, EPI_MUL_DGELU, EPI_ACCUM, EPI_OUT_F32, EPI_RELU = 1, 2, 4, 8, 16, 32, 64
 MAU_CAUSAL, MAU_NO_DIAG, MAU_DIAG_ZERO = 1, 2, 4
 MAU_NO_SKIP = 8
+MAU_COMPACT = 16
 TATTN_CAUSAL = 1
 
 P, I, F, L, U32, I64 = c_void_p, c_int, c_float, c_long, c_uint32, c_int64
@@ -53,6 +54,9 @@
     "edgl_bimau_fwd_db": (I, [P, P, I, P, P, P, P, I, I, I, I, I, F, P, U32, P, F, P, P, P, P, I, I, P]),
     "edgl_bimau_bwd_db": (I, [P, P, P, P, P, P, P, P, P, I, I, I, I, I, F, P, U32, P, F, P, P, P, P, P, P, I, I, P]),
     "edgl_bimau_job_order": (I, [P, I, I, P, P]),
+    "edgl_bimau_job_order_compact": (I, [P, I, I, P, P]),
+    "edgl_bimau_dropbits_ids": (I, [P, I, I, I, F, P, U32, P, P]),
+    "edgl_bimau_compact_supported": (I, [I, I, I, I, I, I]),
     "edgl_bimau_fwd_ord": (I, [P, P, I, P, P, P, P, I, I, I, I, I, F, P, U32, P, F, P, P, P, P, P, I, I, P]),
     "edgl_bimau_bwd_ord": (I, [P, P, P, P, P, P, P, P, I, P, F, P, P, P, I, I, I, I, I, F, P, U32, P, F, P, P, P, P, P, P, P, I, I, P]),
     "edgl_bimau_bwd_workspace": (L, [I, I, I, I, I, I]),
diff --git a/easydgl_amd/csrc/bimau_bwd_impl.h b/easydgl_amd/csrc/bimau_bwd_impl.h
--- a/easydgl_amd/csrc/bimau_bwd_impl.h
+++ b/easydgl_amd/csrc/bimau_bwd_impl.h
@@ -49,6 +49,7 @@
     int waves;
     int flags;
     int noskip;
+    int compact;
     const uint32_t* dbits;
     float qk_scale;
     const void* tpp_desc; int tpp_M; const float* tpp_sums; float tpp_coef;
@@ -63,7 +64,7 @@
     else *reinterpret_cast<uint2*>(dst) = *reinterpret_cast<uint2*>(&f);
 }
 
-template <typename T, int DT, int NT, int EC, bool PREF = true, int FL = -1, bool DB = false, bool TP = false, bool SK = false>
+template <typename T, int DT, int NT, int EC, bool PREF = true, int FL = -1, bool DB = false, bool TP = false, bool SK = false, bool CK = false>
 __global__ __launch_bounds__(256) void bimau_bwd_sweep1_kernel(BwdP p) {
     constexpr int dh = 16 * DT, Tp = 16 * NT, LDT = Tp + 4;
     extern __shared__ __attribute__((aligned(16))) char smem[];
@@ -84,7 +85,7 @@
 
     constexpr bool TR = sizeof(T) == 2;
     constexpr size_t EXTRA = TR ? 0 : (size_t)EP * LDT;
-    constexpr size_t MASK_ELEMS = (size_t)Tp * sizeof(float) / sizeof(T);
+    constexpr size_t MASK_ELEMS = (CK ? 2 : 1) * (size_t)Tp * sizeof(float) / sizeof(T);
     constexpr size_t WAVE_ELEMS = 2 * (size_t)Tp * dh + (size_t)Tp * EP + EXTRA + MASK_ELEMS;
     T* Ks = reinterpret_cast<T*>(smem) + (size_t)wave * WAVE_ELEMS;
     T* Vs = Ks + Tp * dh;
@@ -94,10 +95,14 @@
     const T* dout = reinterpret_cast<const T*>(p.d_out) + (long)b * p.T * p.C;
     T* dqkvt = reinterpret_cast<T*>(p.d_qkvt) + (long)b * p.T * 4 * p.C;
     const int ldq = 4 * p.C;
-    const KeyMask<NT> km = stage_wave<T, DT, NT, EC>(
+    float* madd_s = reinterpret_cast<float*>(Ks + WAVE_ELEMS - MASK_ELEMS);
+    int16_t* korig = reinterpret_cast<int16_t*>(madd_s + Tp);
+    const int16_t* dslot = korig + Tp;
+    (void)dslot;
+    const KeyMask<NT> km = stage_wave<T, DT, NT, EC, CK>(
         qkvt + p.C + head * dh, Ks, nullptr, static_cast<const T*>(nullptr), static_cast<T*>(nullptr), static_cast<T*>(nullptr),
         qkvt + 2 * p.C + head * dh, Vs, nullptr, ldq, p.marks + (long)b * p.T * E, E, Ms, TR ? nullptr : MTs,
-        p.ids + (long)b * p.T, reinterpret_cast<float*>(Ks + WAVE_ELEMS - MASK_ELEMS), p.T, LDT, lane);
+        p.ids + (long)b * p.T, madd_s, p.T, LDT, lane, korig);
     __builtin_amdgcn_fence(__ATOMIC_RELEASE, "wavefront");
     __builtin_amdgcn_wave_barrier();
 
@@ -176,8 +181,8 @@
     };
     PH_DECL
     auto run = [&](auto nk_c) {
-    constexpr int NK = decltype(nk_c)::value, K0 = NT - NK;
-    const KeyMask<NK> kmk = keymask_tail<NK, NT>(km);
+    constexpr int NK = decltype(nk_c)::value, K0 = CK ? 0 : NT - NK;
+    const KeyMask<NK> kmk = keymask_walk<NK, NT, CK>(km);
     float dsc_acc[4] = {0.f, 0.f, 0.f, 0.f}, tp_a = 0.f, tp_b = 0.f;
     f32x4 dVa[DT][NK];
 #pragma unroll
@@ -244,6 +249,11 @@
         float rowdot = 0.f;
         f32x4 dlamT = zero4;
         const uint32_t dbase = (uint32_t)((bp * p.T + q) * p.T);
+        int dkt = -1, dr = 0;
+        if constexpr (CK) {
+            const int dsl = dslot[q];
+            dkt = dsl >> 4; dr = dsl & 15;
+        }
 #pragma unroll
         for (int kt = 0; kt < NK; ++kt) {
             const f32x4 gacc = mma16(frag_ld<T>(Ms + ((K0 + kt) * 16 + l15) * EP + g4s), lf, zero4);
@@ -255,7 +265,7 @@
             const bool dtile = K0 + kt == qt && (FL == 0 || !(p.flags & MAU_NO_DIAG));
             if constexpr (FL == 0) {
 #pragma unroll
-                for (int r = 0; r < 4; ++r) gv[r] = (dtile && g4 + r == l15) ? 1.0f : gacc[r];
+                for (int r = 0; r < 4; ++r) gv[r] = (CK ? (kt == dkt && g4 + r == dr) : (dtile && g4 + r == l15)) ? 1.0f : gacc[r];
             } else if (dtile) {
 #pragma unroll
                 for (int r = 0; r < 4; ++r) gv[r] = (g4 + r == l15) ? ((p.flags & MAU_DIAG_ZERO) ? 0.0f : 1.0f) : gacc[r];
@@ -274,7 +284,7 @@
             }
             if constexpr (FL == 0) {
 #pragma unroll
-                for (int r = 0; r < 4; ++r) dg[r] = (dtile && g4 + r == l15) ? 0.f : dg[r];
+                for (int r = 0; r < 4; ++r) dg[r] = (CK ? (kt == dkt && g4 + r == dr) : (dtile && g4 + r == l15)) ? 0.f : dg[r];
             } else if (dtile) {
 #pragma unroll
                 for (int r = 0; r < 4; ++r) dg[r] = (g4 + r == l15) ? 0.f : dg[r];
@@ -319,12 +329,15 @@
     if (l15 == 0) *reinterpret_cast<float4*>(p.dsc_part + job * EP + g4) = make_float4(dsc_acc[0], dsc_acc[1], dsc_acc[2], dsc_acc[3]);
 #pragma unroll
     for (int kt = 0; kt < NT; ++kt) {
-        const int k = kt * 16 + l15;
+        const int k = CK ? (int)korig[kt * 16 + l15] : kt * 16 + l15;
         if (k < p.T) {
 #pragma unroll
             for (int ut = 0; ut < DT; ++ut) {
                 T* dst = dqkvt + (long)k * ldq + 2 * p.C + head * dh + ut * 16 + g4;
-                if constexpr (K0 > 0) {
+                if constexpr (CK) {
+                    if (kt < NK) st_frag<T>(dst, dVa[ut][kt < NK ? kt : 0]);
+                    else st_frag<T>(dst, zero4);
+                } else if constexpr (K0 > 0) {
                     if (kt < K0) st_frag<T>(dst, zero4);
                     else st_frag<T>(dst, dVa[ut][kt < K0 ? 0 : kt - K0]);
                 } else {
@@ -334,8 +347,8 @@
         }
     }
     };
-    if constexpr (SK) {
-        static_assert(FL == 0 && sizeof(T) == 2, "the key-tile skip exists for the bidirectional bf16 form");
+    if constexpr (SK || CK) {
+        static_assert(FL == 0 && sizeof(T) == 2 && !(SK && CK), "the key-tile skip and the compact keys exist for the bidirectional bf16 form");
         dispatch_nk<NT>(NT - km.kt0, run);
     } else {
         run(std::integral_constant<int, NT>{});
@@ -344,7 +357,7 @@
     PH_FLUSH(0);
 }
 
-template <typename T, int DT, int NT, int EC, int NYP = KY_NY, bool PREF = true, int FL = -1, bool DB = false, int US = 1, int SL = 0, bool SK = false>
+template <typename T, int DT, int NT, int EC, int NYP = KY_NY, bool PREF = true, int FL = -1, bool DB = false, int US = 1, int SL = 0, bool SK = false, bool CK = false>
 __global__ __launch_bounds__(256) void bimau_bwd_sweep2_kernel(BwdP p) {
     constexpr int dh = 16 * DT, Tp = 16 * NT, LDT = Tp + 4;
     static_assert(DT % US == 0 && SL < US, "channel slices");
@@ -367,7 +380,7 @@
 
     constexpr bool TR = sizeof(T) == 2;
     constexpr size_t EXTRA = TR ? 0 : (size_t)dh * LDT;
-    constexpr size_t MASK_ELEMS = (size_t)Tp * sizeof(float) / sizeof(T);
+    constexpr size_t MASK_ELEMS = (CK ? 2 : 1) * (size_t)Tp * sizeof(float) / sizeof(T);
     constexpr size_t WAVE_ELEMS = 3 * (size_t)Tp * dh + (size_t)Tp * EP + EXTRA + MASK_ELEMS;
     T* Ks = reinterpret_cast<T*>(smem) + (size_t)wave * WAVE_ELEMS;
     T* Ts = Ks + Tp * dh;
@@ -379,10 +392,14 @@
     const T* hin = reinterpret_cast<const T*>(p.hin);
     T* dqkvt = reinterpret_cast<T*>(p.d_qkvt) + (long)b * p.T * 4 * p.C;
     const int ldq = 4 * p.C;
-    const KeyMask<NT> km = stage_wave<T, DT, NT, EC>(
+    float* madd_s = reinterpret_cast<float*>(Ks + WAVE_ELEMS - MASK_ELEMS);
+    int16_t* korig = reinterpret_cast<int16_t*>(madd_s + Tp);
+    const int16_t* dslot = korig + Tp;
+    (void)dslot;
+    const KeyMask<NT> km = stage_wave<T, DT, NT, EC, CK>(
         qkvt + p.C + head * dh, Ks, TR ? nullptr : KTs, qkvt + 3 * p.C + head * dh, Ts, static_cast<T*>(nullptr),
         qkvt + 2 * p.C + head * dh, Vs, static_cast<T*>(nullptr), ldq, p.marks + (long)b * p.T * E, E, Ms, static_cast<T*>(nullptr),
-        p.ids + (long)b * p.T, reinterpret_cast<float*>(Ks + WAVE_ELEMS - MASK_ELEMS), p.T, LDT, lane);
+        p.ids + (long)b * p.T, madd_s, p.T, LDT, lane, korig);
     __builtin_amdgcn_fence(__ATOMIC_RELEASE, "wavefront");
     __builtin_amdgcn_wave_barrier();
 
@@ -429,8 +446,8 @@
     const unsigned long long clk_m0 = __builtin_readcyclecounter(), clk_r0 = wall_clock64();
 #endif
     auto run = [&](auto nk_c) {
-    constexpr int NK = decltype(nk_c)::value, K0 = NT - NK;
-    const KeyMask<NK> kmk = keymask_tail<NK, NT>(km);
+    constexpr int NK = decltype(nk_c)::value, K0 = CK ? 0 : NT - NK;
+    const KeyMask<NK> kmk = keymask_walk<NK, NT, CK>(km);
     f32x4 dKa[DTS][NK], dTa[DTS][NK];
 #pragma unroll
     for (int u = 0; u < DTS; ++u)
@@ -512,6 +529,11 @@
 #pragma unroll
         for (int ut = 0; ut < DTS; ++ut) dQ[ut] = zero4;
         const uint32_t dbase = (uint32_t)((bp * p.T + q) * p.T);
+        int dkt = -1, dr = 0;
+        if constexpr (CK) {
+            const int dsl = dslot[q];
+            dkt = dsl >> 4; dr = dsl & 15;
+        }
 #pragma unroll
         for (int kt = 0; kt < NK; ++kt) {
             const f32x4 gacc = mma16(frag_ld<T>(Ms + ((K0 + kt) * 16 + l15) * EP + g4s), lf, zero4);
@@ -523,7 +545,7 @@
             if constexpr (FL == 0) {
                 const bool dtile = K0 + kt == qt;
 #pragma unroll
-                for (int r = 0; r < 4; ++r) gv[r] = (dtile && g4 + r == l15) ? dk.scale : gacc[r];
+                for (int r = 0; r < 4; ++r) gv[r] = (CK ? (kt == dkt && g4 + r == dr) : (dtile && g4 + r == l15)) ? dk.scale : gacc[r];
             } else if (kt == qt && !(p.flags & MAU_NO_DIAG)) {
 #pragma unroll
                 for (int r = 0; r < 4; ++r) gv[r] = (g4 + r == l15) ? ((p.flags & MAU_DIAG_ZERO) ? 0.0f : dk.scale) : gacc[r];
@@ -578,16 +600,16 @@
     flush_pending();
 #pragma unroll
     for (int kt = 0; kt < NT; ++kt) {
-        const int k = kt * 16 + l15;
+        const int k = CK ? (int)korig[kt * 16 + l15] : kt * 16 + l15;
         if (k < p.T) {
 #pragma unroll
             for (int ut = 0; ut < DTS; ++ut) {
                 T* row = dqkvt + (long)k * ldq + head * dh + (U0 + ut) * 16 + g4;
-                if (kt < K0) {
+                if (CK ? kt >= NK : kt < K0) {
                     st_frag<T>(row + p.C, zero4);
                     st_frag<T>(row + 3 * p.C, zero4);
                 } else {
-                    const int kk = kt < K0 ? 0 : kt - K0;
+                    const int kk = CK ? (kt < NK ? kt : 0) : (kt < K0 ? 0 : kt - K0);
                     if constexpr (FL == 0) {
 #pragma unroll
                         for (int r = 0; r < 4; ++r) dKa[ut][kk][r] *= cz;
@@ -599,8 +621,8 @@
         }
     }
     };
-    if constexpr (SK) {
-        static_assert(FL == 0 && sizeof(T) == 2, "the key-tile skip exists for the bidirectional bf16 form");
+    if constexpr (SK || CK) {
+        static_assert(FL == 0 && sizeof(T) == 2 && !(SK && CK), "the key-tile skip and the compact keys exist for the bidirectional bf16 form");
         dispatch_nk<NT>(NT - km.kt0, run);
     } else {
         run(std::integral_constant<int, NT>{});
diff --git a/easydgl_amd/csrc/bimau_common.h b/easydgl_amd/csrc/bimau_common.h
--- a/easydgl_amd/csrc/bimau_common.h
+++ b/easydgl_amd/csrc/bimau_common.h
@@ -134,6 +134,11 @@
     constexpr int K0 = NT - NK;
     return KeyMask<NK>{km.madd + K0 * 16, km.pad >> (K0 * 4), 0};
 }
+template <int NK, int NT, bool CK>
+__device__ __forceinline__ KeyMask<NK> keymask_walk(const KeyMask<NT>& km) {
+    if constexpr (CK) return KeyMask<NK>{km.madd, 0ull, 0};
+    else return keymask_tail<NK, NT>(km);
+}
 inline bool bimau_skip_enabled() {
     return edgl_env_on("EDGL_BIMAU_SKIP");
 }
@@ -280,6 +285,26 @@
             for (int r = 0; r < 4; ++r) s[kt][r] *= inv;
     }
 }
+
+template <int NR>
+__device__ __forceinline__ int rank_below(const uint64_t (&w)[NR], int k) {
+    int r = 0;
+#pragma unroll
+    for (int i = 0; i < NR; ++i) {
+        const int s = k - 64 * i;
+        const uint64_t m = s >= 64 ? ~0ull : (s <= 0 ? 0ull : ((1ull << s) - 1ull));
+        r += __popcll(w[i] & m);
+    }
+    return r;
+}
+template <int NR>
+__device__ __forceinline__ bool bit_at(const uint64_t (&w)[NR], int k) {
+    uint64_t v = w[0];
+#pragma unroll
+    for (int i = 1; i < NR; ++i) v = (k >> 6) == i ? w[i] : v;
+    return ((v >> (k & 63)) & 1ull) != 0ull;
+}
+__host__ __device__ __forceinline__ int compact_tiles(int n, int NT) { return n > 0 ? (n + 15) / 16 : NT; }
 
 template <int I>
 __device__ __forceinline__ float keep_bit_c(uint32_t kb, float x) {
@@ -317,6 +342,56 @@
         w |= (drop_quad_keep<2>(dk, hw) ? 1u : 0u) << (kt * 4 + 2);
         w |= (drop_quad_keep<3>(dk, hw) ? 1u : 0u) << (kt * 4 + 3);
     }
+    bits[job * 64 + lane] = w;
+}
+
+template <int NT>
+__global__ __launch_bounds__(256) void dropbits_compact_kernel(const uint64_t* rng, uint32_t stream_id, float rate, const int64_t* ids, int B, int T,
+                                                               long njobs, uint32_t* bits) {
+    static_assert(NT <= 8, "one 32-bit word per lane and query tile");
+    constexpr int Tp = 16 * NT, NR = (Tp + 63) / 64;
+    __shared__ int16_t korig_s[4][Tp];
+    const int lane = threadIdx.x & 63, wave = threadIdx.x >> 6;
+    const long job = (long)blockIdx.x * 4 + wave;
+    if (job >= njobs) return;
+    const long bp = job / NT;
+    const int b = (int)(bp % B);
+    const int qt = (int)(job % NT), q = qt * 16 + (lane & 15), g4 = (lane >> 4) * 4;
+    uint64_t eff[NR];
+    bool in[NR];
+    int n = 0;
+#pragma unroll
+    for (int i = 0; i < NR; ++i) {
+        const int k = lane + 64 * i;
+        in[i] = k < T;
+        eff[i] = __ballot(in[i] && ids[(long)b * T + min(k, T - 1)] != 0);
+        n += (int)__popcll(eff[i]);
+    }
+    if (n == 0) {
+#pragma unroll
+        for (int i = 0; i < NR; ++i) { eff[i] = __ballot(in[i]); n += (int)__popcll(eff[i]); }
+    }
+#pragma unroll
+    for (int i = 0; i < NR; ++i) {
+        const int k = lane + 64 * i;
+        if (k < Tp) {
+            const int rk = rank_below<NR>(eff, k);
+            korig_s[wave][bit_at<NR>(eff, k) ? rk : n + k - rk] = (int16_t)k;
+        }
+    }
+    __builtin_amdgcn_fence(__ATOMIC_RELEASE, "wavefront");
+    __builtin_amdgcn_wave_barrier();
+    const DropKey dk = make_dropkey(rng, stream_id, rate);
+    const uint32_t dbase = (uint32_t)((bp * T + q) * T);
+    uint32_t w = 0u;
+#pragma unroll
+    for (int kt = 0; kt < NT; ++kt)
+#pragma unroll
+        for (int r = 0; r < 4; ++r) {
+            const uint32_t ko = (uint32_t)korig_s[wave][kt * 16 + g4 + r];
+            const uint64_t hw = drop_hash_quad(dk, dbase + (ko & ~3u));
+            w |= (((uint32_t)(hw >> (16 * (ko & 3u))) & 0xffffu) >= dk.t16 ? 1u : 0u) << (kt * 4 + r);
+        }
     bits[job * 64 + lane] = w;
 }
 
@@ -517,6 +592,11 @@
 #pragma unroll
         for (int j = 0; j < NI; ++j) { uint2& u = *reinterpret_cast<uint2*>(&f[j]); asm volatile("" : "+v"(u.x), "+v"(u.y)); }
     }
+    __device__ __forceinline__ void put(int j, T* rowmajor, int drow, bool zero, int lane) {
+        const int u4 = ((lane + 64 * j) % cpr) * 4;
+        if (zero) f[j] = frag_zero<T>();
+        *reinterpret_cast<uint2*>(rowmajor + drow * dh + swz_col<dh>(drow, u4)) = *reinterpret_cast<uint2*>(&f[j]);
+    }
     __device__ __forceinline__ void store(T* rowmajor, T* transposed, int LDT, int Tlen, int lane) {
 #pragma unroll
         for (int j = 0; j < NI; ++j) {
@@ -533,12 +613,87 @@
 template <typename T, int DT, int NT, int EC>
 constexpr bool stage_merged() { return sizeof(T) == 2 && NT * DT <= 8 && EC == 16; }
 
-template <typename T, int DT, int NT, int EC>
+template <typename T, int DT, int NT, int EC, bool CK = false>
 __device__ __forceinline__ KeyMask<NT> stage_wave(const T* k_src, T* k_rm, T* k_tr, const T* t_src, T* t_rm, T* t_tr,
                                                   const T* v_src, T* v_rm, T* v_tr, int ld, const uint8_t* marks_row, int E,
                                                   T* m_rm, T* m_tr, const int64_t* ids_row, float* lds_madd, int Tlen, int LDT,
-                                                  int lane) {
-    if constexpr (stage_merged<T, DT, NT, EC>()) {
+                                                  int lane, int16_t* kmap = nullptr) {
+    if constexpr (CK) {
+        static_assert(stage_merged<T, DT, NT, EC>(), "compact keys: merged staging only");
+        constexpr int Tp = 16 * NT, NR = (Tp + 63) / 64, cpr = 4 * DT, NI = NT * DT;
+        RowStage<T, DT, NT> sk, st, sv;
+        uint4 mk[NR];
+        int64_t id[NR];
+        sk.load(k_src, ld, Tlen, lane);
+        if (t_src) st.load(t_src, ld, Tlen, lane);
+        if (v_src) sv.load(v_src, ld, Tlen, lane);
+#pragma unroll
+        for (int i = 0; i < NR; ++i) {
+            const int k = min(lane + 64 * i, Tlen - 1);
+            if (marks_row) mk[i] = *reinterpret_cast<const uint4*>(marks_row + (long)k * 16);
+            id[i] = ids_row[k];
+        }
+        sk.pin();
+        if (t_src) st.pin();
+        if (v_src) sv.pin();
+#pragma unroll
+        for (int i = 0; i < NR; ++i) {
+            if (marks_row) asm volatile("" : "+v"(mk[i].x), "+v"(mk[i].y), "+v"(mk[i].z), "+v"(mk[i].w));
+            asm volatile("" : "+v"(id[i]));
+        }
+        uint64_t eff[NR];
+        int n = 0;
+#pragma unroll
+        for (int i = 0; i < NR; ++i) {
+            eff[i] = __ballot(lane + 64 * i < Tlen && id[i] != 0);
+            n += (int)__popcll(eff[i]);
+        }
+        const bool none = n == 0;
+        int ntot = n;
+        if (none) {
+            ntot = 0;
+#pragma unroll
+            for (int i = 0; i < NR; ++i) {
+                eff[i] = __ballot(lane + 64 * i < Tlen);
+                ntot += (int)__popcll(eff[i]);
+            }
+        }
+#pragma unroll
+        for (int j = 0; j < NI; ++j) {
+            const int k = (lane + 64 * j) / cpr, rk = rank_below<NR>(eff, k);
+            const bool e = bit_at<NR>(eff, k);
+            const int d = e ? rk : ntot + k - rk;
+            sk.put(j, k_rm, d, !e, lane);
+            if (t_src) st.put(j, t_rm, d, !e, lane);
+            if (v_src) sv.put(j, v_rm, d, !e, lane);
+        }
+#pragma unroll
+        for (int i = 0; i < NR; ++i) {
+            const int k = lane + 64 * i;
+            if (k < Tp) {
+                const int rk = rank_below<NR>(eff, k);
+                const bool e = bit_at<NR>(eff, k);
+                const int d = e ? rk : ntot + k - rk;
+                if (marks_row && m_rm) {
+                    const uint32_t w[4] = {mk[i].x, mk[i].y, mk[i].z, mk[i].w};
+                    T vals[16];
+#pragma unroll
+                    for (int x = 0; x < 16; ++x) vals[x] = from_f32<T>(e ? (float)((w[x / 4] >> (8 * (x % 4))) & 0xffu) : 0.f);
+#pragma unroll
+                    for (int j = 0; j < 2; ++j)
+                        reinterpret_cast<uint4*>(m_rm + d * EP)[j ^ ((d >> 3) & 1)] = reinterpret_cast<const uint4*>(vals)[j];
+                }
+                lds_madd[d] = e ? (none ? -4294967296.0f : 0.f) : -INFINITY;
+                kmap[d] = (int16_t)k;
+                kmap[Tp + k] = (int16_t)(e ? rk : -1);
+            }
+        }
+        KeyMask<NT> km;
+        km.pad = 0ull;
+        km.madd = lds_madd;
+        km.kt0 = NT - compact_tiles(n, NT);
+        return km;
+    } else if constexpr (stage_merged<T, DT, NT, EC>()) {
         constexpr int Tp = 16 * NT, NR = (Tp + 63) / 64;
         RowStage<T, DT, NT> sk, st, sv;
         uint4 mk[NR];
diff --git a/easydgl_amd/csrc/bimau_fwd_impl.h b/easydgl_amd/csrc/bimau_fwd_impl.h
--- a/easydgl_amd/csrc/bimau_fwd_impl.h
+++ b/easydgl_amd/csrc/bimau_fwd_impl.h
@@ -22,16 +22,17 @@
     float qk_scale;
     const int32_t* order;
     int noskip;
+    int compact;
 };
 
-template <typename T, int DT, int NT, int PHASE>
+template <typename T, int DT, int NT, int PHASE, bool CK = false>
 __host__ __device__ constexpr size_t fwd_wave_bytes() {
     constexpr size_t dh = 16 * DT, Tp = 16 * NT, LDT = Tp + 4;
     constexpr size_t kv = sizeof(T) == 2 ? Tp * dh : dh * LDT;
-    return (Tp * dh + (PHASE != 2 ? kv : 0) + (PHASE != 1 ? kv : 0) + (PHASE != 1 ? Tp * EP : 0)) * sizeof(T) + Tp * sizeof(float);
-}
-
-template <typename T, int DT, int NT, int EC, int PHASE = 0, bool DB = false, bool SK = false>
+    return (Tp * dh + (PHASE != 2 ? kv : 0) + (PHASE != 1 ? kv : 0) + (PHASE != 1 ? Tp * EP : 0)) * sizeof(T) + (CK ? 2 : 1) * Tp * sizeof(float);
+}
+
+template <typename T, int DT, int NT, int EC, int PHASE = 0, bool DB = false, bool SK = false, bool CK = false>
 __global__ __launch_bounds__(256, (sizeof(T) == 2 && DT == 1 && EC == 16 && PHASE == 0) ? FWD_WAVES : 1) void bimau_fwd_kernel(FwdP p) {
     constexpr int dh = 16 * DT, Tp = 16 * NT, LDT = Tp + 4;
     extern __shared__ __attribute__((aligned(16))) char smem[];
@@ -58,21 +59,25 @@
 
     constexpr bool TR = sizeof(T) == 2;
     constexpr size_t KV_ELEMS = TR ? (size_t)Tp * dh : (size_t)dh * LDT;
-    constexpr size_t MASK_ELEMS = (size_t)Tp * sizeof(float) / sizeof(T);
+    constexpr size_t MASK_ELEMS = (CK ? 2 : 1) * (size_t)Tp * sizeof(float) / sizeof(T);
     constexpr size_t WAVE_ELEMS = (size_t)Tp * dh + (HAS_T ? KV_ELEMS : 0) + (HAS_V ? KV_ELEMS : 0) + (HAS_M ? (size_t)Tp * EP : 0) + MASK_ELEMS;
-    static_assert(WAVE_ELEMS * sizeof(T) == fwd_wave_bytes<T, DT, NT, PHASE>(), "host / device LDS layouts differ");
+    static_assert(WAVE_ELEMS * sizeof(T) == fwd_wave_bytes<T, DT, NT, PHASE, CK>(), "host / device LDS layouts differ");
     T* Ks = reinterpret_cast<T*>(smem + pack_bytes) + (size_t)wave * WAVE_ELEMS;
     T* Ts = Ks + Tp * dh;
     T* Vs = Ts + (HAS_T ? KV_ELEMS : 0);
     T* Ms = Vs + (HAS_V ? KV_ELEMS : 0);
     const T* qkvt = reinterpret_cast<const T*>(p.qkvt) + (long)b * p.T * 4 * p.C;
     const int ldq = 4 * p.C;
-    const KeyMask<NT> km = stage_wave<T, DT, NT, EC>(
+    float* madd_s = reinterpret_cast<float*>(Ms + (HAS_M ? Tp * EP : 0));
+    int16_t* kmap = reinterpret_cast<int16_t*>(madd_s + Tp);
+    const int16_t* dslot = kmap + Tp;
+    (void)dslot;
+    const KeyMask<NT> km = stage_wave<T, DT, NT, EC, CK>(
         qkvt + p.C + head * dh, Ks, nullptr,
         HAS_T ? qkvt + 3 * p.C + head * dh : nullptr, TR ? Ts : nullptr, TR ? nullptr : Ts,
         HAS_V ? qkvt + 2 * p.C + head * dh : nullptr, TR ? Vs : nullptr, TR ? nullptr : Vs, ldq,
         HAS_M ? p.marks + (long)b * p.T * E : nullptr, E, Ms, nullptr, p.ids + (long)b * p.T,
-        reinterpret_cast<float*>(Ms + (HAS_M ? Tp * EP : 0)), p.T, LDT, lane);
+        madd_s, p.T, LDT, lane, kmap);
     __builtin_amdgcn_fence(__ATOMIC_RELEASE, "wavefront");
     __builtin_amdgcn_wave_barrier();
 
@@ -103,8 +108,8 @@
         return o;
     };
     auto run = [&](auto nk_c) {
-    constexpr int NK = decltype(nk_c)::value, K0 = NT - NK;
-    const KeyMask<NK> kmk = keymask_tail<NK, NT>(km);
+    constexpr int NK = decltype(nk_c)::value, K0 = CK ? 0 : NT - NK;
+    const KeyMask<NK> kmk = keymask_walk<NK, NT, CK>(km);
     QOps qcur = load_q(0);
     touch_regs(qcur);
     Frag4<T> pend_o[DT];
@@ -140,7 +145,7 @@
         }
         float pinv = 1.0f;
         if constexpr (TR) {
-            if constexpr (K0 == 0) {
+            if constexpr (K0 == 0 && !CK) {
                 if (p.flags & MAU_CAUSAL) pinv = masked_softmax_impl<NT, true, false, false>(s, kmk, cscale, lane, q);
                 else pinv = masked_softmax_impl<NT, false, false, false>(s, kmk, cscale, lane, q);
             } else {
@@ -288,6 +293,11 @@
         const uint32_t dbase = (uint32_t)((bp * p.T + q) * p.T);
         const bool set_diag = !(p.flags & MAU_NO_DIAG);
         const float dval = (p.flags & MAU_DIAG_ZERO) ? 0.0f : gfac;
+        int dkt = -1, dr = 0;
+        if constexpr (CK) {
+            const int dsl = set_diag ? (int)dslot[q] : -1;
+            dkt = dsl >> 4; dr = dsl & 15;
+        }
         auto modulate = [&](auto drop_on) {
 #pragma unroll
             for (int kt = 0; kt < NK; ++kt) {
@@ -295,7 +305,8 @@
                 const bool dtile = set_diag && K0 + kt == qt;
 #pragma unroll
                 for (int r = 0; r < 4; ++r) {
-                    gacc[r] = (dtile && g4 + r == l15) ? dval : gacc[r];
+                    const bool isd = CK ? (kt == dkt && g4 + r == dr) : (dtile && g4 + r == l15);
+                    gacc[r] = isd ? dval : gacc[r];
                     s[kt][r] = gacc[r] * s[kt][r];
                 }
                 if constexpr (decltype(drop_on)::value) {
@@ -332,7 +343,10 @@
     }
     flush_pending();
     };
-    if constexpr (SK) {
+    if constexpr (CK) {
+        static_assert(TR && PHASE == 0 && DT == 1 && !SK, "compact keys exist for the fused bf16 form at head dim 16");
+        dispatch_nk<NT>(NT - km.kt0, run);
+    } else if constexpr (SK) {
         static_assert(TR && PHASE == 0, "the key-tile skip exists for the fused bf16 form");
         dispatch_nk<NT>((p.flags & MAU_CAUSAL) ? NT : NT - km.kt0, run);
     } else {
@@ -344,7 +358,9 @@
 int launch_fwd_e(FwdP p, hipStream_t st) {
     constexpr int dh = 16 * DT;
     const size_t pack_bytes = PHASE == 0 ? pack_dims<T>(dh, p.E).fwd_bytes : 0;
-    constexpr size_t wave_bytes = fwd_wave_bytes<T, DT, NT, PHASE>();
+    constexpr bool CKF = sizeof(T) == 2 && DT == 1 && EC == 16 && PHASE == 0 && NT >= 2 && NT <= 8;
+    const bool ck = CKF && p.compact && p.flags == 0 && (p.rate <= 0.f || p.dbits);
+    const size_t wave_bytes = ck ? fwd_wave_bytes<T, DT, NT, PHASE, CKF>() : fwd_wave_bytes<T, DT, NT, PHASE>();
     int waves = 4;
     while (waves > 1 && pack_bytes + waves * wave_bytes > 80 * 1024) waves >>= 1;
     if (waves == 1 && pack_bytes + wave_bytes > 80 * 1024)
@@ -358,6 +374,7 @@
         const bool sk = NT >= 2 && bimau_skip_enabled() && !p.noskip;
         if (p.dbits && p.rate > 0.f) kern = sk ? bimau_fwd_kernel<T, DT, NT, EC, PHASE, true, (NT >= 2)> : bimau_fwd_kernel<T, DT, NT, EC, PHASE, true>;
         else if (sk) kern = bimau_fwd_kernel<T, DT, NT, EC, PHASE, false, (NT >= 2)>;
+        if (ck) kern = (p.dbits && p.rate > 0.f) ? bimau_fwd_kernel<T, DT, NT, EC, PHASE, true, false, CKF> : bimau_fwd_kernel<T, DT, NT, EC, PHASE, false, false, CKF>;
     }
     if (smem > 48 * 1024) hipFuncSetAttribute((const void*)kern, hipFuncAttributeMaxDynamicSharedMemorySize, (int)smem);
     const long jobs = (long)p.B * p.H;
diff --git a/easydgl_amd/csrc/k_bimau_bwd.hip b/easydgl_amd/csrc/k_bimau_bwd.hip
--- a/easydgl_amd/csrc/k_bimau_bwd.hip
+++ b/easydgl_amd/csrc/k_bimau_bwd.hip
@@ -330,9 +330,11 @@
     p.dsc_part = reinterpret_cast<float*>(ws + wl.dsc); p.wpart = reinterpret_cast<float*>(ws + wl.wpart);
     const long jobs = (long)p.B * p.H;
     constexpr bool TR = sizeof(T) == 2;
+    constexpr bool CKF = sizeof(T) == 2 && DT == 1 && NT >= 2 && NT <= 8;
+    const bool ck = CKF && p.compact && p.flags == 0 && p.E == 16 && (p.rate <= 0.f || p.dbits);
     edgl_prof_begin(EDGL_KERNEL_BIMAU_BWD_ALL, st);
     {
-        const size_t wave_bytes = (2 * (size_t)Tp * dh + (size_t)Tp * EP + (TR ? 0 : (size_t)EP * LDT)) * sizeof(T) + (size_t)Tp * sizeof(float);
+        const size_t wave_bytes = (2 * (size_t)Tp * dh + (size_t)Tp * EP + (TR ? 0 : (size_t)EP * LDT)) * sizeof(T) + (ck ? 2 : 1) * (size_t)Tp * sizeof(float);
         int waves = 4;
         while (waves > 1 && waves * wave_bytes > 64 * 1024) waves >>= 1;
         const size_t smem = waves * wave_bytes;
@@ -351,6 +353,10 @@
                     if (sk) kern = db ? bimau_bwd_sweep1_kernel<T, DT, NT, 16, true, 0, true, true, SKC> : bimau_bwd_sweep1_kernel<T, DT, NT, 16, true, 0, false, true, SKC>;
                     else kern = db ? bimau_bwd_sweep1_kernel<T, DT, NT, 16, true, 0, true, true> : bimau_bwd_sweep1_kernel<T, DT, NT, 16, true, 0, false, true>;
                 }
+                if (ck) {
+                    if (p.tpp_desc) kern = db ? bimau_bwd_sweep1_kernel<T, DT, NT, 16, true, 0, true, true, false, CKF> : bimau_bwd_sweep1_kernel<T, DT, NT, 16, true, 0, false, true, false, CKF>;
+                    else kern = db ? bimau_bwd_sweep1_kernel<T, DT, NT, 16, true, 0, true, false, false, CKF> : bimau_bwd_sweep1_kernel<T, DT, NT, 16, true, 0, false, false, false, CKF>;
+                }
             }
         }
         hipFuncSetAttribute((const void*)kern, hipFuncAttributeMaxDynamicSharedMemorySize, (int)smem);
@@ -371,7 +377,7 @@
         EDGL_LAUNCH_CHECK();
     }
     {
-        const size_t wave_bytes = (3 * (size_t)Tp * dh + (size_t)Tp * EP + (TR ? 0 : (size_t)dh * LDT)) * sizeof(T) + (size_t)Tp * sizeof(float);
+        const size_t wave_bytes = (3 * (size_t)Tp * dh + (size_t)Tp * EP + (TR ? 0 : (size_t)dh * LDT)) * sizeof(T) + (ck ? 2 : 1) * (size_t)Tp * sizeof(float);
         int waves = 4;
         while (waves > 1 && waves * wave_bytes > 80 * 1024) waves >>= 1;
         const size_t smem = waves * wave_bytes;
@@ -386,6 +392,7 @@
                 const bool sk = SKC && p.flags == 0 && p.E == 16 && bimau_skip_enabled() && !p.noskip;
                 if (p.flags == 0 && p.E == 16 && p.dbits && p.rate > 0.f) kern = sk ? bimau_bwd_sweep2_kernel<T, DT, NT, 16, KY_NY, true, 0, true, 1, 0, SKC> : bimau_bwd_sweep2_kernel<T, DT, NT, 16, KY_NY, true, 0, true>;
                 else if (sk) kern = bimau_bwd_sweep2_kernel<T, DT, NT, 16, KY_NY, true, 0, false, 1, 0, SKC>;
+                if (ck) kern = (p.dbits && p.rate > 0.f) ? bimau_bwd_sweep2_kernel<T, DT, NT, 16, KY_NY, true, 0, true, 1, 0, false, CKF> : bimau_bwd_sweep2_kernel<T, DT, NT, 16, KY_NY, true, 0, false, 1, 0, false, CKF>;
             }
         }
         hipFuncSetAttribute((const void*)kern, hipFuncAttributeMaxDynamicSharedMemorySize, (int)smem);
@@ -484,6 +491,7 @@
     p.z = reinterpret_cast<const float*>((const char*)saved + sl.off_z);
     p.B = B; p.T = T; p.C = C; p.H = H; p.E = E; p.rate = drop_rate; p.rng = rng_state;
     p.noskip = (flags & EDGL_MAU_NO_SKIP) ? 1 : 0; flags &= ~EDGL_MAU_NO_SKIP;
+    p.compact = (flags & EDGL_MAU_COMPACT) ? 1 : 0; flags &= ~EDGL_MAU_COMPACT;
     p.stream_id = stream_id; p.d_qkvt = d_qkvt; p.flags = flags; p.dbits = dropbits; p.qk_scale = qk_scale;
     p.tpp_desc = tpp_desc; p.tpp_M = tpp_M; p.tpp_sums = tpp_sums; p.tpp_coef = tpp_coef; p.tpp_part = tpp_part; p.order = order;
     EDGL_REQUIRE(!tpp_desc || (dtype == EDGL_BF16 && C / H == 16 && E == 16 && T <= 128 && flags == 0 && tpp_part && tpp_M > 0 && !d_lam_ext),
diff --git a/easydgl_amd/csrc/k_bimau_fwd.hip b/easydgl_amd/csrc/k_bimau_fwd.hip
--- a/easydgl_amd/csrc/k_bimau_fwd.hip
+++ b/easydgl_amd/csrc/k_bimau_fwd.hip
@@ -68,6 +68,28 @@
     hipStream_t st = (hipStream_t)stream;
     switch (nt) {
 #define EDGL_DB_CASE(N) case N: hipLaunchKernelGGL((bimau::dropbits_kernel<N>), grid, dim3(256), 0, st, rng_state, stream_id, drop_rate, T, njobs, bits); break;
+        EDGL_DB_CASE(1) EDGL_DB_CASE(2) EDGL_DB_CASE(3) EDGL_DB_CASE(4) EDGL_DB_CASE(5) EDGL_DB_CASE(6) EDGL_DB_CASE(7) EDGL_DB_CASE(8)
+#undef EDGL_DB_CASE
+    }
+    EDGL_LAUNCH_CHECK();
+    return EDGL_OK;
+}
+extern "C" int edgl_bimau_compact_supported(int T, int C, int H, int E, int flags, int dtype) {
+    if (T <= 0 || H <= 0 || C % H) return 0;
+    const int nt = (T + 15) / 16;
+    return (dtype == EDGL_BF16 && C / H == 16 && E == 16 && nt >= 2 && nt <= 8 && (flags & ~(EDGL_MAU_NO_SKIP | EDGL_MAU_COMPACT)) == 0) ? 1 : 0;
+}
+extern "C" int edgl_bimau_dropbits_ids(const int64_t* ids, int B, int T, int H, float drop_rate, const uint64_t* rng_state, uint32_t stream_id,
+                                       uint32_t* bits, void* stream) {
+    EDGL_REQUIRE(ids && rng_state && bits, EDGL_ERR_NULL, "edgl_bimau_dropbits_ids: null pointer");
+    EDGL_REQUIRE(B > 0 && T > 0 && H > 0 && T <= 128, EDGL_ERR_SHAPE, "edgl_bimau_dropbits_ids: bad shape B=%d T=%d H=%d (T <= 128)", B, T, H);
+    EDGL_REQUIRE((double)B * H * T * T < 4294967296.0, EDGL_ERR_SHAPE, "edgl_bimau_dropbits_ids: H*B*T*T must be < 2^32");
+    const int nt = (T + 15) / 16;
+    const long njobs = (long)B * H * nt;
+    const dim3 grid((unsigned)((njobs + 3) / 4));
+    hipStream_t st = (hipStream_t)stream;
+    switch (nt) {
+#define EDGL_DB_CASE(N) case N: hipLaunchKernelGGL((bimau::dropbits_compact_kernel<N>), grid, dim3(256), 0, st, rng_state, stream_id, drop_rate, ids, B, T, njobs, bits); break;
         EDGL_DB_CASE(1) EDGL_DB_CASE(2) EDGL_DB_CASE(3) EDGL_DB_CASE(4) EDGL_DB_CASE(5) EDGL_DB_CASE(6) EDGL_DB_CASE(7) EDGL_DB_CASE(8)
 #undef EDGL_DB_CASE
     }
@@ -117,10 +139,7 @@
     if (lane == 0) nk[b] = first < 0 ? NT : NT - (first >> 4);
 }
 constexpr int ORD_THREADS = 256;
-__global__ __launch_bounds__(ORD_THREADS) void job_rank_kernel(const int32_t* nk, int B, int32_t* order) {
-    extern __shared__ __attribute__((aligned(16))) int nk_s[];
-    for (int b = threadIdx.x; b < B; b += ORD_THREADS) nk_s[b] = nk[b];
-    __syncthreads();
+__device__ __forceinline__ void rank_samples(const int* nk_s, int B, int32_t* order) {
     for (int b = threadIdx.x; b < B; b += ORD_THREADS) {
         const int mine = nk_s[b];
         int rank = 0;
@@ -145,12 +164,49 @@
         order[rank] = b;
     }
 }
+__global__ __launch_bounds__(ORD_THREADS) void job_rank_kernel(const int32_t* nk, int B, int32_t* order) {
+    extern __shared__ __attribute__((aligned(16))) int nk_s[];
+    for (int b = threadIdx.x; b < B; b += ORD_THREADS) nk_s[b] = nk[b];
+    __syncthreads();
+    rank_samples(nk_s, B, order);
+}
+__global__ __launch_bounds__(ORD_THREADS) void job_order_compact_kernel(const int64_t* ids, int B, int T, int32_t* nk, unsigned* ctr, int32_t* order) {
+    extern __shared__ __attribute__((aligned(16))) int nk_s[];
+    __shared__ int last_s;
+    const int lane = threadIdx.x & 63, b = blockIdx.x * 4 + (threadIdx.x >> 6);
+    if (b < B) {
+        int n = 0;
+        for (int k0 = 0; k0 < T; k0 += 64) {
+            const int k = k0 + lane;
+            n += (int)__popcll(__ballot(k < T && ids[(long)b * T + min(k, T - 1)] != 0));
+        }
+        if (lane == 0) __hip_atomic_store(nk + b, bimau::compact_tiles(n, (T + 15) / 16), __ATOMIC_RELAXED, __HIP_MEMORY_SCOPE_AGENT);
+    }
+    __threadfence();
+    __syncthreads();
+    if (threadIdx.x == 0) last_s = atomicInc(ctr, gridDim.x - 1) == gridDim.x - 1 ? 1 : 0;
+    __syncthreads();
+    if (!last_s) return;
+    __threadfence();
+    for (int i = threadIdx.x; i < B; i += ORD_THREADS) nk_s[i] = __hip_atomic_load(nk + i, __ATOMIC_RELAXED, __HIP_MEMORY_SCOPE_AGENT);
+    __syncthreads();
+    rank_samples(nk_s, B, order);
+}
 }
 extern "C" int edgl_bimau_job_order(const int64_t* ids, int B, int T, int32_t* order, void* stream) {
     EDGL_REQUIRE(ids && order, EDGL_ERR_NULL, "edgl_bimau_job_order: null pointer");
     EDGL_REQUIRE(B > 0 && T > 0 && B <= 16384, EDGL_ERR_SHAPE, "edgl_bimau_job_order: bad shape B=%d T=%d (B <= 16384)", B, T);
     hipLaunchKernelGGL(job_tiles_kernel, dim3((B + 3) / 4), dim3(256), 0, (hipStream_t)stream, ids, B, T, order + B);
     hipLaunchKernelGGL(job_rank_kernel, dim3(1), dim3(ORD_THREADS), (size_t)((B + 3) & ~3) * sizeof(int), (hipStream_t)stream, order + B, B, order);
+    EDGL_LAUNCH_CHECK();
+    return EDGL_OK;
+}
+
+extern "C" int edgl_bimau_job_order_compact(const int64_t* ids, int B, int T, int32_t* order, void* stream) {
+    EDGL_REQUIRE(ids && order, EDGL_ERR_NULL, "edgl_bimau_job_order_compact: null pointer");
+    EDGL_REQUIRE(B > 0 && T > 0 && B <= 8192, EDGL_ERR_SHAPE, "edgl_bimau_job_order_compact: bad shape B=%d T=%d (B <= 8192)", B, T);
+    hipLaunchKernelGGL(job_order_compact_kernel, dim3((B + 3) / 4), dim3(ORD_THREADS), (size_t)((B + 3) & ~3) * sizeof(int), (hipStream_t)stream,
+                       ids, B, T, order + B, reinterpret_cast<unsigned*>(order + 2 * B), order);
     EDGL_LAUNCH_CHECK();
     return EDGL_OK;
 }
@@ -168,8 +224,9 @@
     EDGL_REQUIRE(ld_res % 4 == 0, EDGL_ERR_SHAPE, "edgl_bimau_fwd: ld_res must be a multiple of 4");
     EDGL_REQUIRE((double)B * H * T * T < 4294967296.0, EDGL_ERR_SHAPE, "edgl_bimau_fwd: H*B*T*T must be < 2^32");
     FwdP p{qkvt, resid, ld_res, ids, spans, marks, (const char*)pack, B, T, C, H, E, drop_rate, rng_state, stream_id,
-           out, lam_out, nullptr, nullptr, nullptr, 4, flags & ~EDGL_MAU_NO_SKIP, dropbits, qk_scale, order, (flags & EDGL_MAU_NO_SKIP) ? 1 : 0};
-    flags &= ~EDGL_MAU_NO_SKIP;
+           out, lam_out, nullptr, nullptr, nullptr, 4, flags & ~(EDGL_MAU_NO_SKIP | EDGL_MAU_COMPACT), dropbits, qk_scale, order,
+           (flags & EDGL_MAU_NO_SKIP) ? 1 : 0, (flags & EDGL_MAU_COMPACT) ? 1 : 0};
+    flags &= ~(EDGL_MAU_NO_SKIP | EDGL_MAU_COMPACT);
     hipStream_t st = (hipStream_t)stream;
     if (C / H == 64 || C / H == 128) {
         if (zero_rows && hipMemsetAsync(zero_rows, 0, (size_t)H * B * T * E * sizeof(float), st) != hipSuccess) {
diff --git a/easydgl_amd/engine.py b/easydgl_amd/engine.py
--- a/easydgl_amd/engine.py
+++ b/easydgl_amd/engine.py
@@ -21,7 +21,7 @@
         self.sw_flash_ce = env("EDGL_FLASH_CE", "1") != "0"
         self.sw_tpp_fused = env("EDGL_TPP_FUSED", "1") != "0"
         self.sw_prep_in_encoder = env("EDGL_PREP_IN_ENCODER", "1") != "0"
-        self.sw_bimau_order = env("EDGL_BIMAU_ORDER", "0") == "1"
+        self.sw_bimau_order = env("EDGL_BIMAU_ORDER", "1") != "0"
         self.sw_ce_parts = env("EDGL_CE_PARTS", "1") != "0"
         self.sw_defer_loss = env("EDGL_DEFER_LOSS", "1") != "0"
         self.sw_adam_ex = env("EDGL_ADAM_EX", "1") != "0"
@@ -61,6 +61,7 @@
         self.spans = e(B, T, dtype=f32)
         self.marks = e(B, T, E, dtype=torch.uint8)
         self.blk = []
+        have_bits = False
         for i in range(nb):
             d = dict(qkvt=e(B, T, 4 * C), att=e(B, T, C), lam=e(H * B, T, E, dtype=f32), ao=e(B, T, C), a1=e(B, T, C),
                      st1=e(B, 2, dtype=f32), pre_f=e(B, T, 2 * C), f=e(B, T, 2 * C), o=e(B, T, C), y=e(B, T, C),
@@ -72,6 +73,7 @@
                      tpp=torch.zeros(max(lib.edgl_tpp_workspace(), lib.edgl_tpp_rows_workspace(B, H, M)), device=dev, dtype=f32))
             nb_bits = int(lib.edgl_bimau_dropbits_bytes(B, T, H)) if m.attention_probs_dropout_rate > 0 else 0
             d["dbits"] = e(nb_bits // 4, dtype=torch.int32) if nb_bits > 0 else None
+            have_bits = nb_bits > 0
             if self.mgroups:
                 dh = C // H
                 d["grp"] = []
@@ -84,8 +86,10 @@
                         lam=e(H * B, T, eg, dtype=f32), dlam=e(H * B, T, eg, dtype=f32),
                         out=e(B, T, C) if e0 else None, dqkvt=e(B, T, 4 * C) if e0 else None))
             self.blk.append(d)
-        self.job_order = (torch.arange(2 * B, device=dev, dtype=torch.int32)
-                          if (not self.mgroups and B <= 16384 and nb > 0 and self.sw_bimau_order) else None)
+        self.compact = (not self.mgroups and nb > 0 and (m.attention_probs_dropout_rate <= 0 or have_bits)
+                        and bool(lib.edgl_bimau_compact_supported(T, C, H, E, 0, self.code)))
+        self.job_order = (torch.cat([torch.arange(2 * B, dtype=torch.int32), torch.zeros(1, dtype=torch.int32)]).to(dev)
+                          if (self.compact and B <= 8192 and self.sw_bimau_order) else None)
         self.tpp_desc = torch.zeros(int(lib.edgl_tpp_prep_bytes(B, T, M)), device=dev, dtype=torch.uint8) if self.fused_tpp else None
         self.zero_resid = torch.zeros((B, T, C), device=dev, dtype=self.dt) if self.mgroups else None
         self.pre_t, self.so, self.st3 = e(B, T, C), e(B, T, C), e(B, 2, dtype=f32)
@@ -122,7 +126,7 @@
         self._pending_label = None
         self._lazy_loss, self._side_has_grads, self._loss_unjoined = False, False, False
         self._label_fused = False
-        self.mau_flags = _lib.MAU_NO_SKIP
+        self.mau_flags = _lib.MAU_COMPACT if self.compact else _lib.MAU_NO_SKIP
         self.adam_ex = (not use_graph) and self.sw_adam_ex
         self._rng_alt, self._adam_alt = torch.zeros_like(m._rng_state), torch.zeros_like(m._adam_state)
         self._slabs = None
@@ -283,7 +287,7 @@
                 tab.grad.zero_()
                 m.output_bias.grad.zero_()
             if self.job_order is not None:
-                check(lib.edgl_bimau_job_order(_ptr(self.ids), B, T, _ptr(self.job_order), sst), "edgl_bimau_job_order")
+                check(lib.edgl_bimau_job_order_compact(_ptr(self.ids), B, T, _ptr(self.job_order), sst), "edgl_bimau_job_order_compact")
             for i, (blk, b) in enumerate(zip(m.layers, self.blk)):
                 att = blk.attention
                 if m.ct_reg != 0.0 and not self._dp and not self.fused_tpp:
@@ -302,7 +306,10 @@
                 else:
                     check(lib.edgl_bimau_pack(_ptr(att.st_kernel), _ptr(att.st_bias), _ptr(att.weight), _ptr(att.scaling), C, H, E,
                                               _ptr(b["pack"]), code, sst), "edgl_bimau_pack")
-                if b["dbits"] is not None:
+                if b["dbits"] is not None and self.compact:
+                    check(lib.edgl_bimau_dropbits_ids(_ptr(self.ids), B, T, H, float(ad), _ptr(m._rng_state), 10 + 4 * i, _ptr(b["dbits"]),
+                                                      sst), "edgl_bimau_dropbits_ids")
+                elif b["dbits"] is not None:
                     check(lib.edgl_bimau_dropbits(B, T, H, float(ad), _ptr(m._rng_state), 10 + 4 * i, _ptr(b["dbits"]), sst),
                           "edgl_bimau_dropbits")
             l2_behind = l2_from_parts and bool(self.blk)
diff --git a/include/easydgl_hip.h b/include/easydgl_hip.h
--- a/include/easydgl_hip.h
+++ b/include/easydgl_hip.h
@@ -104,6 +104,8 @@
 #define EDGL_MAU_NO_DIAG 2
 #define EDGL_MAU_DIAG_ZERO 4
 #define EDGL_MAU_NO_SKIP 8
+#define EDGL_MAU_COMPACT 16
+int edgl_bimau_compact_supported(int T, int C, int H, int E, int flags, int dtype);
 long edgl_bimau_pack_bytes(int C, int H, int E, int dtype);
 long edgl_bimau_saved_bytes(int B, int T, int C, int H, int dtype);
 int edgl_bimau_mark_group(int C, int H, int dtype);
@@ -121,12 +123,15 @@
 long edgl_bimau_dropbits_bytes(int B, int T, int H);
 int edgl_bimau_dropbits(int B, int T, int H, float drop_rate, const uint64_t* rng_state, uint32_t stream_id, uint32_t* bits,
                         void* stream);
+int edgl_bimau_dropbits_ids(const int64_t* ids, int B, int T, int H, float drop_rate, const uint64_t* rng_state, uint32_t stream_id,
+                            uint32_t* bits, void* stream);
 int edgl_bimau_fwd_db(const void* qkvt, const void* resid, int ld_res, const int64_t* ids, const float* spans,
                       const uint8_t* marks, const void* pack, int B, int T, int C, int H, int E, float drop_rate,
                       const uint64_t* rng_state, uint32_t stream_id, const uint32_t* dropbits, float qk_scale, void* out,
                       float* lam_out, void* saved, float* zero_rows, int flags, int dtype, void* stream);
 
 int edgl_bimau_job_order(const int64_t* ids, int B, int T, int32_t* order, void* stream);
+int edgl_bimau_job_order_compact(const int64_t* ids, int B, int T, int32_t* order, void* stream);
 int edgl_bimau_fwd_ord(const void* qkvt, const void* resid, int ld_res, const int64_t* ids, const float* spans,
                        const uint8_t* marks, const void* pack, int B, int T, int C, int H, int E, float drop_rate,
                        const uint64_t* rng_state, uint32_t stream_id, const uint32_t* dropbits, float qk_scale, void* out,
```

New measurement: 629,700. -5.1%, worse.
